# cocowy1/Cost-Volume-Aggregation-in-Stereo-Matching-Revisited

Hardware: AMD Instinct MI355X
Metric: cost-volumes/sec (fwd+bwd) at 544x960 D=192 (higher is better)
Workload: dtype f32

## Files before the change

### cost-volume-aggregation-in-stereo-matching-revisited_amd/csrc/pointwise.hip

```cpp
#include "dca_frag.h"
#include "../../include/dca_hip.h"

__global__ __launch_bounds__(256) void bn_stats_kernel(const float* __restrict__ x, double* __restrict__ part, int N,
                                                       int C, long S, int nchunk, long chunk_len, int vec) {
  const int c = blockIdx.x, ch = blockIdx.y, tid = threadIdx.x;
  const long s0 = ch * chunk_len, s1 = min(S, s0 + chunk_len);
  const float K = x[(long)c * S];
  if (ch == 0 && tid == 0) part[(long)C * nchunk * 2 + c] = (double)K;
  float s = 0.f, ss = 0.f;
  for (int n = 0; n < N; ++n) {
    const float* p = x + ((long)n * C + c) * S;
    if (vec) {
      for (long i = s0 + 4 * tid; i < s1; i += 1024) {
        float4 v = *(const float4*)(p + i);
        v.x -= K; v.y -= K; v.z -= K; v.w -= K;
        s += (v.x + v.y) + (v.z + v.w);
        ss += (v.x * v.x + v.y * v.y) + (v.z * v.z + v.w * v.w);
      }
    } else {
      for (long i = s0 + tid; i < s1; i += 256) {
        const float v = p[i] - K;
        s += v;
        ss += v * v;
      }
    }
  }
  double ds = wave_sum_d((double)s), dss = wave_sum_d((double)ss);
  __shared__ double red[8];
  if ((tid & 63) == 0) { red[(tid >> 6) * 2] = ds; red[(tid >> 6) * 2 + 1] = dss; }
  __syncthreads();
  if (tid == 0) {
    part[((long)c * nchunk + ch) * 2 + 0] = red[0] + red[2] + red[4] + red[6];
    part[((long)c * nchunk + ch) * 2 + 1] = red[1] + red[3] + red[5] + red[7];
  }
}

__device__ __forceinline__ int bn_bound_exp(float gamma, float beta, double count, int c, const unsigned* rp_slots, int rp_n,
                                            const unsigned* rq_slots, int rq_n) {
  unsigned a = 0, b2 = 0;
  const int lane = threadIdx.x & 63;
  if (rp_slots) for (int i = lane; i < rp_n; i += 64) { const unsigned u = rp_slots[(long)c * DCA_AMAX_CSLOTS + i]; a = a > u ? a : u; }
  if (rq_slots) for (int i = lane; i < rq_n; i += 64) { const unsigned u = rq_slots[(long)c * DCA_AMAX_CSLOTS + i]; b2 = b2 > u ? b2 : u; }
#pragma unroll
  for (int o = 32; o > 0; o >>= 1) {
    const unsigned u = (unsigned)__shfl_xor((int)a, o, 64), w = (unsigned)__shfl_xor((int)b2, o, 64);
    a = a > u ? a : u;
    b2 = b2 > w ? b2 : w;
  }
  const float b = (fabsf(gamma) * sqrtf((float)count) + fabsf(beta) + __uint_as_float(a) + __uint_as_float(b2)) * 1.0001f;
  return x2_scale_exp(__float_as_uint(b));
}

__global__ __launch_bounds__(64) void bn_finalize_kernel(const double* __restrict__ part, int nchunk, double count,
                                   const float* __restrict__ gamma, const float* __restrict__ beta,
                                   float* __restrict__ running_mean, float* __restrict__ running_var, float momentum,
                                   float eps, int training, float* __restrict__ stats, int* __restrict__ zexps,
                                   const unsigned* __restrict__ rp_slots, int rp_n, const unsigned* __restrict__ rq_slots,
                                   int rq_n, int C) {
  const int c = blockIdx.x, lane = threadIdx.x;
  float mean, var;
  if (training) {
    double s = 0.0, ss = 0.0;
    for (int i = lane; i < nchunk; i += 64) {
      s += part[((long)c * nchunk + i) * 2 + 0];
      ss += part[((long)c * nchunk + i) * 2 + 1];
    }
    s = wave_sum_d(s);
    ss = wave_sum_d(ss);
    const double ms = s / count;
    double v = ss / count - ms * ms;
    if (v < 0.0) v = 0.0;
    const double m = part[(long)C * nchunk * 2 + c] + ms;
    mean = (float)m;
    var = (float)v;
    if (running_mean && lane == 0) {
      const double unb = count > 1.0 ? v * count / (count - 1.0) : v;
      running_mean[c] = (1.f - momentum) * running_mean[c] + momentum * mean;
      running_var[c] = (1.f - momentum) * running_var[c] + momentum * (float)unb;
    }
  } else {
    mean = running_mean[c];
    var = running_var[c];
  }
  const float g = gamma ? gamma[c] : 1.f, b = beta ? beta[c] : 0.f;
  const int ze = zexps ? bn_bound_exp(g, b, count, c, rp_slots, rp_n, rq_slots, rq_n) : 0;
  if (lane != 0) return;
  const float invstd = 1.0f / sqrtf(var + eps);
  stats[c] = mean;
  stats[C + c] = invstd;
  stats[2 * C + c] = g * invstd;
  stats[3 * C + c] = b - mean * g * invstd;
  if (zexps) zexps[c] = ze;
}

__global__ __launch_bounds__(64) void bn_finalize_centered_kernel(const double* __restrict__ part, int nchunk,
                                   const float* __restrict__ gamma, const float* __restrict__ beta,
                                   float* __restrict__ running_mean, float* __restrict__ running_var, float momentum,
                                   float eps, float* __restrict__ stats, int* __restrict__ zexps,
                                   const unsigned* __restrict__ rp_slots, int rp_n, const unsigned* __restrict__ rq_slots,
                                   int rq_n, int C) {
  const int c = blockIdx.x, lane = threadIdx.x;
  const double* p = part + (long)c * nchunk * 4;
  const double kref = p[0];
  double n = 0.0, s = 0.0, q = 0.0;
  for (int i = lane; i < nchunk; i += 64) {
    const double ki = p[i * 4 + 0], ni = p[i * 4 + 1], si = p[i * 4 + 2], qi = p[i * 4 + 3];
    const double dk = ki - kref;
    n += ni;
    s += si + ni * dk;
    q += qi + 2.0 * dk * si + ni * dk * dk;
  }
  n = wave_sum_d(n);
  s = wave_sum_d(s);
  q = wave_sum_d(q);
  const float g = gamma ? gamma[c] : 1.f, b = beta ? beta[c] : 0.f;
  const int ze = zexps ? bn_bound_exp(g, b, n, c, rp_slots, rp_n, rq_slots, rq_n) : 0;
  if (lane != 0) return;
  const double ms = s / n;
  double v = q / n - ms * ms;
  if (v < 0.0) v = 0.0;
  const float mean = (float)(kref + ms), var = (float)v;
  if (running_mean) {
    const double unb = n > 1.0 ? v * n / (n - 1.0) : v;
    running_mean[c] = (1.f - momentum) * running_mean[c] + momentum * mean;
    running_var[c] = (1.f - momentum) * running_var[c] + momentum * (float)unb;
  }
  const float invstd = 1.0f / sqrtf(var + eps);
  stats[c] = mean;
  stats[C + c] = invstd;
  stats[2 * C + c] = g * invstd;
  stats[3 * C + c] = b - mean * g * invstd;
  if (zexps) zexps[c] = ze;
}


__global__ __launch_bounds__(256) void bn_apply_kernel(const float* __restrict__ y, const float* __restrict__ stats,
                                                       const float* __restrict__ res_pre, const float* __restrict__ res_post,
                                                       float* __restrict__ z, int N, int C, long S, long chunk_len,
                                                       float slope, int vec, unsigned* __restrict__ zmax,
                                                       unsigned* __restrict__ ymax) {
  const int c = blockIdx.y, ch = blockIdx.x, tid = threadIdx.x;
  const long s0 = ch * chunk_len, s1 = min(S, s0 + chunk_len);
  const float mean = stats[c], sc = stats[2 * C + c], sh = stats[3 * C + c];
  float am = 0.f, ym = 0.f;
  for (int n = N - 1; n >= 0; --n) {
    const long base = ((long)n * C + c) * S;
    if (vec) {
      for (long i = s0 + 4 * tid; i < s1; i += 1024) {
        float4 v = *(const float4*)(y + base + i);
        ym = fmaxf(fmaxf(ym, fmaxf(fabsf(v.x - mean), fabsf(v.y - mean))), fmaxf(fabsf(v.z - mean), fabsf(v.w - mean)));
        v.x = v.x * sc + sh; v.y = v.y * sc + sh; v.z = v.z * sc + sh; v.w = v.w * sc + sh;
        if (res_pre) { const float4 r = *(const float4*)(res_pre + base + i); v.x += r.x; v.y += r.y; v.z += r.z; v.w += r.w; }
        v.x = act_apply(v.x, slope); v.y = act_apply(v.y, slope); v.z = act_apply(v.z, slope); v.w = act_apply(v.w, slope);
        if (res_post) { const float4 r = *(const float4*)(res_post + base + i); v.x += r.x; v.y += r.y; v.z += r.z; v.w += r.w; }
        *(float4*)(z + base + i) = v;
        am = fmaxf(fmaxf(am, fmaxf(fabsf(v.x), fabsf(v.y))), fmaxf(fabsf(v.z), fabsf(v.w)));
      }
    } else {
      for (long i = s0 + tid; i < s1; i += 256) {
        const float yv = y[base + i];
        ym = fmaxf(ym, fabsf(yv - mean));
        float v = yv * sc + sh;
        if (res_pre) v += res_pre[base + i];
        v = act_apply(v, slope);
        if (res_post) v += res_post[base + i];
        z[base + i] = v;
        am = fmaxf(am, fabsf(v));
      }
    }
  }
  if (zmax) dca_cmax_put(am, zmax + (long)c * DCA_AMAX_CSLOTS + ch);
  if (ymax) dca_cmax_put(ym, ymax + (long)c * DCA_AMAX_CSLOTS + ch);
}

__device__ __forceinline__ void px2_split(float v, int e, unsigned short& h, unsigned short& l) {
  _Float16 hh, ll;
  x2_split(v, e, hh, ll);
  h = __builtin_bit_cast(unsigned short, hh);
  l = __builtin_bit_cast(unsigned short, ll);
}
typedef unsigned short u16x8 __attribute__((ext_vector_type(8)));

__global__ __launch_bounds__(256) void bn_apply_pack_kernel(const float* __restrict__ y, const float* __restrict__ stats,
                                                            const int* __restrict__ zexps, char* __restrict__ zp, int N,
                                                            int C, long S, long chunk_len, float slope,
                                                            unsigned* __restrict__ ymax, const float* __restrict__ res_pre,
                                                            const float* __restrict__ res_post, float* __restrict__ zf,
                                                            unsigned* __restrict__ zmax) {
  const int cg = blockIdx.y, ch = blockIdx.x, tid = threadIdx.x;
  const long s0 = ch * chunk_len, s1 = min(S, s0 + chunk_len);
  float mean[8], sc[8], sh[8], ym[8], zm[8];
  int ex[8];
#pragma unroll
  for (int j = 0; j < 8; ++j) {
    const int c = cg * 8 + j;
    mean[j] = stats ? stats[c] : 0.f;
    sc[j] = stats ? stats[2 * C + c] : 1.f;
    sh[j] = stats ? stats[3 * C + c] : 0.f;
    ex[j] = dca_coherent_loadi(zexps + c);
    ym[j] = zm[j] = 0.f;
  }
  const long tb = px2_term_bytes(C, S);
  for (int n = N - 1; n >= 0; --n) {
    const float* yb = y + ((long)n * C + cg * 8) * S;
    char* zb = zp + (long)n * 2 * tb + (long)cg * S * 16;
    const long cb = ((long)n * C + cg * 8) * S;
    for (long i = s0 + tid; i < s1; i += 256) {
      float v[8], rp[8], rq[8];
#pragma unroll
      for (int j = 0; j < 8; ++j) {
        v[j] = yb[j * S + i];
        rp[j] = res_pre ? res_pre[cb + j * S + i] : -0.f;
        rq[j] = res_post ? res_post[cb + j * S + i] : -0.f;
      }
      u16x8 hv, lv;
#pragma unroll
      for (int j = 0; j < 8; ++j) {
        ym[j] = fmaxf(ym[j], fabsf(v[j] - mean[j]));
        const float zz = act_apply(v[j] * sc[j] + sh[j] + rp[j], slope) + rq[j];
        if (zf) zf[cb + j * S + i] = zz;
        zm[j] = fmaxf(zm[j], fabsf(zz));
        unsigned short h, l;
        px2_split(zz, ex[j], h, l);
        hv[j] = h; lv[j] = l;
      }
      *(u16x8*)(zb + i * 16) = hv;
      *(u16x8*)(zb + tb + i * 16) = lv;
    }
  }
  if (ymax) {
#pragma unroll
    for (int j = 0; j < 8; ++j) dca_cmax_put(ym[j], ymax + (long)(cg * 8 + j) * DCA_AMAX_CSLOTS + ch);
  }
  if (zmax) {
#pragma unroll
    for (int j = 0; j < 8; ++j) dca_cmax_put(zm[j], zmax + (long)(cg * 8 + j) * DCA_AMAX_CSLOTS + ch);
  }
}

__global__ __launch_bounds__(256) void bn_apply_pack4_kernel(const float* __restrict__ y, const float* __restrict__ stats,
                                                             const int* __restrict__ zexps, char* __restrict__ zp, int N,
                                                             int C, long S, long chunk_len, float slope,
                                                             unsigned* __restrict__ ymax, const float* __restrict__ res_pre,
                                                             const float* __restrict__ res_post, float* __restrict__ zf,
                                                             unsigned* __restrict__ zmax) {
  const int cg = blockIdx.y, ch = blockIdx.x, tid = threadIdx.x;
  const long s0 = ch * chunk_len, s1 = min(S, s0 + chunk_len);
  float mean[8], sc[8], sh[8], ym[8], zm[8];
  int ex[8];
#pragma unroll
  for (int j = 0; j < 8; ++j) {
    const int c = cg * 8 + j;
    mean[j] = stats ? stats[c] : 0.f;
    sc[j] = stats ? stats[2 * C + c] : 1.f;
    sh[j] = stats ? stats[3 * C + c] : 0.f;
    ex[j] = dca_coherent_loadi(zexps + c);
    ym[j] = zm[j] = 0.f;
  }
  const long tb = px2_term_bytes(C, S);
  for (int n = N - 1; n >= 0; --n) {
    const long cb = ((long)n * C + cg * 8) * S;
    char* zb = zp + (long)n * 2 * tb + (long)cg * S * 16;
    for (long i = s0 + 4 * tid; i < s1; i += 1024) {
      u16x8 hv[4], lv[4];
#pragma unroll
      for (int j = 0; j < 8; ++j) {
        const float4 v4 = *(const float4*)(y + cb + j * S + i);
        float4 p4 = make_float4(-0.f, -0.f, -0.f, -0.f), q4 = p4;
        if (res_pre) p4 = *(const float4*)(res_pre + cb + j * S + i);
        if (res_post) q4 = *(const float4*)(res_post + cb + j * S + i);
        const float v[4] = {v4.x, v4.y, v4.z, v4.w}, rp[4] = {p4.x, p4.y, p4.z, p4.w}, rq[4] = {q4.x, q4.y, q4.z, q4.w};
        float zz[4];
#pragma unroll
        for (int e = 0; e < 4; ++e) {
          ym[j] = fmaxf(ym[j], fabsf(v[e] - mean[j]));
          zz[e] = act_apply(v[e] * sc[j] + sh[j] + rp[e], slope) + rq[e];
          zm[j] = fmaxf(zm[j], fabsf(zz[e]));
          unsigned short h, l;
          px2_split(zz[e], ex[j], h, l);
          hv[e][j] = h; lv[e][j] = l;
        }
        if (zf) *(float4*)(zf + cb + j * S + i) = make_float4(zz[0], zz[1], zz[2], zz[3]);
      }
#pragma unroll
      for (int e = 0; e < 4; ++e) {
        *(u16x8*)(zb + (i + e) * 16) = hv[e];
        *(u16x8*)(zb + tb + (i + e) * 16) = lv[e];
      }
    }
  }
  if (ymax) {
#pragma unroll
    for (int j = 0; j < 8; ++j) dca_cmax_put(ym[j], ymax + (long)(cg * 8 + j) * DCA_AMAX_CSLOTS + ch);
  }
  if (zmax) {
#pragma unroll
    for (int j = 0; j < 8; ++j) dca_cmax_put(zm[j], zmax + (long)(cg * 8 + j) * DCA_AMAX_CSLOTS + ch);
  }
}

__global__ __launch_bounds__(256) void cmax_kernel(const float* __restrict__ x, int N, int C, long S, long chunk_len, int vec,
                                                   unsigned* __restrict__ slots) {
  const int c = blockIdx.y, ch = blockIdx.x, tid = threadIdx.x;
  const long s0 = ch * chunk_len, s1 = min(S, s0 + chunk_len);
  float m = 0.f;
  for (int n = 0; n < N; ++n) {
    const float* p = x + ((long)n * C + c) * S;
    if (vec) {
      for (long i = s0 + 4 * tid; i < s1; i += 1024) {
        const float4 v = *(const float4*)(p + i);
        m = fmaxf(fmaxf(m, fmaxf(fabsf(v.x), fabsf(v.y))), fmaxf(fabsf(v.z), fabsf(v.w)));
      }
    } else {
      for (long i = s0 + tid; i < s1; i += 256) m = fmaxf(m, fabsf(p[i]));
    }
  }
  dca_cmax_put(m, slots + (long)c * DCA_AMAX_CSLOTS + ch);
}

__global__ __launch_bounds__(64) void cmax_exps_kernel(const unsigned* __restrict__ slots, int nslots, int* __restrict__ exps) {
  const int c = blockIdx.x, lane = threadIdx.x;
  unsigned v = 0;
  for (int i = lane; i < nslots; i += 64) { const unsigned u = slots[(long)c * DCA_AMAX_CSLOTS + i]; v = v > u ? v : u; }
#pragma unroll
  for (int o = 32; o > 0; o >>= 1) { const unsigned u = (unsigned)__shfl_xor((int)v, o, 64); v = v > u ? v : u; }
  if (lane == 0) exps[c] = x2_scale_exp(v);
}

__global__ __launch_bounds__(256) void bn_bwd_reduce_kernel(const float* __restrict__ dz, const float* __restrict__ y,
                                                            const float* __restrict__ res_pre,
                                                            const float* __restrict__ stats,
                                                            double* __restrict__ part, int N, int C, long S,
                                                            int nchunk, long chunk_len, float slope, int vec,
                                                            unsigned* __restrict__ gmax) {
  const int c = blockIdx.x, ch = blockIdx.y, tid = threadIdx.x;
  const long s0 = ch * chunk_len, s1 = min(S, s0 + chunk_len);
  const float mean = stats[c], invstd = stats[C + c], sc = stats[2 * C + c], sh = stats[3 * C + c];
  float a0 = 0.f, a1 = 0.f, gm = 0.f;
  for (int n = N - 1; n >= 0; --n) {
    const long base = ((long)n * C + c) * S;
    if (vec) {
      for (long i = s0 + 4 * tid; i < s1; i += 1024) {
        const float4 yv = *(const float4*)(y + base + i);
        const float4 dv = *(const float4*)(dz + base + i);
        float4 rv = make_float4(0.f, 0.f, 0.f, 0.f);
        if (res_pre) rv = *(const float4*)(res_pre + base + i);
        const float ys[4] = {yv.x, yv.y, yv.z, yv.w}, ds[4] = {dv.x, dv.y, dv.z, dv.w}, rs[4] = {rv.x, rv.y, rv.z, rv.w};
#pragma unroll
        for (int j = 0; j < 4; ++j) {
          const float u = ys[j] * sc + sh + rs[j];
          const float g = ds[j] * (u > 0.f ? 1.f : slope);
          a0 += g;
          a1 += g * (ys[j] - mean) * invstd;
          gm = fmaxf(gm, fabsf(g));
        }
      }
    } else {
      for (long i = s0 + tid; i < s1; i += 256) {
        const float yv = y[base + i];
        float u = yv * sc + sh;
        if (res_pre) u += res_pre[base + i];
        const float g = dz[base + i] * (u > 0.f ? 1.f : slope);
        a0 += g;
        a1 += g * (yv - mean) * invstd;
        gm = fmaxf(gm, fabsf(g));
      }
    }
  }
  double d0 = wave_sum_d((double)a0), d1 = wave_sum_d((double)a1);
  __shared__ double red[8];
  if ((tid & 63) == 0) { red[(tid >> 6) * 2] = d0; red[(tid >> 6) * 2 + 1] = d1; }
  __syncthreads();
  if (tid == 0) {
    part[((long)c * nchunk + ch) * 2 + 0] = red[0] + red[2] + red[4] + red[6];
    part[((long)c * nchunk + ch) * 2 + 1] = red[1] + red[3] + red[5] + red[7];
  }
  if (gmax) dca_cmax_put(gm, gmax + (long)c * DCA_AMAX_CSLOTS + ch);
}

__global__ __launch_bounds__(64) void bn_bwd_finalize_kernel(const double* __restrict__ part, int nchunk, double count,
                                       float* __restrict__ dgb, int C, const float* __restrict__ stats, int training,
                                       const unsigned* __restrict__ gmax, const unsigned* __restrict__ ymax, int ymax_slots,
                                       int* __restrict__ dyexps) {
  const int c = blockIdx.x, lane = threadIdx.x;
  double s0 = 0.0, s1 = 0.0;
  for (int i = lane; i < nchunk; i += 64) {
    s0 += part[((long)c * nchunk + i) * 2 + 0];
    s1 += part[((long)c * nchunk + i) * 2 + 1];
  }
  s0 = wave_sum_d(s0);
  s1 = wave_sum_d(s1);
  unsigned gmb = 0, ymb = 0;
  if (dyexps) {
    for (int i = lane; i < nchunk; i += 64) { const unsigned u = gmax[(long)c * DCA_AMAX_CSLOTS + i]; gmb = gmb > u ? gmb : u; }
    if (ymax)
      for (int i = lane; i < ymax_slots; i += 64) { const unsigned u = ymax[(long)c * DCA_AMAX_CSLOTS + i]; ymb = ymb > u ? ymb : u; }
#pragma unroll
    for (int o = 32; o > 0; o >>= 1) {
      const unsigned u = (unsigned)__shfl_xor((int)gmb, o, 64), w = (unsigned)__shfl_xor((int)ymb, o, 64);
      gmb = gmb > u ? gmb : u;
      ymb = ymb > w ? ymb : w;
    }
  }
  if (lane != 0) return;
  dgb[c] = (float)s1;
  dgb[C + c] = (float)s0;
  dgb[2 * C + c] = (float)(s0 / count);
  dgb[3 * C + c] = (float)(s1 / count);
  if (dyexps) {
    const float invstd = stats[C + c], sc = fabsf(stats[2 * C + c]);
    const float xh = ymax ? __uint_as_float(ymb) * invstd : sqrtf((float)count);
    float bound = __uint_as_float(gmb);
    if (training) bound += fabsf((float)(s0 / count)) + xh * fabsf((float)(s1 / count));
    dyexps[c] = x2_scale_exp(__float_as_uint(bound * sc * 1.0001f));
  }
}

__global__ __launch_bounds__(256) void bn_bwd_apply_kernel(const float* __restrict__ dz, const float* __restrict__ y,
                                    const float* __restrict__ res_pre, const float* __restrict__ stats,
                                    const float* __restrict__ dgb, float* __restrict__ dy, float* __restrict__ g_out,
                                    int N, int C, long S, long chunk_len, float slope, int training, int vec,
                                    unsigned* __restrict__ dmax) {
  const int c = blockIdx.y, ch = blockIdx.x, tid = threadIdx.x;
  const long s0 = ch * chunk_len, s1 = min(S, s0 + chunk_len);
  const float mean = stats[c], invstd = stats[C + c], sc = stats[2 * C + c], sh = stats[3 * C + c];
  const float k1 = training ? dgb[2 * C + c] : 0.f, k2 = training ? dgb[3 * C + c] * invstd : 0.f;
  float am = 0.f;
  for (int n = 0; n < N; ++n) {
    const long base = ((long)n * C + c) * S;
    if (vec) {
      for (long i = s0 + 4 * tid; i < s1; i += 1024) {
        const float4 yv = *(const float4*)(y + base + i), dv = *(const float4*)(dz + base + i);
        float4 rv = make_float4(0.f, 0.f, 0.f, 0.f);
        if (res_pre) rv = *(const float4*)(res_pre + base + i);
        const float ys[4] = {yv.x, yv.y, yv.z, yv.w}, ds[4] = {dv.x, dv.y, dv.z, dv.w}, rs[4] = {rv.x, rv.y, rv.z, rv.w};
        float o[4], g[4];
#pragma unroll
        for (int j = 0; j < 4; ++j) {
          const float u = ys[j] * sc + sh + rs[j];
          g[j] = ds[j] * (u > 0.f ? 1.f : slope);
          o[j] = (g[j] - k1 - (ys[j] - mean) * k2) * sc;
        }
        *(float4*)(dy + base + i) = make_float4(o[0], o[1], o[2], o[3]);
        if (g_out) *(float4*)(g_out + base + i) = make_float4(g[0], g[1], g[2], g[3]);
        am = fmaxf(fmaxf(am, fmaxf(fabsf(o[0]), fabsf(o[1]))), fmaxf(fabsf(o[2]), fabsf(o[3])));
      }
    } else {
      for (long i = s0 + tid; i < s1; i += 256) {
        const float yv = y[base + i];
        float u = yv * sc + sh;
        if (res_pre) u += res_pre[base + i];
        const float g = dz[base + i] * (u > 0.f ? 1.f : slope);
        float v = g;
        if (training) v -= dgb[2 * C + c] + (yv - mean) * invstd * dgb[3 * C + c];
        dy[base + i] = v * sc;
        if (g_out) g_out[base + i] = g;
        am = fmaxf(am, fabsf(v * sc));
      }
    }
  }
  if (dmax) dca_cmax_put(am, dmax + (long)c * DCA_AMAX_CSLOTS + ch);
}

__global__ __launch_bounds__(256) void bn_bwd_apply_pack_kernel(const float* __restrict__ dz, const float* __restrict__ y,
                                    const float* __restrict__ stats, const float* __restrict__ dgb,
                                    const int* __restrict__ dyexps, char* __restrict__ dyp, int N, int C, long S,
                                    long chunk_len, float slope, int training) {
  const int cg = blockIdx.y, ch = blockIdx.x, tid = threadIdx.x;
  const long s0 = ch * chunk_len, s1 = min(S, s0 + chunk_len);
  float mean[8], sc[8], sh[8], k1[8], k2[8];
  int ex[8];
#pragma unroll
  for (int j = 0; j < 8; ++j) {
    const int c = cg * 8 + j;
    mean[j] = stats[c]; sc[j] = stats[2 * C + c]; sh[j] = stats[3 * C + c];
    k1[j] = training ? dca_coherent_loadf(dgb + 2 * C + c) : 0.f;
    k2[j] = training ? dca_coherent_loadf(dgb + 3 * C + c) * stats[C + c] : 0.f;
    ex[j] = dca_coherent_loadi(dyexps + c);
  }
  const long tb = px2_term_bytes(C, S);
  for (int n = 0; n < N; ++n) {
    const long base = ((long)n * C + cg * 8) * S;
    char* ob = dyp + (long)n * 2 * tb + (long)cg * S * 16;
    for (long i = s0 + tid; i < s1; i += 256) {
      float yv[8], dv[8];
#pragma unroll
      for (int j = 0; j < 8; ++j) { yv[j] = y[base + j * S + i]; dv[j] = dz[base + j * S + i]; }
      u16x8 hv, lv;
#pragma unroll
      for (int j = 0; j < 8; ++j) {
        const float u = yv[j] * sc[j] + sh[j];
        const float g = dv[j] * (u > 0.f ? 1.f : slope);
        const float o = (g - k1[j] - (yv[j] - mean[j]) * k2[j]) * sc[j];
        unsigned short h, l;
        px2_split(o, ex[j], h, l);
        hv[j] = h; lv[j] = l;
      }
      *(u16x8*)(ob + i * 16) = hv;
      *(u16x8*)(ob + tb + i * 16) = lv;
    }
  }
}

__global__ __launch_bounds__(256) void avgpool3d_fwd_kernel(const float* __restrict__ x, float* __restrict__ y, int Di,
                                                            int Hi, int Wi, int Do, int Ho, int Wo) {
  const long row = blockIdx.x;
  const int od = (int)(row % Do);
  const long nc = row / Do;
  const long plane = (long)Di * Hi * Wi;
  const __amdgpu_buffer_rsrc_t xr = dca_rsrc(x + nc * plane, plane * 4);
  const int HW = Ho * Wo, end = min(HW, ((int)blockIdx.y + 1) * 1024);
  for (int i = blockIdx.y * 1024 + threadIdx.x; i < end; i += 256) {
    const int oh = i / Wo, ow = i - oh * Wo;
    float s = 0.f;
#pragma unroll
    for (int kd = 0; kd < 3; ++kd) {
      const int d = 2 * od - 1 + kd;
#pragma unroll
      for (int kh = 0; kh < 3; ++kh) {
        const int h = 2 * oh - 1 + kh;
#pragma unroll
        for (int kw = 0; kw < 3; ++kw) {
          const int w = 2 * ow - 1 + kw;
          const int ok = (int)((unsigned)d < (unsigned)Di) & (int)((unsigned)h < (unsigned)Hi) & (int)((unsigned)w < (unsigned)Wi);
          s += dca_bload1(xr, ((d * Hi + h) * Wi + w) * 4, ok);
        }
      }
    }
    y[row * HW + i] = s * (1.0f / 27.0f);
  }
}

__global__ __launch_bounds__(256) void avgpool3d_bwd_kernel(const float* __restrict__ gy, float* __restrict__ gx,
                                                            const float* __restrict__ res, const float* __restrict__ res2,
                                                            int Di, int Hi, int Wi, int Do, int Ho, int Wo) {
  const long row = blockIdx.x;
  const int d = (int)(row % Di);
  const long nc = row / Di;
  const long plane = (long)Do * Ho * Wo;
  const __amdgpu_buffer_rsrc_t gr = dca_rsrc(gy + nc * plane, plane * 4);
  const int HW = Hi * Wi, end = min(HW, ((int)blockIdx.y + 1) * 1024);
  const int d0 = d >> 1, dn = d & 1;
  for (int i = blockIdx.y * 1024 + threadIdx.x; i < end; i += 256) {
    const int h = i / Wi, w = i - h * Wi;
    const int h0 = h >> 1, hn = h & 1, w0 = w >> 1, wn = w & 1;
    float s = 0.f;
#pragma unroll
    for (int a = 0; a < 2; ++a)
#pragma unroll
      for (int b = 0; b < 2; ++b)
#pragma unroll
        for (int c = 0; c < 2; ++c) {
          const int od = d0 + a, oh = h0 + b, ow = w0 + c;
          const int ok = (a <= dn) & (b <= hn) & (c <= wn) & (int)(od < Do) & (int)(oh < Ho) & (int)(ow < Wo);
          s += dca_bload1(gr, ((od * Ho + oh) * Wo + ow) * 4, ok);
        }
    float o = s * (1.0f / 27.0f) + (res ? res[row * HW + i] : 0.f);
    if (res2) o += res2[row * HW + i];
    gx[row * HW + i] = o;
  }
}

__global__ __launch_bounds__(256) void avgpool3d_fwd_tiled_kernel(const float* __restrict__ x, float* __restrict__ y,
                                                                  int Di, int Hi, int Wi, int Do, int Ho, int Wo) {
  constexpr int TH = 8, TW = 32, FH = 2 * TH + 1, PW = 2 * TW + 2;
  __shared__ __attribute__((aligned(16))) float tile[3 * FH * PW];
  const int tid = threadIdx.x, ow0 = blockIdx.x * TW, oh0 = blockIdx.y * TH;
  const int od = blockIdx.z % Do;
  const long nc = blockIdx.z / Do;
  const long plane = (long)Di * Hi * Wi;
  const __amdgpu_buffer_rsrc_t xr = dca_rsrc(x + nc * plane, plane * 4);
  constexpr int NQ = 3 * FH * 16, KQ = (NQ + 255) / 256;
  float4 rq[KQ];
#pragma unroll
  for (int k = 0; k < KQ; ++k) {
    const int it = tid + 256 * k, q = it & 15, row = it >> 4, a = row / FH, b = row - a * FH;
    const int d = 2 * od - 1 + a, h = 2 * oh0 - 1 + b, w = 2 * ow0 + 4 * q;
    const int ok = (int)(it < NQ) & (int)((unsigned)d < (unsigned)Di) & (int)((unsigned)h < (unsigned)Hi) & (int)(w < Wi);
    rq[k] = dca_bload4(xr, ((d * Hi + h) * Wi + w) * 4, ok);
  }
  float redge = 0.f;
  {
    const int a = tid / FH, b = tid - a * FH;
    const int d = 2 * od - 1 + a, h = 2 * oh0 - 1 + b, w = 2 * ow0 - 1;
    const int ok = (int)(tid < 3 * FH) & (int)((unsigned)d < (unsigned)Di) & (int)((unsigned)h < (unsigned)Hi) &
                   (int)((unsigned)w < (unsigned)Wi);
    redge = dca_bload1(xr, ((d * Hi + h) * Wi + w) * 4, ok);
  }
#pragma unroll
  for (int k = 0; k < KQ; ++k) {
    const int it = tid + 256 * k;
    if (it < NQ) {
      float* p = tile + (it >> 4) * PW + 1 + 4 * (it & 15);
      p[0] = rq[k].x; p[1] = rq[k].y; p[2] = rq[k].z; p[3] = rq[k].w;
    }
  }
  if (tid < 3 * FH) tile[tid * PW] = redge;
  __syncthreads();
  const int hl = tid >> 5, wl = tid & 31, oh = oh0 + hl, ow = ow0 + wl;
  if (oh >= Ho || ow >= Wo) return;
  float s = 0.f;
#pragma unroll
  for (int kd = 0; kd < 3; ++kd)
#pragma unroll
    for (int kh = 0; kh < 3; ++kh) {
      const float* row = tile + (kd * FH + 2 * hl + kh) * PW + 2 * wl;
      const float2 lo = *(const float2*)row;
      s += lo.x;
      s += lo.y;
      s += row[2];
    }
  y[((nc * Do + od) * Ho + oh) * (long)Wo + ow] = s * (1.0f / 27.0f);
}

__global__ __launch_bounds__(256) void avgpool3d_bwd_vec_kernel(const float* __restrict__ gy, float* __restrict__ gx,
                                                                const float* __restrict__ res, const float* __restrict__ res2,
                                                                int Di, int Hi, int Wi, int Do, int Ho, int Wo) {
  const int BD = Di / 2 + 1, BH = Hi / 2 + 1;
  const int bd = (int)(blockIdx.x % BD);
  const long nc = blockIdx.x / BD;
  const long plane = (long)Do * Ho * Wo;
  const __amdgpu_buffer_rsrc_t gr = dca_rsrc(gy + nc * plane, plane * 4);
  const int WQ = Wi >> 2, HQ = BH * WQ, end = min(HQ, ((int)blockIdx.y + 1) * 1024);
  for (int i = blockIdx.y * 1024 + threadIdx.x; i < end; i += 256) {
    const int bh = i / WQ, t = i - bh * WQ, c0 = 2 * t;
    float g[2][2][3];
#pragma unroll
    for (int a = 0; a < 2; ++a)
#pragma unroll
      for (int b = 0; b < 2; ++b)
#pragma unroll
        for (int c = 0; c < 3; ++c) {
          const int od = bd - 1 + a, oh = bh - 1 + b, ow = c0 + c;
          const int ok = (int)((unsigned)od < (unsigned)Do) & (int)((unsigned)oh < (unsigned)Ho) & (int)(ow < Wo);
          g[a][b][c] = dca_bload1(gr, ((od * Ho + oh) * Wo + ow) * 4, ok);
        }
#pragma unroll
    for (int pd = 0; pd < 2; ++pd) {
      const int d = 2 * bd - 1 + pd;
      if ((unsigned)d >= (unsigned)Di) continue;
#pragma unroll
      for (int ph = 0; ph < 2; ++ph) {
        const int h = 2 * bh - 1 + ph;
        if ((unsigned)h >= (unsigned)Hi) continue;
        float o[4];
#pragma unroll
        for (int e = 0; e < 4; ++e) {
          float s = 0.f;
#pragma unroll
          for (int a = pd; a < 2; ++a)
#pragma unroll
            for (int b = ph; b < 2; ++b) {
              s += g[a][b][e >> 1];
              s += (e & 1) ? g[a][b][(e + 1) >> 1] : 0.f;
            }
          o[e] = s * (1.0f / 27.0f);
        }
        const long off = ((nc * Di + d) * Hi + h) * (long)Wi + 4 * t;
        if (res) {
          const float4 r = *(const float4*)(res + off);
          o[0] += r.x; o[1] += r.y; o[2] += r.z; o[3] += r.w;
        }
        if (res2) {
          const float4 r = *(const float4*)(res2 + off);
          o[0] += r.x; o[1] += r.y; o[2] += r.z; o[3] += r.w;
        }
        *(float4*)(gx + off) = make_float4(o[0], o[1], o[2], o[3]);
      }
    }
  }
}

__device__ __forceinline__ void lin_src(int o, float rs, int n, int& i0, int& i1, float& l0, float& l1) {
  float src = rs * ((float)o + 0.5f) - 0.5f;
  if (src < 0.f) src = 0.f;
  i0 = (int)src;
  i1 = i0 + (i0 < n - 1 ? 1 : 0);
  l1 = src - (float)i0;
  l0 = 1.f - l1;
}

__global__ void trilinear_fwd_kernel(const float* __restrict__ x, float* __restrict__ y, long NC, int Di, int Hi,
                                     int Wi, int s) {
  const int Do = Di * s, Ho = Hi * s, Wo = Wi * s;
  const float rs = 1.0f / (float)s;
  const long total = NC * Do * Ho * Wo;
  for (long idx = (long)blockIdx.x * blockDim.x + threadIdx.x; idx < total; idx += (long)gridDim.x * blockDim.x) {
    const int ow = idx % Wo;
    long t = idx / Wo;
    const int oh = t % Ho; t /= Ho;
    const int od = t % Do;
    const long nc = t / Do;
    int d0, d1, h0, h1, w0, w1;
    float ld0, ld1, lh0, lh1, lw0, lw1;
    lin_src(od, rs, Di, d0, d1, ld0, ld1);
    lin_src(oh, rs, Hi, h0, h1, lh0, lh1);
    lin_src(ow, rs, Wi, w0, w1, lw0, lw1);
    const float* p = x + nc * Di * Hi * Wi;
#define XV(d, h, w) p[((long)(d) * Hi + (h)) * Wi + (w)]
    const float v = ld0 * (lh0 * (lw0 * XV(d0, h0, w0) + lw1 * XV(d0, h0, w1)) +
                           lh1 * (lw0 * XV(d0, h1, w0) + lw1 * XV(d0, h1, w1))) +
                    ld1 * (lh0 * (lw0 * XV(d1, h0, w0) + lw1 * XV(d1, h0, w1)) +
                           lh1 * (lw0 * XV(d1, h1, w0) + lw1 * XV(d1, h1, w1)));
#undef XV
    y[idx] = v;
  }
}

__device__ __forceinline__ float lin_w(int o, int i, float rs, int n) {
  int i0, i1;
  float l0, l1;
  lin_src(o, rs, n, i0, i1, l0, l1);
  return (i0 == i ? l0 : 0.f) + (i1 == i ? l1 : 0.f);
}

__global__ void trilinear_bwd_kernel(const float* __restrict__ gy, float* __restrict__ gx, long NC, int Di, int Hi,
                                     int Wi, int s) {
  const int Do = Di * s, Ho = Hi * s, Wo = Wi * s;
  const float rs = 1.0f / (float)s;
  const long total = NC * Di * Hi * Wi;
  const int lo_off = (s + 1) / 2, hi_off = (3 * s) / 2 - 1 + (s & 1);
  for (long idx = (long)blockIdx.x * blockDim.x + threadIdx.x; idx < total; idx += (long)gridDim.x * blockDim.x) {
    const int w = idx % Wi;
    long t = idx / Wi;
    const int h = t % Hi; t /= Hi;
    const int d = t % Di;
    const long nc = t / Di;
    const float* p = gy + nc * Do * Ho * Wo;
    const int od0 = max(0, s * d - lo_off), od1 = min(Do - 1, s * d + hi_off);
    const int oh0 = max(0, s * h - lo_off), oh1 = min(Ho - 1, s * h + hi_off);
    const int ow0 = max(0, s * w - lo_off), ow1 = min(Wo - 1, s * w + hi_off);
    float acc = 0.f;
    for (int od = od0; od <= od1; ++od) {
      const float wd = lin_w(od, d, rs, Di);
      if (wd == 0.f) continue;
      for (int oh = oh0; oh <= oh1; ++oh) {
        const float wh = lin_w(oh, h, rs, Hi);
        if (wh == 0.f) continue;
        const float* row = p + ((long)od * Ho + oh) * Wo;
        float r = 0.f;
        for (int ow = ow0; ow <= ow1; ++ow) r += lin_w(ow, w, rs, Wi) * row[ow];
        acc += wd * wh * r;
      }
    }
    gx[idx] = acc;
  }
}

__global__ __launch_bounds__(256) void trilinear_up2_fwd_kernel(const float* __restrict__ x, float* __restrict__ y,
                                                                int Di, int Hi, int Wi) {
  const int mw = blockIdx.x * 64 + (threadIdx.x & 63), mh = blockIdx.y * 4 + (threadIdx.x >> 6);
  const int md = blockIdx.z % Di;
  const long nc = blockIdx.z / Di;
  if (mw >= Wi || mh >= Hi) return;
  const float* p = x + nc * Di * Hi * Wi;
  const int dm = max(md - 1, 0), dp = min(md + 1, Di - 1), hm = max(mh - 1, 0), hp = min(mh + 1, Hi - 1);
  const int wm = max(mw - 1, 0), wp = min(mw + 1, Wi - 1);
  float r0[3][3], r1[3][3];
  const int ds[3] = {dm, md, dp}, hs[3] = {hm, mh, hp};
#pragma unroll
  for (int a = 0; a < 3; ++a)
#pragma unroll
    for (int b = 0; b < 3; ++b) {
      const float* row = p + ((long)ds[a] * Hi + hs[b]) * Wi;
      const float xm = row[wm], x0 = row[mw], xp = row[wp];
      r0[a][b] = 0.25f * xm + 0.75f * x0;
      r1[a][b] = 0.75f * x0 + 0.25f * xp;
    }
  const int Ho = 2 * Hi, Wo = 2 * Wi;
  float* q = y + nc * (2L * Di) * Ho * Wo;
#pragma unroll
  for (int pd = 0; pd < 2; ++pd)
#pragma unroll
    for (int ph = 0; ph < 2; ++ph) {
      const int a0 = pd ? 1 : 0, a1 = pd ? 2 : 1, b0 = ph ? 1 : 0, b1 = ph ? 2 : 1;
      const float wa0 = pd ? 0.75f : 0.25f, wa1 = pd ? 0.25f : 0.75f, wb0 = ph ? 0.75f : 0.25f, wb1 = ph ? 0.25f : 0.75f;
      float2 o;
      o.x = wa0 * (wb0 * r0[a0][b0] + wb1 * r0[a0][b1]) + wa1 * (wb0 * r0[a1][b0] + wb1 * r0[a1][b1]);
      o.y = wa0 * (wb0 * r1[a0][b0] + wb1 * r1[a0][b1]) + wa1 * (wb0 * r1[a1][b0] + wb1 * r1[a1][b1]);
      *(float2*)(q + ((long)(2 * md + pd) * Ho + 2 * mh + ph) * Wo + 2 * mw) = o;
    }
}

__device__ __forceinline__ void up2_bwd_w(int i, int n, float w[4]) {
  w[0] = (i > 0) ? 0.25f : 0.f;
  w[1] = (i > 0) ? 0.75f : 1.0f;
  w[2] = (i < n - 1) ? 0.75f : 1.0f;
  w[3] = (i < n - 1) ? 0.25f : 0.f;
}

__global__ __launch_bounds__(256) void trilinear_up2_bwd_kernel(const float* __restrict__ gy, float* __restrict__ gx,
                                                                int Di, int Hi, int Wi) {
  const int w = blockIdx.x * 256 + threadIdx.x, h = blockIdx.y;
  const int d = blockIdx.z % Di;
  const long nc = blockIdx.z / Di;
  const int Ho = 2 * Hi, Wo = 2 * Wi;
  const long plane = (2L * Di) * Ho * Wo;
  const __amdgpu_buffer_rsrc_t gr = dca_rsrc(gy + nc * plane, plane * 4);
  const int wok = (int)(w < Wi);
  float wd[4], wh[4], ww[4];
  up2_bwd_w(d, Di, wd); up2_bwd_w(h, Hi, wh); up2_bwd_w(w, Wi, ww);
  float acc = 0.f;
#pragma unroll
  for (int a = 0; a < 4; ++a) {
    const int od = 2 * d - 1 + a;
#pragma unroll
    for (int b = 0; b < 4; ++b) {
      const int oh = 2 * h - 1 + b;
      const int ok = wok & (int)(wd[a] != 0.f) & (int)(wh[b] != 0.f);
      const int off = ((od * Ho + oh) * Wo + 2 * w) * 4;
      const float2 mid = dca_bload2(gr, off, ok);
      const float lo = dca_bload1(gr, off - 4, ok & (int)(ww[0] != 0.f));
      const float hi = dca_bload1(gr, off + 8, ok & (int)(ww[3] != 0.f));
      float r = ww[1] * mid.x + ww[2] * mid.y;
      r += ww[0] * lo;
      r += ww[3] * hi;
      acc += wd[a] * wh[b] * r;
    }
  }
  if (wok) gx[((nc * Di + d) * Hi + h) * Wi + w] = acc;
}

__global__ __launch_bounds__(256) void trilinear_up2_bwd_tiled_kernel(const float* __restrict__ gy, float* __restrict__ gx,
                                                                      int Di, int Hi, int Wi) {
  constexpr int TH = 8, TW = 32, FH = 2 * TH + 2, FW = 2 * TW + 2, PW = FW + 2;
  __shared__ __attribute__((aligned(16))) float tile[4 * FH * PW];
  const int tid = threadIdx.x, w0 = blockIdx.x * TW, h0 = blockIdx.y * TH;
  const int d = blockIdx.z % Di;
  const long nc = blockIdx.z / Di;
  const int Do = 2 * Di, Ho = 2 * Hi, Wo = 2 * Wi;
  const long plane = (long)Do * Ho * Wo;
  const __amdgpu_buffer_rsrc_t gr = dca_rsrc(gy + nc * plane, plane * 4);
  constexpr int NQ = 4 * FH * 16, KQ = (NQ + 255) / 256;
  float4 rq[KQ];
#pragma unroll
  for (int k = 0; k < KQ; ++k) {
    const int it = tid + 256 * k, q = it & 15, row = it >> 4, a = row / FH, b = row - a * FH;
    const int od = 2 * d - 1 + a, oh = 2 * h0 - 1 + b, ow = 2 * w0 + 4 * q;
    const int ok = (int)(it < NQ) & (int)((unsigned)od < (unsigned)Do) & (int)((unsigned)oh < (unsigned)Ho) &
                   (int)(ow < Wo);
    rq[k] = dca_bload4(gr, ((od * Ho + oh) * Wo + ow) * 4, ok);
  }
  float redge = 0.f;
  {
    const int side = tid & 1, row = tid >> 1, a = row / FH, b = row - a * FH;
    const int od = 2 * d - 1 + a, oh = 2 * h0 - 1 + b, ow = side ? 2 * w0 + 2 * TW : 2 * w0 - 1;
    const int ok = (int)(tid < 4 * FH * 2) & (int)((unsigned)od < (unsigned)Do) & (int)((unsigned)oh < (unsigned)Ho) &
                   (int)((unsigned)ow < (unsigned)Wo);
    redge = dca_bload1(gr, ((od * Ho + oh) * Wo + ow) * 4, ok);
  }
#pragma unroll
  for (int k = 0; k < KQ; ++k) {
    const int it = tid + 256 * k;
    if (it < NQ) {
      float* p = tile + (it >> 4) * PW + 1 + 4 * (it & 15);
      p[0] = rq[k].x; p[1] = rq[k].y; p[2] = rq[k].z; p[3] = rq[k].w;
    }
  }
  if (tid < 4 * FH * 2) tile[(tid >> 1) * PW + ((tid & 1) ? FW - 1 : 0)] = redge;
  __syncthreads();
  const int hl = tid >> 5, wl = tid & 31, h = h0 + hl, w = w0 + wl;
  if (h >= Hi || w >= Wi) return;
  float wd[4], wh[4], ww[4];
  up2_bwd_w(d, Di, wd); up2_bwd_w(h, Hi, wh); up2_bwd_w(w, Wi, ww);
  float acc = 0.f;
#pragma unroll
  for (int a = 0; a < 4; ++a)
#pragma unroll
    for (int b = 0; b < 4; ++b) {
      const float* row = tile + (a * FH + 2 * hl + b) * PW + 2 * wl;
      const float2 lo = *(const float2*)row, hi = *(const float2*)(row + 2);
      float r = ww[1] * lo.y + ww[2] * hi.x;
      r += ww[0] * lo.x;
      r += ww[3] * hi.y;
      acc += wd[a] * wh[b] * r;
    }
  gx[((nc * Di + d) * Hi + h) * Wi + w] = acc;
}

static int ew_grid(long total) {
  long g = (total + 255) / 256;
  return (int)(g < 8192 ? (g > 0 ? g : 1) : 8192);
}

static void chunking(long S, int C, int* nchunk, long* chunk_len) {
  long want = (2048 + C - 1) / C;
  if (want > 256) want = 256;
  long len = (S + want - 1) / want;
  len = ((len + 1023) / 1024) * 1024;
  *chunk_len = len;
  *nchunk = (int)((S + len - 1) / len);
}

extern "C" int dca_bn_num_chunks(int C, long S) {
  int n; long l;
  chunking(S, C, &n, &l);
  return n;
}
extern "C" int dca_bn_pack_chunks(int C, long S) {
  int n; long l;
  chunking(S, (C + 7) / 8, &n, &l);
  return n;
}

extern "C" int dca_bn_stats(const float* x, double* part, int N, int C, long S, hipStream_t stream) {
  DCA_REQUIRE(x && part && N > 0 && C > 0 && S > 0 && C <= 65535);
  int nchunk; long len;
  chunking(S, C, &nchunk, &len);
  const int vec = (S % 4 == 0) && (((uintptr_t)x & 15) == 0);
  hipLaunchKernelGGL(bn_stats_kernel, dim3(C, nchunk), dim3(256), 0, stream, x, part, N, C, S, nchunk, len, vec);
  return dca_launch_status();
}

extern "C" int dca_bn_finalize(const double* part, int nchunk, double count, const float* gamma, const float* beta,
                               float* running_mean, float* running_var, float momentum, float eps, int training,
                               float* stats, int* zexps, const unsigned* rpre_slots, int rpre_n,
                               const unsigned* rpost_slots, int rpost_n, int C, hipStream_t stream) {
  DCA_REQUIRE(stats && C > 0 && (training ? (part != nullptr && nchunk > 0) : (running_mean && running_var)));
  DCA_REQUIRE(zexps == nullptr || training);
  DCA_REQUIRE((rpre_slots == nullptr || (rpre_n > 0 && rpre_n <= DCA_AMAX_CSLOTS)) &&
              (rpost_slots == nullptr || (rpost_n > 0 && rpost_n <= DCA_AMAX_CSLOTS)));
  hipLaunchKernelGGL(bn_finalize_kernel, dim3(C), dim3(64), 0, stream, part, nchunk, count, gamma, beta,
                     running_mean, running_var, momentum, eps, training, stats, zexps, rpre_slots, rpre_n, rpost_slots,
                     rpost_n, C);
  return dca_launch_status();
}

extern "C" int dca_bn_finalize_centered(const double* part, int nchunk, const float* gamma, const float* beta,
                                        float* running_mean, float* running_var, float momentum, float eps, float* stats,
                                        int* zexps, const unsigned* rpre_slots, int rpre_n, const unsigned* rpost_slots,
                                        int rpost_n, int C, hipStream_t stream) {
  DCA_REQUIRE(part && nchunk > 0 && stats && C > 0 && ((running_mean == nullptr) == (running_var == nullptr)));
  DCA_REQUIRE((rpre_slots == nullptr || (rpre_n > 0 && rpre_n <= DCA_AMAX_CSLOTS)) &&
              (rpost_slots == nullptr || (rpost_n > 0 && rpost_n <= DCA_AMAX_CSLOTS)));
  hipLaunchKernelGGL(bn_finalize_centered_kernel, dim3(C), dim3(64), 0, stream, part, nchunk, gamma, beta, running_mean,
                     running_var, momentum, eps, stats, zexps, rpre_slots, rpre_n, rpost_slots, rpost_n, C);
  return dca_launch_status();
}

extern "C" int dca_bn_apply(const float* y, const float* stats, const float* res_pre, const float* res_post, float* z,
                            int N, int C, long S, float slope, unsigned* zmax, unsigned* ymax, hipStream_t stream) {
  DCA_REQUIRE(y && stats && z && N > 0 && C > 0 && S > 0 && C <= 65535);
  int nchunk; long len;
  chunking(S, C, &nchunk, &len);
  const uintptr_t al = (uintptr_t)y | (uintptr_t)z | (uintptr_t)res_pre | (uintptr_t)res_post;
  const int vec = (S % 4 == 0) && ((al & 15) == 0);
  hipLaunchKernelGGL(bn_apply_kernel, dim3(nchunk, C), dim3(256), 0, stream, y, stats, res_pre, res_post, z, N, C, S, len,
                     slope, vec, zmax, ymax);
  return dca_launch_status();
}

extern "C" int dca_bn_apply_pack(const float* y, const float* stats, const int* zexps, void* zp, int N, int C, long S,
                                 float slope, unsigned* ymax, const float* res_pre, const float* res_post, float* zf,
                                 unsigned* zmax, hipStream_t stream) {
  DCA_REQUIRE(y && zexps && zp && N > 0 && C > 0 && C % 8 == 0 && S > 0 && C / 8 <= 65535 && ((((uintptr_t)zp) & 15) == 0));
  DCA_REQUIRE(stats != nullptr || (ymax == nullptr && slope == 1.f));
  int nchunk; long len;
  chunking(S, C / 8, &nchunk, &len);
  const uintptr_t al = (uintptr_t)y | (uintptr_t)res_pre | (uintptr_t)res_post | (uintptr_t)zf;
  const bool four = (res_pre || res_post) && S % 4 == 0 && (al & 15) == 0;
  auto kern = four ? bn_apply_pack4_kernel : bn_apply_pack_kernel;
  hipLaunchKernelGGL(kern, dim3(nchunk, C / 8), dim3(256), 0, stream, y, stats, zexps, (char*)zp, N, C, S, len, slope, ymax,
                     res_pre, res_post, zf, zmax);
  return dca_launch_status();
}

extern "C" int dca_cmax_f32(const float* x, int N, int C, long S, unsigned* slots, hipStream_t stream) {
  DCA_REQUIRE(x && slots && N > 0 && C > 0 && S > 0 && C <= 65535);
  int nchunk; long len;
  chunking(S, C, &nchunk, &len);
  const int vec = (S % 4 == 0) && ((((uintptr_t)x) & 15) == 0);
  hipLaunchKernelGGL(cmax_kernel, dim3(nchunk, C), dim3(256), 0, stream, x, N, C, S, len, vec, slots);
  return dca_launch_status();
}

extern "C" int dca_cmax_exps(const unsigned* slots, int nslots, int C, int* exps, hipStream_t stream) {
  DCA_REQUIRE(slots && exps && C > 0 && nslots > 0 && nslots <= DCA_AMAX_CSLOTS);
  hipLaunchKernelGGL(cmax_exps_kernel, dim3(C), dim3(64), 0, stream, slots, nslots, exps);
  return dca_launch_status();
}

extern "C" int dca_bn_backward(const float* dz, const float* y, const float* res_pre, const float* stats,
                               double* part, float* dgb, float* dy, float* g_out, int N, int C, long S, float slope,
                               int training, unsigned* dmax, hipStream_t stream) {
  DCA_REQUIRE(dz && y && stats && part && dgb && dy && N > 0 && C > 0 && S > 0 && C <= 65535);
  int nchunk; long len;
  chunking(S, C, &nchunk, &len);
  const uintptr_t al = (uintptr_t)dz | (uintptr_t)y | (uintptr_t)res_pre | (uintptr_t)dy | (uintptr_t)g_out;
  const int vec = (S % 4 == 0) && ((al & 15) == 0);
  hipLaunchKernelGGL(bn_bwd_reduce_kernel, dim3(C, nchunk), dim3(256), 0, stream, dz, y, res_pre, stats, part, N, C, S,
                     nchunk, len, slope, vec, (unsigned*)nullptr);
  hipLaunchKernelGGL(bn_bwd_finalize_kernel, dim3(C), dim3(64), 0, stream, part, nchunk, (double)N * (double)S, dgb, C,
                     stats, training, (const unsigned*)nullptr, (const unsigned*)nullptr, 0, (int*)nullptr);
  hipLaunchKernelGGL(bn_bwd_apply_kernel, dim3(nchunk, C), dim3(256), 0, stream, dz, y, res_pre, stats, dgb, dy, g_out, N, C,
                     S, len, slope, training, vec, dmax);
  return dca_launch_status();
}

extern "C" int dca_bn_backward_reduce(const float* dz, const float* y, const float* stats, double* part, float* dgb, int N,
                                      int C, long S, float slope, int training, hipStream_t stream) {
  DCA_REQUIRE(dz && y && stats && part && dgb && N > 0 && C > 0 && S > 0 && C <= 65535);
  int nchunk; long len;
  chunking(S, C, &nchunk, &len);
  const int vec = (S % 4 == 0) && ((((uintptr_t)dz | (uintptr_t)y) & 15) == 0);
  hipLaunchKernelGGL(bn_bwd_reduce_kernel, dim3(C, nchunk), dim3(256), 0, stream, dz, y, (const float*)nullptr, stats, part,
                     N, C, S, nchunk, len, slope, vec, (unsigned*)nullptr);
  hipLaunchKernelGGL(bn_bwd_finalize_kernel, dim3(C), dim3(64), 0, stream, part, nchunk, (double)N * (double)S, dgb, C,
                     stats, training, (const unsigned*)nullptr, (const unsigned*)nullptr, 0, (int*)nullptr);
  return dca_launch_status();
}

extern "C" int dca_bn_backward_pack(const float* dz, const float* y, const float* stats, double* part, float* dgb, void* dyp,
                                    int* dyexps, unsigned* gmax, const unsigned* ymax, int ymax_slots, int N, int C, long S,
                                    float slope, int training, hipStream_t stream) {
  DCA_REQUIRE(dz && y && stats && part && dgb && dyp && dyexps && gmax && N > 0 && C > 0 && C % 8 == 0 && S > 0 && C <= 65535);
  DCA_REQUIRE((ymax == nullptr || (ymax_slots > 0 && ymax_slots <= DCA_AMAX_CSLOTS)) && ((((uintptr_t)dyp) & 15) == 0));
  int nchunk; long len;
  chunking(S, C, &nchunk, &len);
  const uintptr_t al = (uintptr_t)dz | (uintptr_t)y;
  const int vec = (S % 4 == 0) && ((al & 15) == 0);
  hipLaunchKernelGGL(bn_bwd_reduce_kernel, dim3(C, nchunk), dim3(256), 0, stream, dz, y, (const float*)nullptr, stats, part,
                     N, C, S, nchunk, len, slope, vec, gmax);
  hipLaunchKernelGGL(bn_bwd_finalize_kernel, dim3(C), dim3(64), 0, stream, part, nchunk, (double)N * (double)S, dgb, C,
                     stats, training, (const unsigned*)gmax, ymax, ymax_slots, dyexps);
  int pchunk; long plen;
  chunking(S, C / 8, &pchunk, &plen);
  hipLaunchKernelGGL(bn_bwd_apply_pack_kernel, dim3(pchunk, C / 8), dim3(256), 0, stream, dz, y, stats, dgb, dyexps,
                     (char*)dyp, N, C, S, plen, slope, training);
  return dca_launch_status();
}

extern "C" int dca_avgpool3d_fwd(const float* x, float* y, long NC, int Di, int Hi, int Wi, hipStream_t stream) {
  DCA_REQUIRE(x && y && NC > 0 && Di > 0 && Hi > 0 && Wi > 0);
  const int Do = (Di + 1) / 2, Ho = (Hi + 1) / 2, Wo = (Wi + 1) / 2;
  DCA_REQUIRE((long)Di * Hi * Wi * 4 < 0x7ffffff0L && NC * Do < 0x7fffffffL);
  if (Wi % 4 == 0 && (((uintptr_t)x) & 15) == 0 && NC * Do <= 65535 && cdiv(Ho, 8) <= 65535) {
    hipLaunchKernelGGL(avgpool3d_fwd_tiled_kernel, dim3(cdiv(Wo, 32), cdiv(Ho, 8), (unsigned)(NC * Do)), dim3(256), 0, stream,
                       x, y, Di, Hi, Wi, Do, Ho, Wo);
    return dca_launch_status();
  }
  hipLaunchKernelGGL(avgpool3d_fwd_kernel, dim3((unsigned)(NC * Do), cdiv((long)Ho * Wo, 1024)), dim3(256), 0, stream, x,
                     y, Di, Hi, Wi, Do, Ho, Wo);
  return dca_launch_status();
}

extern "C" int dca_avgpool3d_bwd(const float* gy, float* gx, const float* res, const float* res2, long NC, int Di, int Hi,
                                 int Wi, hipStream_t stream) {
  DCA_REQUIRE(gy && gx && NC > 0 && Di > 0 && Hi > 0 && Wi > 0 && (res || !res2));
  const int Do = (Di + 1) / 2, Ho = (Hi + 1) / 2, Wo = (Wi + 1) / 2;
  DCA_REQUIRE((long)Di * Hi * Wi * 4 < 0x7ffffff0L && NC * Di < 0x7fffffffL);
  if (Wi % 4 == 0 && ((((uintptr_t)gx) | ((uintptr_t)res) | ((uintptr_t)res2)) & 15) == 0) {
    hipLaunchKernelGGL(avgpool3d_bwd_vec_kernel, dim3((unsigned)(NC * (Di / 2 + 1)), cdiv((long)(Hi / 2 + 1) * (Wi / 4), 1024)),
                       dim3(256), 0, stream, gy, gx, res, res2, Di, Hi, Wi, Do, Ho, Wo);
    return dca_launch_status();
  }
  hipLaunchKernelGGL(avgpool3d_bwd_kernel, dim3((unsigned)(NC * Di), cdiv((long)Hi * Wi, 1024)), dim3(256), 0, stream, gy,
                     gx, res, res2, Di, Hi, Wi, Do, Ho, Wo);
  return dca_launch_status();
}

extern "C" int dca_trilinear_fwd(const float* x, float* y, long NC, int Di, int Hi, int Wi, int scale,
                                 hipStream_t stream) {
  DCA_REQUIRE(x && y && NC > 0 && Di > 0 && Hi > 0 && Wi > 0 && scale >= 1);
  if (scale == 2 && Hi <= 65535 && NC * Di <= 65535 && (((uintptr_t)y & 7) == 0)) {
    hipLaunchKernelGGL(trilinear_up2_fwd_kernel, dim3(cdiv(Wi, 64), cdiv(Hi, 4), (unsigned)(NC * Di)), dim3(256), 0, stream,
                       x, y, Di, Hi, Wi);
    return dca_launch_status();
  }
  const long total = NC * Di * Hi * Wi * scale * scale * scale;
  hipLaunchKernelGGL(trilinear_fwd_kernel, dim3(ew_grid(total)), dim3(256), 0, stream, x, y, NC, Di, Hi, Wi, scale);
  return dca_launch_status();
}

extern "C" int dca_trilinear_bwd(const float* gy, float* gx, long NC, int Di, int Hi, int Wi, int scale,
                                 hipStream_t stream) {
  DCA_REQUIRE(gy && gx && NC > 0 && Di > 0 && Hi > 0 && Wi > 0 && scale >= 1);
  if (scale == 2 && cdiv(Hi, 8) <= 65535 && NC * Di <= 65535 && 32L * Di * Hi * Wi < 0x7ffffff0L && Wi % 2 == 0 &&
      (((uintptr_t)gy & 15) == 0)) {
    hipLaunchKernelGGL(trilinear_up2_bwd_tiled_kernel, dim3(cdiv(Wi, 32), cdiv(Hi, 8), (unsigned)(NC * Di)), dim3(256), 0,
                       stream, gy, gx, Di, Hi, Wi);
    return dca_launch_status();
  }
  if (scale == 2 && Hi <= 65535 && NC * Di <= 65535 && 32L * Di * Hi * Wi < 0x7ffffff0L && (((uintptr_t)gy & 7) == 0)) {
    hipLaunchKernelGGL(trilinear_up2_bwd_kernel, dim3(cdiv(Wi, 256), Hi, (unsigned)(NC * Di)), dim3(256), 0, stream, gy, gx,
                       Di, Hi, Wi);
    return dca_launch_status();
  }
  hipLaunchKernelGGL(trilinear_bwd_kernel, dim3(ew_grid(NC * Di * Hi * Wi)), dim3(256), 0, stream, gy, gx, NC, Di, Hi,
                     Wi, scale);
  return dca_launch_status();
}
```

### cost-volume-aggregation-in-stereo-matching-revisited_amd/models/augment/cva.py

```python
import torch
import torch.nn as nn

from .._bootstrap import ensure as _ensure
from ..submodule import ConvBn3d, ConvBnReLU3d, conv3d_plain, convbn_3d
from .semantic_level import SemanticLevelContext

ops = _ensure().ops


class _DeconvBn3d(nn.Sequential):

    def __init__(self, cin, cout):
        super().__init__(nn.ConvTranspose3d(cin, cout, 3, padding=1, output_padding=1, stride=2, bias=False),
                         nn.BatchNorm3d(cout))

    def forward(self, x, slope=1.0, res_pre=None, res_post=None, pack_out=False):
        return ops.convbn3d(x, self[0], self[1], slope, res_pre, res_post, pack_out=pack_out)


class Multi_Aggregation(nn.Module):

    def __init__(self, in_channels):
        super().__init__()
        self.conv1 = ConvBnReLU3d(in_channels, in_channels * 2, 3, 2, 1)
        self.conv2 = ConvBnReLU3d(in_channels * 2, in_channels * 2, 3, 1, 1)
        self.conv3 = _DeconvBn3d(in_channels * 2, in_channels)
        self.redir = convbn_3d(in_channels, in_channels, kernel_size=1, stride=1, pad=0)

    def forward(self, x, res_post=None):
        c1, skip = ops.convbn3d_pair(x, self.conv1[0][0], self.conv1[0][1], 0.0, self.redir[0], self.redir[1], 1.0,
                                     pack_a=True)
        c2 = self.conv2(c1)
        return self.conv3(c2, slope=0.0, res_pre=skip, res_post=res_post, pack_out="both")


class _Downsample(nn.Sequential):

    def __init__(self):
        super().__init__(nn.AvgPool3d((3, 3, 3), stride=2, padding=1), ConvBn3d(32, 32, 3, 1, 1),
                         nn.ReLU(inplace=True))

    def forward(self, x):
        return self[1](ops.avg_pool3d_k3s2p1(x), slope=0.0)


class _Classify(nn.Sequential):

    def __init__(self, c):
        super().__init__(ConvBn3d(c, c, 3, 1, 1), nn.ReLU(inplace=True),
                         nn.Conv3d(c, 1, kernel_size=3, padding=1, stride=1, bias=False))

    def forward(self, x, alias=False):
        if alias:
            h, xa = self[0](x, slope=0.0, alias=True)
            return conv3d_plain(h, self[2]), xa
        h = self[0](x, slope=0.0)
        if h.dtype != torch.float32:
            return ops.conv3d_c1_lp(h, self[2].weight)
        return conv3d_plain(h, self[2])


class cva(nn.Module):

    def __init__(self, max_disp, in_channel, downsample=True):
        super().__init__()
        self.max_disp = max_disp
        self.channel = in_channel
        if downsample:
            self.downsample = _Downsample()
        self.slc_net = SemanticLevelContext(feats_channels=self.channel, transform_channels=self.channel,
                                            concat_input=True)
        self.classify = _Classify(self.channel)
        self.fuse = nn.Sequential(ConvBn3d(64, 32, 1, 1, 0))
        self.cost_agg = Multi_Aggregation(self.channel)

    def _forward_lp(self, x, res_post):
        lp = x.dtype
        aff = lambda bn: (lambda st, C: (st[2 * C:3 * C], st[3 * C:]))(ops.bn_eval_affine(bn), bn.num_features)
        cost_down = self.downsample[1](ops.avg_pool3d_lp(x), slope=0.0)
        prob_volume = self.classify(cost_down).squeeze(1)
        aug = ops.trilinear_up2_lp(self.slc_net(cost_down, prob_volume), lp)
        sc, sh = aff(self.fuse[0][1])
        fused = ops.conv1x1_lp(aug, self.fuse[0][0].weight, lp, x2=x, scale=sc, shift=sh, slope=1.0)
        agg = self.cost_agg
        sc, sh = aff(agg.conv1[0][1])
        c1 = ops.conv3d_s2_lp(fused, agg.conv1[0][0].weight, sc, sh, 0.0)
        c2 = agg.conv2(c1)
        sc, sh = aff(agg.redir[1])
        skip = ops.conv1x1_lp(fused, agg.redir[0].weight, lp, scale=sc, shift=sh, slope=1.0)
        sc, sh = aff(agg.conv3[1])
        out = ops.deconv3d_lp(c2, agg.conv3[0].weight, lp, sc, sh, 0.0, res_pre=skip, res_post=res_post)
        return prob_volume.unsqueeze(1), out

    def forward(self, cost_volume, downsample=True, res_post=None):
        if cost_volume.dtype != torch.float32:
            if not downsample:
                raise NotImplementedError("reduced-precision path: only the down-sampling form used by GwcNet")
            return self._forward_lp(cost_volume, res_post)
        if downsample:
            if res_post is cost_volume:
                pooled, cost_volume, res_post = ops.avg_pool3d_fork(cost_volume, third=True)
            else:
                pooled, cost_volume = ops.avg_pool3d_fork(cost_volume)
            cost_down = self.downsample[1](pooled, slope=0.0)
            prob_volume = self.classify(cost_down).squeeze(1)
            aug_down = self.slc_net(cost_down, prob_volume)
            aug = ops.trilinear_upsample(aug_down, 2)
        else:
            prob_volume = self.classify(cost_volume).squeeze(1)
            aug = self.slc_net(cost_volume, prob_volume)
        aug = self.fuse[0](aug, x2=cost_volume)
        aug = self.cost_agg(aug, res_post=res_post)
        return prob_volume.unsqueeze(1), aug
```

### cost-volume-aggregation-in-stereo-matching-revisited_amd/ops.py

```python
from __future__ import annotations

import ctypes
import math
import os
import threading
from typing import Optional

import torch

from . import _lib
from . import geometry as _geometry

_C = _lib.CONSTANTS
_vp = ctypes.c_void_p


def _L():
    return _lib.load()


def _ptr(t: Optional[torch.Tensor]):
    return _vp(t.data_ptr()) if t is not None else None


_raw_stream = getattr(torch._C, "_cuda_getCurrentRawStream", None)
_raw_device = getattr(torch._C, "_cuda_getDevice", None)


def _stream():
    if _raw_stream is not None and _raw_device is not None:
        return _vp(_raw_stream(_raw_device()))
    return _vp(torch.cuda.current_stream().cuda_stream)


def _chk(rc: int, name: str):
    if rc != 0:
        raise RuntimeError(f"{name} failed with hipError_t {rc}")


def _req(t: torch.Tensor, name: str, packed_ok: bool = False) -> torch.Tensor:
    if getattr(t, "_dca_px2", None) is not None and not packed_ok:
        raise RuntimeError(f"{name}: got a tensor in the packed px2 operand format (only the f16x2 3x3x3 stride-1 convolution "
                           "reads it; ask the producer for an fp32 result)")
    if not isinstance(t, torch.Tensor) or not t.is_cuda:
        raise RuntimeError(
            f"{name}: the DCANet hot path runs only as HIP kernels on a ROCm device (got "
            f"{'a ' + str(t.device) + ' tensor' if isinstance(t, torch.Tensor) else type(t)}); there is no CPU fallback")
    if t.dtype != torch.float32:
        raise RuntimeError(f"{name}: expected float32, got {t.dtype}")
    t = t.contiguous()
    if t.data_ptr() % 16:
        t = t.clone(memory_format=torch.contiguous_format)
    return t


def _opt(t, name):
    return None if t is None else _req(t, name)


class _GwcVolume(torch.autograd.Function):
    @staticmethod
    def forward(ctx, ref, tgt, maxdisp, num_groups):
        ref, tgt = _req(ref, "build_gwc_volume"), _req(tgt, "build_gwc_volume")
        B, C, H, W = ref.shape
        vol = torch.empty((B, num_groups, maxdisp, H, W), device=ref.device, dtype=torch.float32)
        with torch.cuda.device_of(ref):
            _chk(_L().dca_gwc_volume_fwd(_ptr(ref), _ptr(tgt), _ptr(vol), B, C, H, W, maxdisp, num_groups, _stream()),
                 "dca_gwc_volume_fwd")
        ctx.save_for_backward(ref, tgt)
        ctx.meta = (maxdisp, num_groups)
        return vol

    @staticmethod
    def backward(ctx, gvol):
        ref, tgt = ctx.saved_tensors
        maxdisp, G = ctx.meta
        gvol = _req(gvol, "build_gwc_volume.backward")
        B, C, H, W = ref.shape
        gref, gtgt = torch.empty_like(ref), torch.empty_like(tgt)
        with torch.cuda.device_of(ref):
            _chk(_L().dca_gwc_volume_bwd(_ptr(gvol), _ptr(ref), _ptr(tgt), _ptr(gref), _ptr(gtgt), B, C, H, W,
                                         maxdisp, G, _stream()), "dca_gwc_volume_bwd")
        return gref, gtgt, None, None


class _ConcatVolume(torch.autograd.Function):
    @staticmethod
    def forward(ctx, ref, tgt, maxdisp):
        ref, tgt = _req(ref, "build_concat_volume"), _req(tgt, "build_concat_volume")
        B, C, H, W = ref.shape
        vol = torch.empty((B, 2 * C, maxdisp, H, W), device=ref.device, dtype=torch.float32)
        with torch.cuda.device_of(ref):
            _chk(_L().dca_concat_volume_fwd(_ptr(ref), _ptr(tgt), _ptr(vol), B, C, H, W, maxdisp, _stream()),
                 "dca_concat_volume_fwd")
        ctx.meta = (B, C, H, W, maxdisp)
        return vol

    @staticmethod
    def backward(ctx, gvol):
        B, C, H, W, maxdisp = ctx.meta
        gvol = _req(gvol, "build_concat_volume.backward")
        gref = torch.empty((B, C, H, W), device=gvol.device, dtype=torch.float32)
        gtgt = torch.empty_like(gref)
        with torch.cuda.device_of(gvol):
            _chk(_L().dca_concat_volume_bwd(_ptr(gvol), _ptr(gref), _ptr(gtgt), B, C, H, W, maxdisp, _stream()),
                 "dca_concat_volume_bwd")
        return gref, gtgt, None


def gwc_volume(ref, tgt, maxdisp, num_groups):
    return _GwcVolume.apply(ref, tgt, int(maxdisp), int(num_groups))


class _CostVolume(torch.autograd.Function):

    @staticmethod
    def forward(ctx, maxdisp, num_groups, out_dtype, nseg, has_concat, *tensors):
        refs = [_req(t, "cost_volume.ref") for t in tensors[:nseg]]
        tgts = [_req(t, "cost_volume.tgt") for t in tensors[nseg:2 * nseg]]
        cref = _req(tensors[2 * nseg], "cost_volume.cref") if has_concat else None
        ctgt = _req(tensors[2 * nseg + 1], "cost_volume.ctgt") if has_concat else None
        B, _, H, W = refs[0].shape
        segC = [t.shape[1] for t in refs]
        Cc = cref.shape[1] if has_concat else 0
        for r_, t_ in zip(refs, tgts):
            assert r_.shape == t_.shape and r_.shape[0] == B and tuple(r_.shape[2:]) == (H, W)
        vol = torch.empty((B, num_groups + 2 * Cc, maxdisp, H, W), device=refs[0].device, dtype=out_dtype)
        rp = (ctypes.c_void_p * nseg)(*[t.data_ptr() for t in refs])
        tp = (ctypes.c_void_p * nseg)(*[t.data_ptr() for t in tgts])
        sc = (ctypes.c_int * nseg)(*segC)
        code = 0 if out_dtype == torch.float32 else LP_DTYPES[out_dtype]
        vmax = _cslots(num_groups, vol.device) if (CONV_X2 and AMAX_EMIT and code == 0 and Cc == 0 and B * H <= CSLOTS) else None
        with torch.cuda.device_of(vol):
            _chk(_L().dca_cost_volume_fwd(rp, tp, sc, nseg, _ptr(cref), _ptr(ctgt), Cc, _ptr(vol), B, H, W, maxdisp,
                                          num_groups, code, _ptr(vmax), _stream()), "dca_cost_volume_fwd")
        ctx.save_for_backward(*refs, *tgts)
        ctx.meta = (maxdisp, num_groups, nseg, segC, Cc, (B, H, W))
        return _tag_cmax(vol, vmax, B * H)

    @staticmethod
    def backward(ctx, gvol):
        maxdisp, G, nseg, segC, Cc, (B, H, W) = ctx.meta
        refs, tgts = ctx.saved_tensors[:nseg], ctx.saved_tensors[nseg:]
        gvol = _req(gvol, "cost_volume.backward")
        ref = refs[0] if nseg == 1 else torch.cat(refs, 1)
        tgt = tgts[0] if nseg == 1 else torch.cat(tgts, 1)
        gg = gvol if Cc == 0 else gvol[:, :G].contiguous()
        gref, gtgt = torch.empty_like(ref), torch.empty_like(tgt)
        lib = _L()
        with torch.cuda.device_of(gvol):
            _chk(lib.dca_gwc_volume_bwd(_ptr(gg), _ptr(ref), _ptr(tgt), _ptr(gref), _ptr(gtgt), B, ref.shape[1], H, W,
                                        maxdisp, G, _stream()), "dca_gwc_volume_bwd")
            grads = list(gref.split(segC, 1)) + list(gtgt.split(segC, 1))
            if Cc:
                gc = gvol[:, G:].contiguous()
                gcr = torch.empty((B, Cc, H, W), device=gvol.device, dtype=torch.float32)
                gct = torch.empty_like(gcr)
                _chk(lib.dca_concat_volume_bwd(_ptr(gc), _ptr(gcr), _ptr(gct), B, Cc, H, W, maxdisp, _stream()),
                     "dca_concat_volume_bwd")
                grads += [gcr, gct]
        return (None, None, None, None, None) + tuple(grads)


def cost_volume(ref, tgt, maxdisp, num_groups, cref=None, ctgt=None, out_dtype=torch.float32):
    refs = tuple(ref) if isinstance(ref, (tuple, list)) else (ref,)
    tgts = tuple(tgt) if isinstance(tgt, (tuple, list)) else (tgt,)
    W = refs[0].shape[-1]
    C = sum(t.shape[1] for t in refs)
    cpg = C // num_groups if num_groups else 0
    ok = (W % 4 == 0 and (maxdisp % 4 == 0 or out_dtype != torch.float32) and len(refs) <= 3 and cpg in (1, 2, 4, 8, 16)
          and C % num_groups == 0 and all(t.shape[1] % cpg == 0 for t in refs))
    if not ok:
        if out_dtype != torch.float32:
            raise RuntimeError("cost_volume: the reduced-precision volume needs W % 4 == 0")
        r1 = refs[0] if len(refs) == 1 else torch.cat(refs, 1)
        t1 = tgts[0] if len(tgts) == 1 else torch.cat(tgts, 1)
        vol = gwc_volume(r1, t1, maxdisp, num_groups)
        return vol if cref is None else torch.cat((vol, concat_volume(cref, ctgt, maxdisp)), 1)
    extra = () if cref is None else (cref, ctgt)
    return _CostVolume.apply(int(maxdisp), int(num_groups), out_dtype, len(refs), cref is not None, *refs, *tgts, *extra)


def concat_volume(ref, tgt, maxdisp):
    return _ConcatVolume.apply(ref, tgt, int(maxdisp))


class _SoftArgmin(torch.autograd.Function):
    @staticmethod
    def forward(ctx, x, mode):
        x = _req(x, "softargmin")
        B, K = x.shape[0], x.shape[1]
        HW = x[0, 0].numel()
        out = torch.empty_like(x) if mode == 0 else torch.empty((B, 1) + tuple(x.shape[2:]), device=x.device,
                                                                dtype=torch.float32)
        with torch.cuda.device_of(x):
            _chk(_L().dca_softargmin_fwd(_ptr(x), _ptr(out), B, K, HW, mode, _stream()), "dca_softargmin_fwd")
        ctx.mode = mode
        ctx.save_for_backward(out if mode == 0 else x)
        return out

    @staticmethod
    def backward(ctx, g):
        (aux,) = ctx.saved_tensors
        g = _req(g, "softargmin.backward")
        B, K = aux.shape[0], aux.shape[1]
        HW = aux[0, 0].numel()
        gx = torch.empty_like(aux)
        with torch.cuda.device_of(aux):
            _chk(_L().dca_softargmin_bwd(_ptr(aux), _ptr(g), _ptr(gx), B, K, HW, ctx.mode, _stream()),
                 "dca_softargmin_bwd")
        return gx, None


def softmax_dim1(x):
    return _SoftArgmin.apply(x, 0)


def softargmin(x):
    return _SoftArgmin.apply(x, 1)


def regression(x):
    return _SoftArgmin.apply(x, 2)


CONF_DISP, CONF_DUNI, CONF_MASS, CONF_ENT, CONF_STD, CONF_PLANES = (
    _C[f"DCA_CONF_{n}"] for n in ("DISP", "DUNI", "MASS", "ENT", "STD", "PLANES"))


def _req_no_grad(name, *tensors):
    if torch.is_grad_enabled() and any(isinstance(t, torch.Tensor) and t.requires_grad for t in tensors):
        raise RuntimeError(f"{name} is inference only (no backward): call it under torch.no_grad() or detach its inputs")


def softargmin_stats(logits, radius=1):
    _req_no_grad("softargmin_stats", logits)
    x = _req(logits, "softargmin_stats")
    radius = int(radius)
    if x.dim() < 3 or x.numel() == 0 or radius < 0:
        raise RuntimeError(f"softargmin_stats: expected non-empty (B,K,*spatial) logits and radius >= 0, got "
                           f"{tuple(x.shape)} and radius {radius}")
    B, K = x.shape[0], x.shape[1]
    HW = x[0, 0].numel()
    out = torch.empty((B, CONF_PLANES) + tuple(x.shape[2:]), device=x.device, dtype=torch.float32)
    with torch.cuda.device_of(x):
        _chk(_L().dca_softargmin_stats(_ptr(x), _ptr(out), B, K, HW, min(radius, K), _stream()), "dca_softargmin_stats")
    return out


class _UpSoftArgmin(torch.autograd.Function):

    @staticmethod
    def forward(ctx, logits, scale):
        logits = _req(logits, "up_softargmin")
        B, n, hc, wc = logits.shape
        disp = torch.empty((B, 1, scale * hc, scale * wc), device=logits.device, dtype=torch.float32)
        with torch.cuda.device_of(logits):
            _chk(_L().dca_up_softargmin_fwd(_ptr(logits), _ptr(disp), B, n, hc, wc, scale, _stream()),
                 "dca_up_softargmin_fwd")
        ctx.save_for_backward(logits)
        ctx.scale = scale
        return disp

    @staticmethod
    def backward(ctx, g):
        (logits,) = ctx.saved_tensors
        g = _req(g, "up_softargmin.backward")
        B, n, hc, wc = logits.shape
        s = ctx.scale
        g1 = torch.empty((B, n, s * hc, s * wc), device=logits.device, dtype=torch.float32)
        gl = torch.empty_like(logits)
        with torch.cuda.device_of(logits):
            _chk(_L().dca_up_softargmin_bwd(_ptr(logits), _ptr(g), _ptr(g1), _ptr(gl), B, n, hc, wc, s, _stream()),
                 "dca_up_softargmin_bwd")
        return gl, None


def up_softargmin(logits, scale):
    if logits.shape[1] > 64 or logits.shape[1] < 2 or scale not in (2, 4, 8):
        return softargmin(trilinear_upsample(logits.unsqueeze(1), scale).squeeze(1))
    return _UpSoftArgmin.apply(logits, int(scale))


def _round_up(a, m):
    return (a + m - 1) // m * m


_CONV_MODE = os.environ.get("DCA_CONV", "x2")
CONV_X3 = _CONV_MODE != "fp32"
CONV_X2 = _CONV_MODE == "x2"
WGRAD_S2_X2 = os.environ.get("DCA_WGRAD_S2", "x2") != "fp32"
DECONV_X3 = os.environ.get("DCA_DECONV", "x3") != "fp32"
C1_WGRAD_FUSED = os.environ.get("DCA_C1_WGRAD", "fused") != "expand"
CONV_S2_X2 = os.environ.get("DCA_CONV_S2", "x2") != "fp32"
BN_FUSE = os.environ.get("DCA_BN_FUSE", "1") != "0"
C1_BWD_FUSE = os.environ.get("DCA_C1_BWD", "fused") != "split"
_X3_MIN_WORKGROUPS = 1


AMAX_STATS = {"tagged": 0, "computed": 0, "packed": 0}
CSLOTS = _C["DCA_AMAX_CSLOTS"]
AMAX_EMIT = os.environ.get("DCA_AMAX_EMIT", "1") != "0"
PACK = os.environ.get("DCA_PACK", "1") != "0"


def _cslots(C, device):
    if not AMAX_EMIT:
        return None
    return torch.empty((C * CSLOTS,), device=device, dtype=torch.int32)


def _ver(t):
    return None if t.is_inference() else t._version


def _tag_cmax(t, slots, nslots):
    if slots is not None:
        t._dca_cmax = (slots, int(nslots), _ver(t))
    return t


def _tag_px2(t, exps):
    t._dca_px2 = (exps,)
    return t


def _tag_exps(t, exps):
    t._dca_exps = (exps, _ver(t))


def _tag_twin(t, twin):
    t._dca_twin = (twin, _ver(t))


def _tag_ok(t, name):
    tag = getattr(t, name, None)
    if tag is not None and tag[-1] == _ver(t) and tag[0].device == t.device:
        return tag
    return None


def _copy_tags(src, dst):
    cmax, exps, twin = _tag_ok(src, "_dca_cmax"), _tag_ok(src, "_dca_exps"), _tag_ok(src, "_dca_twin")
    if cmax is not None:
        _tag_cmax(dst, cmax[0], cmax[1])
    if exps is not None:
        _tag_exps(dst, exps[0])
    if twin is not None:
        _tag_twin(dst, twin[0])


def _is_packed(t):
    return getattr(t, "_dca_px2", None) is not None


def _twin_of(t):
    tag = _tag_ok(t, "_dca_twin")
    return None if tag is None else tag[0]


def _slots_of(t):
    tag = _tag_ok(t, "_dca_cmax")
    if tag is not None:
        AMAX_STATS["tagged"] += 1
        return tag[0], tag[1]
    AMAX_STATS["computed"] += 1
    N, C = t.shape[0], t.shape[1]
    S = t[0, 0].numel()
    slots = torch.empty((C * CSLOTS,), device=t.device, dtype=torch.int32)
    lib = _L()
    _chk(lib.dca_cmax_f32(_ptr(t), N, C, S, _ptr(slots), _stream()), "dca_cmax_f32")
    nslots = lib.dca_bn_num_chunks(C, S)
    _tag_cmax(t, slots, nslots)
    return slots, nslots


def _exps_cached(t):
    if _is_packed(t):
        return t._dca_px2[0]
    tag = _tag_ok(t, "_dca_exps")
    return None if tag is None else tag[0]


def _exps_of(t):
    ex = _exps_cached(t)
    if ex is not None:
        return ex
    slots, nslots = _slots_of(t)
    C = t.shape[1]
    ex = torch.empty((C,), device=t.device, dtype=torch.int32)
    _chk(_L().dca_cmax_exps(_ptr(slots), nslots, C, _ptr(ex), _stream()), "dca_cmax_exps")
    _tag_exps(t, ex)
    return ex


def pack_x2(x):
    x = _req(x, "pack_x2")
    N, C = x.shape[0], x.shape[1]
    S = x[0, 0].numel()
    ex = _exps_of(x)
    xp = torch.empty_like(x)
    _chk(_L().dca_bn_apply_pack(_ptr(x), None, _ptr(ex), _ptr(xp), N, C, S, 1.0, None, None, None, None, None, _stream()),
         "dca_bn_apply_pack")
    return _tag_px2(xp, ex)


def _x3_eligible(x, x2, ksize, stride, transposed, A, B):
    if not CONV_X3 or ksize != 3 or stride != 1 or transposed or x2 is not None:
        return False
    N, _, D, H, W = x.shape
    tiles = N * ((D + 3) // 4) * ((H + 7) // 8) * ((W + 15) // 16) * ((B + 31) // 32)
    return tiles >= _X3_MIN_WORKGROUPS and max(A, B) * D * H * W * 4 < 0x7ffffff0


def _dx3_eligible(x, x2, ksize, stride, transposed, A, B):
    if not CONV_X3 or not DECONV_X3 or not transposed or ksize != 3 or stride != 2 or x2 is not None or B > 32 or A > 64:
        return False
    N, _, D, H, W = x.shape
    return W % 4 == 0 and x.data_ptr() % 16 == 0 and max(A, 8) * D * H * W * 4 < 0x7ffffff0 and 256 * D * H * W * 4 < 0x7ffffff0


def _s2x2_eligible(x, x2, ksize, stride, transposed, A, B, scale, res_pre, slope):
    if not (CONV_X2 and CONV_X3 and CONV_S2_X2) or ksize != 3 or stride != 2 or transposed or x2 is not None:
        return False
    if res_pre is not None or A > 256 or A <= 4:
        return False
    N, _, D, H, W = x.shape
    Do, Ho, Wo = (D + 1) // 2, (H + 1) // 2, (W + 1) // 2
    tiles = N * ((Do + 1) // 2) * ((Ho + 3) // 4) * ((Wo + 31) // 32) * ((B + 63) // 64)
    return (W % 4 == 0 and x.data_ptr() % 16 == 0 and tiles >= _X3_MIN_WORKGROUPS
            and (A + 3) * D * H * W * 4 < 0x7ffffff0 and (B + 63) * Do * Ho * Wo * 4 < 0x7ffffff0)


def _c1x3_eligible(x, x2, ksize, A, C1, y):
    if not CONV_X3 or ksize != 1:
        return False
    C2 = 0 if x2 is None else x2.shape[1]
    if (C1, C2) not in ((32, 0), (64, 0), (32, 32)) or A != C1 + C2:
        return False
    S = x[0, 0].numel()
    ptrs = [x.data_ptr(), y.data_ptr()] + ([] if x2 is None else [x2.data_ptr()])
    return S % 4 == 0 and all(p % 16 == 0 for p in ptrs) and 64 * S * 4 < 0x7ffffff0


def _conv_family(x, x2, A, B, ksize, stride, transposed, scale=None, res_pre=None, slope=1.0, y=None):
    if _x3_eligible(x, x2, ksize, stride, transposed, A, B):
        return "x2" if CONV_X2 else "x3"
    if _s2x2_eligible(x, x2, ksize, stride, transposed, A, B, scale, res_pre, slope):
        return "s2x2"
    if _dx3_eligible(x, x2, ksize, stride, transposed, A, B):
        return "dx3"
    return "c1x3" if _c1x3_eligible(x, x2, ksize, A, x.shape[1], y) else "mfma"


def _c1_bwd_route(x, x2, weight, res_pre=None):
    if not C1_BWD_FUSE or res_pre is not None or weight.dim() != 5 or weight.shape[2] != 1 or not torch.is_grad_enabled():
        return "split"
    C1, C2 = x.shape[1], (0 if x2 is None else x2.shape[1])
    if weight.shape[0] != 32 or (C1, C2) not in ((32, 0), (32, 32)) or weight.shape[1] != C1 + C2:
        return "split"
    tensors = (x, weight) if x2 is None else (x, x2, weight)
    if not all(t.is_cuda and t.dtype == torch.float32 and t.requires_grad for t in tensors):
        return "split"
    if x2 is not None and x2.shape != x.shape:
        return "split"
    S = x[0, 0].numel()
    return "fused" if (S % 4 == 0 and x.shape[0] * 32 * S * 4 < 0x7ffff000) else "split"


def _c1_bwd_fused(dz, x, x2, weight):
    tag = getattr(dz, "_dca_lazy", None)
    if tag is None:
        raise RuntimeError("conv3d.backward: expected the gradient the BatchNorm behind this 1x1x1 convolution hands on "
                           "(the tag was lost on the way through autograd)")
    y, stats, dgb, slope, training = tag
    if y.shape != dz.shape or y.shape[0] != x.shape[0] or y.shape[2:] != x.shape[2:]:
        raise RuntimeError("conv3d.backward: the BatchNorm's gradient does not belong to this convolution")
    N, C1 = x.shape[0], x.shape[1]
    C2 = 0 if x2 is None else x2.shape[1]
    S = x[0, 0].numel()
    lib = _L()
    part = torch.empty((lib.dca_conv1_bwd_fused_workspace(N, S, int(x2 is not None)),), device=x.device, dtype=torch.float32)
    gx = torch.empty_like(x)
    gx2 = None if x2 is None else torch.empty_like(x2)
    gw = torch.empty_like(weight)
    _chk(lib.dca_conv1_bwd_fused(_ptr(dz), _ptr(y), _ptr(stats), _ptr(dgb), float(slope), int(training), _ptr(x), _ptr(x2),
                                 _ptr(weight), _ptr(part), _ptr(gx), _ptr(gx2), _ptr(gw), C1 + C2, 1, N, C1, C2,
                                 weight.shape[0], S, _stream()), "dca_conv1_bwd_fused")
    return gx, gx2, gw


def _k3s1(weight, stride, transposed, x2, head=False):
    return x2 is None and not transposed and int(stride) == 1 and weight.shape[2] == 3 and (weight.shape[0] == 1) == head


def _x2_pairs(xp, yp, W):
    return W % 4 == 0 or (xp and yp)


def _wgrad_family(x, dy, Cx, Cy, ksize, stride):
    Di, Hi, Wi = x.shape[2:]
    Do, Ho, Wo = dy.shape[2:]
    xp, yp = _is_packed(x), _is_packed(dy)
    split = (CONV_X3 and ksize == 3 and x.data_ptr() % 16 == 0 and dy.data_ptr() % 16 == 0
             and max(Cx, Cy) * Di * Hi * Wi * 4 < 0x7ffffff0)
    if split and CONV_X2 and stride == 1 and _x2_pairs(xp, yp, Wi):
        return "x2"
    if xp or yp:
        raise RuntimeError("weight gradient: a packed px2 operand can only feed the f16x2 3x3x3 stride-1 kernel")
    if split and stride == 1 and Wi % 4 == 0:
        return "x3"
    if (split and CONV_X2 and WGRAD_S2_X2 and stride == 2 and Wi % 4 == 0 and Wo % 4 == 0
            and (Do, Ho, Wo) == ((Di + 1) // 2, (Hi + 1) // 2, (Wi + 1) // 2)):
        return "s2x2"
    return "mfma"


def _slice_width(ksize, stride, transposed, B):
    if ksize == 1 or transposed:
        return 32
    return 32 if (stride == 1 and B <= 32) else 64


def _prep_weight(w_src, A, B, K, src_ab, flip, ksize, stride, transposed, b_off=0, Bn=None):
    Bn = B if Bn is None else Bn
    if ksize == 1:
        Apad = 32 if A <= 32 else 64
        Bpad = 32
    else:
        Apad = _round_up(A, 8)
        Bpad = 32 if (transposed or (stride == 1 and Bn <= 32)) else 64
    def build():
        wt = torch.empty((K, Apad, Bpad), device=w_src.device, dtype=torch.float32)
        _chk(_L().dca_conv3d_prep_weight(_ptr(w_src), _ptr(wt), A, Bn, Apad, Bpad, K, int(src_ab), int(flip), B, b_off,
                                         _stream()), "dca_conv3d_prep_weight")
        return wt
    return _memo(("prep", A, B, K, int(src_ab), int(flip), Apad, Bpad, b_off, Bn), (w_src,), build,
                 (0, A, Bn, Apad, Bpad, K, int(src_ab), int(flip), B, b_off)), Apad


def _x2_weights(prefix, x, w_src, A, B, src_ab, flip, cached_key):
    lib = _L()
    wx = torch.empty((getattr(lib, prefix + "_weight_bytes")(A, B) // 2,), device=x.device, dtype=torch.int16)
    xexps = _exps_cached(x)
    if xexps is not None:
        AMAX_STATS[cached_key] += 1
        slots, nslots = None, 0
    else:
        slots, nslots = _slots_of(x)
        xexps = torch.empty((A,), device=x.device, dtype=torch.int32)
    _chk(getattr(lib, prefix + "_prep_weight")(_ptr(w_src), _ptr(wx), A, B, int(src_ab), int(flip), _ptr(slots), nslots,
                                               _ptr(xexps), _stream()), prefix + "_prep_weight")
    if slots is not None:
        _tag_exps(x, xexps)
    return wx, xexps


def _x3_weights(w_src, A, B, src_ab, flip):
    def build():
        w3 = torch.empty((_L().dca_conv3d_x3_weight_bytes(A, B) // 2,), device=w_src.device, dtype=torch.int16)
        _chk(_L().dca_conv3d_x3_prep_weight(_ptr(w_src), _ptr(w3), A, B, int(src_ab), int(flip), _stream()),
             "dca_conv3d_x3_prep_weight")
        return w3
    return _memo(("x3prep", A, B, int(src_ab), int(flip)), (w_src,), build, (1, A, B, 0, 0, 27, int(src_ab), int(flip), B, 0))


def _out_dims(dims, ksize, stride, transposed):
    if ksize == 1 or stride == 1:
        return tuple(dims)
    if transposed:
        return tuple(2 * d for d in dims)
    return tuple((d + 1) // 2 for d in dims)


def _conv_sliced(x, x2, w_src, A, B, K, src_ab, flip, ksize, stride, transposed, scale=None, shift=None, slope=1.0,
                 res_pre=None, res_post=None, want_stats=False, emit_amax=False):
    N, C1, Di, Hi, Wi = x.shape
    Do, Ho, Wo = _out_dims((Di, Hi, Wi), ksize, stride, transposed)
    y = torch.empty((N, B, Do, Ho, Wo), device=x.device, dtype=torch.float32)
    packed = _is_packed(x)
    family = _conv_family(x, x2, A, B, ksize, stride, transposed, scale, res_pre, slope, y)
    if packed and family != "x2":
        raise RuntimeError("conv3d: a packed px2 operand can only feed the f16x2 3x3x3 stride-1 convolution")
    lib = _L()
    partials = lambda nchunk: torch.empty((B * nchunk * 4,), device=x.device, dtype=torch.float64)
    part = None
    if family == "x2":
        wx, xexps = _x2_weights("dca_conv3d_x2", x, w_src, A, B, src_ab, flip, "packed" if packed else "tagged")
        if want_stats:
            part = partials(lib.dca_conv3d_x2_stats_chunks(N, B, Di, Hi, Wi))
            _chk(lib.dca_conv3d_x2_forward_stats(_ptr(x), int(packed), _ptr(xexps), _ptr(wx), _ptr(y), _ptr(part), N, A, B,
                                                 Di, Hi, Wi, _stream()), "dca_conv3d_x2_forward_stats")
        else:
            ycm = _cslots(B, x.device) if emit_amax else None
            _chk(lib.dca_conv3d_x2_forward(_ptr(x), int(packed), _ptr(xexps), _ptr(wx), _ptr(y), _ptr(scale), _ptr(shift),
                                           _ptr(res_pre), _ptr(res_post), float(slope), _ptr(ycm), N, A, B, Di, Hi, Wi,
                                           _stream()), "dca_conv3d_x2_forward")
            _tag_cmax(y, ycm, lib.dca_conv3d_x2_stats_chunks(N, B, Di, Hi, Wi))
    elif family == "x3":
        wx = _x3_weights(w_src, A, B, src_ab, flip)
        if want_stats:
            part = partials(lib.dca_conv3d_x3_stats_chunks(N, B, Di, Hi, Wi))
            _chk(lib.dca_conv3d_x3_forward_stats(_ptr(x), _ptr(wx), _ptr(y), _ptr(part), N, A, B, Di, Hi, Wi, _stream()),
                 "dca_conv3d_x3_forward_stats")
        else:
            _chk(lib.dca_conv3d_x3_forward(_ptr(x), _ptr(wx), _ptr(y), _ptr(scale), _ptr(shift), _ptr(res_pre),
                                           _ptr(res_post), float(slope), N, A, B, Di, Hi, Wi, _stream()),
                 "dca_conv3d_x3_forward")
    elif family == "s2x2":
        wx, xexps = _x2_weights("dca_conv3d_s2x2", x, w_src, A, B, src_ab, flip, "tagged")
        nsl = lib.dca_conv3d_s2x2_out_slots(N, B, Di, Hi, Wi)
        ycm = _cslots(B, x.device) if (emit_amax and nsl <= CSLOTS) else None
        _chk(lib.dca_conv3d_s2x2_forward(_ptr(x), _ptr(xexps), _ptr(wx), _ptr(y), _ptr(scale), _ptr(shift), float(slope),
                                         _ptr(res_post), _ptr(ycm), N, A, B, Di, Hi, Wi, _stream()), "dca_conv3d_s2x2_forward")
        if ycm is not None:
            _tag_cmax(y, ycm, nsl)
    elif family == "dx3":
        wx = _x3_weights(w_src, A, B, src_ab, flip)
        if want_stats:
            part = partials(lib.dca_deconv3d_x3_stats_chunks(N, Di, Hi, Wi))
            _chk(lib.dca_deconv3d_x3_forward_stats(_ptr(x), _ptr(wx), _ptr(y), _ptr(part), N, A, B, Di, Hi, Wi,
                                                   _stream()), "dca_deconv3d_x3_forward_stats")
        else:
            _chk(lib.dca_deconv3d_x3_forward(_ptr(x), _ptr(wx), _ptr(y), _ptr(scale), _ptr(shift), _ptr(res_pre),
                                             _ptr(res_post), float(slope), N, A, B, Di, Hi, Wi, _stream()),
                 "dca_deconv3d_x3_forward")
    elif family == "c1x3":
        S = Do * Ho * Wo
        C2 = 0 if x2 is None else x2.shape[1]
        if want_stats:
            part = partials(lib.dca_conv1_x3_stats_chunks(N, S))
        for b0 in range(0, B, 32):
            bn = min(32, B - b0)

            def build_c1(b0=b0, bn=bn):
                wf = torch.empty((lib.dca_conv1_x3_weight_bytes(A) // 2,), device=x.device, dtype=torch.int16)
                _chk(lib.dca_conv1_x3_prep_weight(_ptr(w_src), _ptr(wf), A, bn, int(src_ab), B, b0, _stream()),
                     "dca_conv1_x3_prep_weight")
                return wf
            wf = _memo(("c1x3prep", A, B, int(src_ab), b0, bn), (w_src,), build_c1,
                       (2, A, bn, 0, 0, 1, int(src_ab), 0, B, b0))
            if part is not None:
                _chk(lib.dca_conv1_x3_forward_stats(_ptr(x), _ptr(x2), _ptr(wf), _ptr(y), _ptr(part), N, C1, C2, bn, B, b0,
                                                    S, _stream()), "dca_conv1_x3_forward_stats")
            else:
                _chk(lib.dca_conv1_x3_forward(_ptr(x), _ptr(x2), _ptr(wf), _ptr(y), _ptr(scale), _ptr(shift),
                                              _ptr(res_pre), _ptr(res_post), float(slope), N, C1, C2, bn, B, b0, S,
                                              _stream()), "dca_conv1_x3_forward")
    else:
        width = _slice_width(ksize, stride, transposed, B)
        for b0 in range(0, B, width):
            bn = min(width, B - b0)
            wt, Apad = _prep_weight(w_src, A, B, K, src_ab, flip, ksize, stride, transposed, b0, bn)
            _chk(lib.dca_conv3d_forward(_ptr(x), _ptr(x2), _ptr(wt), _ptr(y), _ptr(scale), _ptr(shift), _ptr(res_pre),
                                        _ptr(res_post), float(slope), N, A, C1, bn, Apad, B, b0, Di, Hi, Wi, Do, Ho, Wo,
                                        ksize, stride, int(transposed), _stream()), "dca_conv3d_forward")
    return (y, part) if want_stats else y


def conv3d_prepared(x, wt, A, Apad, B, ksize, stride, transposed):
    N = x.shape[0]
    Di, Hi, Wi = x.shape[2:]
    Do, Ho, Wo = _out_dims((Di, Hi, Wi), ksize, stride, transposed)
    y = torch.empty((N, B, Do, Ho, Wo), device=x.device, dtype=torch.float32)
    _chk(_L().dca_conv3d_forward(_ptr(x), None, _ptr(wt), _ptr(y), None, None, None, None, 1.0, N, A, A, B, Apad, B, 0,
                                 Di, Hi, Wi, Do, Ho, Wo, ksize, stride, int(transposed), _stream()),
         "dca_conv3d_forward")
    return y


def _conv_forward_impl(x, x2, weight, stride, transposed, scale=None, shift=None, slope=1.0, res_pre=None,
                       res_post=None, want_stats=False, emit_amax=False):
    ksize = weight.shape[2]
    K = ksize ** 3
    if transposed:
        Cin, Cout = weight.shape[0], weight.shape[1]
        src_ab = 1
    else:
        Cout, Cin = weight.shape[0], weight.shape[1]
        src_ab = 0
    assert x.shape[1] + (x2.shape[1] if x2 is not None else 0) == Cin, "conv3d: channel mismatch"
    return _conv_sliced(x, x2, weight, Cin, Cout, K, src_ab, 0, ksize, stride, transposed, scale, shift, slope,
                        res_pre, res_post, want_stats, emit_amax)


def _wgrad(x, dy, dw_view_ptr_tensor, dst_offset, Cx, Cy, ksize, stride, s_cy, s_cx):
    N = x.shape[0]
    Di, Hi, Wi = x.shape[2:]
    Do, Ho, Wo = dy.shape[2:]
    dst = _vp(dw_view_ptr_tensor.data_ptr() + 4 * dst_offset)
    lib = _L()
    family = _wgrad_family(x, dy, Cx, Cy, ksize, stride)
    workspace = lambda nws: torch.empty((nws,), device=x.device, dtype=torch.float32)
    if family == "x2":
        xex, yex = _exps_of(x), _exps_of(dy)
        part = workspace(lib.dca_conv3d_wgrad_x2_workspace(N, Cx, Cy, Di, Hi, Wi))
        _chk(lib.dca_conv3d_wgrad_x2(_ptr(x), int(_is_packed(x)), _ptr(xex), _ptr(dy), int(_is_packed(dy)), _ptr(yex),
                                     _ptr(part), dst, N, Cx, Cy, Di, Hi, Wi, s_cy, s_cx, _stream()), "dca_conv3d_wgrad_x2")
    elif family == "x3":
        part = workspace(lib.dca_conv3d_wgrad_x3_workspace(N, Cx, Cy, Di, Hi, Wi))
        _chk(lib.dca_conv3d_wgrad_x3(_ptr(x), _ptr(dy), _ptr(part), dst, N, Cx, Cy, Di, Hi, Wi, s_cy, s_cx, _stream()),
             "dca_conv3d_wgrad_x3")
    elif family == "s2x2":
        xex, yex = _exps_of(x), _exps_of(dy)
        part = workspace(lib.dca_conv3d_wgrad_s2_x2_workspace(N, Cx, Cy, Di, Hi, Wi))
        _chk(lib.dca_conv3d_wgrad_s2_x2(_ptr(x), _ptr(xex), _ptr(dy), _ptr(yex), _ptr(part), dst, N, Cx, Cy, Di, Hi, Wi,
                                        s_cy, s_cx, _stream()), "dca_conv3d_wgrad_s2_x2")
    else:
        part = workspace(lib.dca_conv3d_wgrad_workspace(N, Cx, Cy, Do, Ho, Wo, ksize, stride))
        _chk(lib.dca_conv3d_wgrad(_ptr(x), _ptr(dy), _ptr(part), dst, N, Cx, Cy, Di, Hi, Wi, Do, Ho, Wo, ksize, stride,
                                  s_cy, s_cx, _stream()), "dca_conv3d_wgrad")


class _Conv3dC1(torch.autograd.Function):

    @staticmethod
    def forward(ctx, x, weight):
        x, weight = _req(x, "conv3d"), _req(weight, "conv3d.weight")
        N, C, D, H, W = x.shape
        with torch.cuda.device_of(x):
            T = _conv_sliced(x, None, weight, C, 27, 1, 1, 0, 1, 1, False)
            y = torch.empty((N, 1, D, H, W), device=x.device, dtype=torch.float32)
            _chk(_L().dca_conv3d_c1_gather(_ptr(T), _ptr(y), N, D, H, W, _stream()), "dca_conv3d_c1_gather")
        ctx.save_for_backward(x, weight)
        return y

    @staticmethod
    def backward(ctx, dy):
        x, weight = ctx.saved_tensors
        dy = _req(dy, "conv3d.backward")
        N, C, D, H, W = x.shape
        gx = gw = None
        lib = _L()
        with torch.cuda.device_of(x):
            if ctx.needs_input_grad[0]:
                gx = torch.empty_like(x)
                _chk(lib.dca_conv3d_c1_bwd_data(_ptr(dy), _ptr(weight), _ptr(gx), N, C, D, H, W, _stream()),
                     "dca_conv3d_c1_bwd_data")
            if ctx.needs_input_grad[1]:
                gw = torch.empty_like(weight)
                if (C1_WGRAD_FUSED and W % 4 == 0 and x.data_ptr() % 16 == 0 and dy.data_ptr() % 16 == 0
                        and x.numel() * 4 < 0x7ffffff0):
                    nws = lib.dca_conv3d_wgrad_workspace(N, C, 27, D, H, W, 1, 1)
                    part = torch.empty((nws,), device=x.device, dtype=torch.float32)
                    _chk(lib.dca_conv3d_c1_wgrad(_ptr(x), _ptr(dy), _ptr(part), _ptr(gw), N, C, D, H, W, _stream()),
                         "dca_conv3d_c1_wgrad")
                else:
                    G = torch.empty((N, 27, D, H, W), device=x.device, dtype=torch.float32)
                    _chk(lib.dca_conv3d_c1_expand(_ptr(dy), _ptr(G), N, D, H, W, _stream()), "dca_conv3d_c1_expand")
                    _wgrad(x, G, gw, 0, C, 27, 1, 1, 1, 27)
        return gx, gw


class _Conv3d(torch.autograd.Function):

    @staticmethod
    def forward(ctx, x, x2, weight, stride, transposed, want_stats=False, alias=False, packed_dy=False, lazy_dy=False):
        x, weight = _req(x, "conv3d", packed_ok=True), _req(weight, "conv3d.weight")
        x2 = _opt(x2, "conv3d.x2")
        if _is_packed(x) and alias:
            raise RuntimeError("conv3d: alias output of a packed px2 operand")
        ctx.save_for_backward(x, x2, weight)
        ctx.meta = (stride, transposed)
        ctx.alias = bool(alias)
        ctx.set_materialize_grads(False)
        ctx.x_px2 = getattr(x, "_dca_px2", None)
        ctx.packed_dy = bool(packed_dy)
        ctx.lazy_dy = bool(lazy_dy)
        ctx.x_exps = None
        Cout, Cin = weight.shape[:2]
        twin = PACK and _k3s1(weight, stride, transposed, x2) and _conv_family(x, None, Cin, Cout, 3, 1, False) == "x2"
        xt = _twin_of(x) if twin else None
        ctx.x_twin = xt
        xin = x if xt is None else xt
        with torch.cuda.device_of(x):
            out = _conv_forward_impl(xin, x2, weight, stride, transposed, want_stats=want_stats)
            ctx.x_exps = _exps_cached(xin)
        if want_stats:
            part = out[1] if out[1] is not None else torch.empty((0,), device=x.device, dtype=torch.float64)
            ctx.mark_non_differentiable(part)
            out = (out[0], part)
        if alias:
            xa = x.view_as(x)
            _copy_tags(x, xa)
            out = (out + (xa,)) if want_stats else (out, xa)
        return out

    @staticmethod
    def backward(ctx, dy, *rest):
        x, x2, weight = ctx.saved_tensors
        xw = x
        if ctx.x_twin is not None:
            xw = ctx.x_twin
        elif ctx.x_px2 is not None:
            _tag_px2(x, ctx.x_px2[0])
        elif ctx.x_exps is not None and _exps_cached(x) is None:
            _tag_exps(x, ctx.x_exps)
        stride, transposed = ctx.meta
        g_alias = _opt(rest[-1], "conv3d.backward") if (ctx.alias and rest) else None
        if dy is None:
            return g_alias, None, None, None, None, None, None, None, None
        if ctx.packed_dy and not _is_packed(dy):
            raise RuntimeError("conv3d.backward: expected the packed px2 gradient of the BatchNorm behind this convolution "
                               "(the tag was lost on the way through autograd)")
        dy = _req(dy, "conv3d.backward", packed_ok=True)
        if ctx.x_twin is not None and not _x2_pairs(True, _is_packed(dy), x.shape[-1]):
            xw = x
        ksize = weight.shape[2]
        K = ksize ** 3
        gx = gx2 = gw = None
        need_x, need_x2, need_w = ctx.needs_input_grad[0], ctx.needs_input_grad[1], ctx.needs_input_grad[2]
        with torch.cuda.device_of(x):
            if transposed:
                Cin, Cout = weight.shape[0], weight.shape[1]
                if need_x:
                    gx = _conv_sliced(dy, None, weight, Cout, Cin, K, 0, 0, 3, 2, False)
                if need_w:
                    gw = torch.empty_like(weight)
                    _wgrad(dy, x, gw, 0, Cout, Cin, 3, 2, Cout * K, K)
            elif ksize == 3:
                Cout, Cin = weight.shape[0], weight.shape[1]
                if need_x:
                    if stride == 1:
                        gx = _conv_sliced(dy, None, weight, Cout, Cin, K, 1, 1, 3, 1, False, res_post=g_alias)
                        g_alias = None
                    else:
                        gx = _conv_sliced(dy, None, weight, Cout, Cin, K, 1, 0, 3, 2, True)
                        if gx.shape != x.shape:
                            raise RuntimeError("stride-2 conv backward needs even input dims")
                if need_w:
                    gw = torch.empty_like(weight)
                    _wgrad(xw, dy, gw, 0, Cin, Cout, 3, stride, Cin * K, K)
            else:
                Cout, Cin = weight.shape[0], weight.shape[1]
                w2 = weight.reshape(Cout, Cin)
                C1 = x.shape[1]
                if Cout not in (32, 64):
                    raise RuntimeError("1x1x1 conv backward-data needs 32 or 64 output channels")
                if ctx.lazy_dy:
                    gx, gx2, gw = _c1_bwd_fused(dy, x, x2, weight)
                    need_x = need_x2 = need_w = False
                if need_x:
                    wa = w2[:, :C1].contiguous()
                    gx = _conv_sliced(dy, None, wa, Cout, C1, 1, 1, 0, 1, 1, False)
                if x2 is not None and need_x2:
                    wb = w2[:, C1:].contiguous()
                    gx2 = _conv_sliced(dy, None, wb, Cout, Cin - C1, 1, 1, 0, 1, 1, False)
                if need_w:
                    gw = torch.empty_like(weight)
                    _wgrad(x, dy, gw, 0, C1, Cout, 1, 1, Cin, 1)
                    if x2 is not None:
                        _wgrad(x2, dy, gw, C1, Cin - C1, Cout, 1, 1, Cin, 1)
        if g_alias is not None:
            gx = g_alias if gx is None else gx + g_alias
        return gx, gx2, gw, None, None, None, None, None, None


class _ConvPair(torch.autograd.Function):

    @staticmethod
    def forward(ctx, x, wa, wb, want_stats, lazy_b=False):
        x, wa, wb = _req(x, "conv_pair"), _req(wa, "conv_pair.weight_a"), _req(wb, "conv_pair.weight_b")
        ctx.save_for_backward(x, wa, wb)
        ctx.lazy_b = bool(lazy_b)
        with torch.cuda.device_of(x):
            if want_stats:
                ya, pa = _conv_forward_impl(x, None, wa, 2, False, want_stats=True)
                yb, pb = _conv_forward_impl(x, None, wb, 1, False, want_stats=True)
            else:
                ya, pa = _conv_forward_impl(x, None, wa, 2, False), None
                yb, pb = _conv_forward_impl(x, None, wb, 1, False), None
        none = lambda: torch.empty((0,), device=x.device, dtype=torch.float64)
        pa, pb = (none() if pa is None else pa), (none() if pb is None else pb)
        ctx.mark_non_differentiable(pa, pb)
        return ya, pa, yb, pb

    @staticmethod
    def backward(ctx, dya, _dpa, dyb, _dpb):
        x, wa, wb = ctx.saved_tensors
        dya, dyb = _req(dya, "conv_pair.backward"), _req(dyb, "conv_pair.backward")
        Ca, Cin, Cb = wa.shape[0], wa.shape[1], wb.shape[0]
        if Cb not in (32, 64):
            raise RuntimeError("1x1x1 conv backward-data needs 32 or 64 output channels")
        with torch.cuda.device_of(x):
            if ctx.lazy_b:
                gb, _, gwb = _c1_bwd_fused(dyb, x, None, wb)
            else:
                gb = _conv_sliced(dyb, None, wb.reshape(Cb, Cin).contiguous(), Cb, Cin, 1, 1, 0, 1, 1, False)
                gwb = None
            gx = _conv_sliced(dya, None, wa, Ca, Cin, 27, 1, 0, 3, 2, True, res_post=gb)
            if gx.shape != x.shape:
                raise RuntimeError("stride-2 conv backward needs even input dims")
            gwa = torch.empty_like(wa)
            _wgrad(x, dya, gwa, 0, Cin, Ca, 3, 2, Cin * 27, 27)
            if gwb is None:
                gwb = torch.empty_like(wb)
                _wgrad(x, dyb, gwb, 0, Cin, Cb, 1, 1, Cin, 1)
        return gx, gwa, gwb, None, None


PAIR_FUSE = os.environ.get("DCA_PAIR_FUSE", "1") != "0"


def convbn3d_pair(x, conv_a, bn_a, slope_a, conv_b, bn_b, slope_b, pack_a=False):
    inference = (not bn_a.training and not bn_b.training and not torch.is_grad_enabled())
    ok = (PAIR_FUSE and not inference and _lp_dtype() is None and conv_a.kernel_size[0] == 3 and conv_a.stride[0] == 2
          and conv_b.kernel_size[0] == 1 and conv_b.weight.shape[0] in (32, 64) and x.dtype == torch.float32
          and not isinstance(conv_a, torch.nn.ConvTranspose3d) and all(d % 2 == 0 for d in x.shape[2:]))
    if not ok:
        return convbn3d(x, conv_a, bn_a, slope_a, pack_out=pack_a), convbn3d(x, conv_b, bn_b, slope_b)
    stats = bool(BN_FUSE and bn_a.training and bn_b.training)
    lazy = _c1_bwd_route(x, None, conv_b.weight) == "fused"
    ya, pa, yb, pb = _ConvPair.apply(x, conv_a.weight, conv_b.weight, stats, lazy)
    za = bn_act(ya, bn_a, slope_a, stats_part=pa if pa.numel() else None, pack_out=pack_a)
    zb = bn_act(yb, bn_b, slope_b, stats_part=pb if pb.numel() else None, lazy_dy=lazy)
    return za, zb


def conv3d(x, weight, stride=1, transposed=False, x2=None):
    if _k3s1(weight, stride, transposed, x2, head=True) and weight.shape[1] in (32, 64):
        return _Conv3dC1.apply(x, weight)
    return _Conv3d.apply(x, x2, weight, int(stride), bool(transposed))


def conv3d_fused_inference(x, weight, stride, transposed, scale, shift, slope, res_pre=None, res_post=None, x2=None):
    x, weight = _req(x, "conv3d"), _req(weight, "conv3d.weight")
    with torch.cuda.device_of(x):
        return _conv_forward_impl(x, _opt(x2, "x2"), weight, int(stride), bool(transposed), _opt(scale, "scale"),
                                  _opt(shift, "shift"), slope, _opt(res_pre, "res_pre"), _opt(res_post, "res_post"),
                                  emit_amax=CONV_X2 and AMAX_EMIT)


def bn_stats_vector(y, gamma, beta, running_mean, running_var, training, momentum, eps, part=None, zexps=None,
                    rpre=None, rpost=None):
    rps, rpn = rpre if rpre is not None else (None, 0)
    rqs, rqn = rpost if rpost is not None else (None, 0)
    N, C = y.shape[0], y.shape[1]
    S = y[0, 0].numel()
    stats = torch.empty((4 * C,), device=y.device, dtype=torch.float32)
    lib = _L()
    if training:
        if part is not None:
            _chk(lib.dca_bn_finalize_centered(_ptr(part), part.numel() // (4 * C), _ptr(gamma), _ptr(beta),
                                              _ptr(running_mean), _ptr(running_var), float(momentum), float(eps),
                                              _ptr(stats), _ptr(zexps), _ptr(rps), rpn, _ptr(rqs), rqn, C, _stream()),
                 "dca_bn_finalize_centered")
            return stats
        nchunk = lib.dca_bn_num_chunks(C, S)
        part = torch.empty((C * nchunk * 2 + C,), device=y.device, dtype=torch.float64)
        _chk(lib.dca_bn_stats(_ptr(y), _ptr(part), N, C, S, _stream()), "dca_bn_stats")
        _chk(lib.dca_bn_finalize(_ptr(part), nchunk, float(N * S), _ptr(gamma), _ptr(beta), _ptr(running_mean),
                                 _ptr(running_var), float(momentum), float(eps), 1, _ptr(stats), _ptr(zexps), _ptr(rps), rpn,
                                 _ptr(rqs), rqn, C, _stream()), "dca_bn_finalize")
    else:
        assert zexps is None
        _chk(lib.dca_bn_finalize(None, 0, float(N * S), _ptr(gamma), _ptr(beta), _ptr(running_mean),
                                 _ptr(running_var), float(momentum), float(eps), 0, _ptr(stats), None, None, 0, None, 0, C,
                                 _stream()), "dca_bn_finalize")
    return stats


def bn_eval_affine(bn):
    C = bn.num_features

    def build():
        stats = torch.empty((4 * C,), device=bn.running_mean.device, dtype=torch.float32)
        _chk(_L().dca_bn_finalize(None, 0, 1.0, _ptr(bn.weight), _ptr(bn.bias), _ptr(bn.running_mean),
                                  _ptr(bn.running_var), 0.1, float(bn.eps), 0, _ptr(stats), None, None, 0, None, 0, C, _stream()),
             "dca_bn_finalize")
        return stats
    src = tuple(t for t in (bn.weight, bn.bias, bn.running_mean, bn.running_var) if t is not None)
    return _memo(("bnfold", float(bn.eps)), src, build)


class _BnAct(torch.autograd.Function):

    @staticmethod
    def forward(ctx, y, gamma, beta, running_mean, running_var, training, momentum, eps, slope, res_pre, res_post,
                part=None, zmax=None, pack_z=False, pack_dy=False, lazy_dy=False):
        y = _req(y, "batch_norm")
        res_pre, res_post = _opt(res_pre, "res_pre"), _opt(res_post, "res_post")
        N, C = y.shape[0], y.shape[1]
        S = y[0, 0].numel()
        lib = _L()
        pack_z = int(pack_z) if (training and C % 8 == 0) else 0
        pack_dy = bool(pack_dy and res_pre is None and C % 8 == 0)
        ctx.lazy_dy = bool(lazy_dy and res_pre is None and not pack_dy)
        with torch.cuda.device_of(y):
            zexps = torch.empty((C,), device=y.device, dtype=torch.int32) if pack_z else None
            rpre = _slots_of(res_pre) if (pack_z and res_pre is not None) else None
            rpost = _slots_of(res_post) if (pack_z and res_post is not None) else None
            stats = bn_stats_vector(y, gamma, beta, running_mean, running_var, training, momentum, eps, part, zexps, rpre, rpost)
            ymax = torch.empty((C * CSLOTS,), device=y.device, dtype=torch.int32) if pack_dy else None
            z = torch.empty_like(y)
            if pack_z:
                zp = z if pack_z == 1 else torch.empty_like(y)
                _chk(lib.dca_bn_apply_pack(_ptr(y), _ptr(stats), _ptr(zexps), _ptr(zp), N, C, S, float(slope), _ptr(ymax),
                                           _ptr(res_pre), _ptr(res_post), _ptr(z) if pack_z == 2 else None,
                                           _ptr(zmax) if pack_z == 2 else None, _stream()), "dca_bn_apply_pack")
                ymax_slots = lib.dca_bn_pack_chunks(C, S)
                _tag_px2(zp, zexps)
                if pack_z == 2:
                    _tag_twin(z, zp)
            else:
                _chk(lib.dca_bn_apply(_ptr(y), _ptr(stats), _ptr(res_pre), _ptr(res_post), _ptr(z), N, C, S, float(slope),
                                      _ptr(zmax), _ptr(ymax), _stream()), "dca_bn_apply")
                ymax_slots = lib.dca_bn_num_chunks(C, S)
        ctx.save_for_backward(y, stats, res_pre if slope != 1.0 else None, ymax)
        ctx.meta = (training, slope, res_pre is not None, res_post is not None, pack_dy, ymax_slots)
        return z if pack_z == 1 else _tag_cmax(z, zmax, ymax_slots)

    @staticmethod
    def backward(ctx, dz):
        y, stats, res_pre, ymax = ctx.saved_tensors
        training, slope, has_pre, has_post, pack_dy, ymax_slots = ctx.meta
        dz = _req(dz, "batch_norm.backward")
        N, C = y.shape[0], y.shape[1]
        S = y[0, 0].numel()
        lib = _L()
        with torch.cuda.device_of(y):
            nchunk = lib.dca_bn_num_chunks(C, S)
            part = torch.empty((C * nchunk * 2,), device=y.device, dtype=torch.float64)
            dgb = torch.empty((4 * C,), device=y.device, dtype=torch.float32)
            g_out = None
            if ctx.lazy_dy:
                _chk(lib.dca_bn_backward_reduce(_ptr(dz), _ptr(y), _ptr(stats), _ptr(part), _ptr(dgb), N, C, S, float(slope),
                                                int(training), _stream()), "dca_bn_backward_reduce")
                dy = dz.view_as(dz)
                dy._dca_lazy = (y, stats, dgb, slope, training)
            elif pack_dy:
                dyexps = torch.empty((C,), device=y.device, dtype=torch.int32)
                gmax = torch.empty((C * CSLOTS,), device=y.device, dtype=torch.int32)
                dy = torch.empty_like(y)
                _chk(lib.dca_bn_backward_pack(_ptr(dz), _ptr(y), _ptr(stats), _ptr(part), _ptr(dgb), _ptr(dy), _ptr(dyexps),
                                              _ptr(gmax), _ptr(ymax), ymax_slots if ymax is not None else 0, N, C, S,
                                              float(slope), int(training), _stream()), "dca_bn_backward_pack")
                _tag_px2(dy, dyexps)
            else:
                dy = torch.empty_like(y)
                want_g = has_pre and slope != 1.0 and ctx.needs_input_grad[9]
                g_out = torch.empty_like(y) if want_g else None
                dm = _cslots(C, y.device) if CONV_X2 else None
                _chk(lib.dca_bn_backward(_ptr(dz), _ptr(y), _ptr(res_pre), _ptr(stats), _ptr(part), _ptr(dgb), _ptr(dy),
                                         _ptr(g_out), N, C, S, float(slope), int(training), _ptr(dm), _stream()),
                     "dca_bn_backward")
                _tag_cmax(dy, dm, nchunk)
        g_pre = None
        if has_pre and ctx.needs_input_grad[9]:
            g_pre = g_out if g_out is not None else dz
        g_post = dz if (has_post and ctx.needs_input_grad[10]) else None
        return dy, dgb[:C], dgb[C:2 * C], None, None, None, None, None, None, g_pre, g_post, None, None, None, None, None


_tls = threading.local()


class frozen_weights:

    def __enter__(self):
        self.prev = getattr(_tls, "frozen", None)
        _tls.frozen = {}
        return self

    def __exit__(self, *exc):
        _tls.frozen = self.prev
        return False


_PLAN_RECORDER = None
_PLAN_ACTIVE = None


class PrepackPlan:

    def __init__(self):
        self.entries = {}
        self.table = None
        self.n = 0

    def recording(self):
        plan = self

        class _Rec:
            def __enter__(self_inner):
                global _PLAN_RECORDER
                self_inner.prev, _PLAN_RECORDER = _PLAN_RECORDER, plan

            def __exit__(self_inner, *exc):
                global _PLAN_RECORDER
                _PLAN_RECORDER = self_inner.prev
                return False
        return _Rec()

    def finalize(self):
        import struct
        rows = []
        for out, desc, tensors in self.entries.values():
            kind, A, Bn, Apad, Bpad, K, src_ab, flip, Btotal, b_off = desc
            nch = (A + 15) // 16
            rows.append(struct.pack("<QQ12iq", tensors[0].data_ptr(), out.data_ptr(), kind, A, Bn, Apad, Bpad, K, src_ab,
                                    flip, Btotal, b_off, nch, 0, out.numel()))
        self.n = len(rows)
        if self.n:
            dev = next(iter(self.entries.values()))[0].device
            self.table = torch.frombuffer(bytearray(b"".join(rows)), dtype=torch.uint8).to(dev)
        return self

    def refresh(self):
        if self.n:
            _chk(_L().dca_conv3d_prep_many(_ptr(self.table), self.n, _stream()), "dca_conv3d_prep_many")

    def active(self):
        plan = self

        class _Act:
            def __enter__(self_inner):
                global _PLAN_ACTIVE
                self_inner.prev = _PLAN_ACTIVE
                _PLAN_ACTIVE = {k: out for k, (out, _, _t) in plan.entries.items()}

            def __exit__(self_inner, *exc):
                global _PLAN_ACTIVE
                _PLAN_ACTIVE = self_inner.prev
                return False
        return _Act()


def _memo(key, tensors, build, desc=None):
    rec = _PLAN_RECORDER
    if rec is not None:
        out = build()
        t = tensors[0] if tensors else None
        if desc is not None and t is not None and t.is_leaf and t._base is None:
            rec.entries[(key,) + tuple((id(x), x.data_ptr()) for x in tensors)] = (out, desc, tensors)
        return out
    act = _PLAN_ACTIVE
    if act is not None and desc is not None:
        hit = act.get((key,) + tuple((id(x), x.data_ptr()) for x in tensors))
        if hit is not None:
            return hit
    cache = getattr(_tls, "frozen", None)
    if cache is None or (tensors and tensors[0].is_cuda and torch.cuda.is_current_stream_capturing()):
        return build()
    k = (key,) + tuple((id(t), t.data_ptr()) for t in tensors)
    hit = cache.get(k)
    if hit is None:
        hit = cache[k] = (build(), tensors)
    return hit[0]


class batched_bn_counters:

    def __enter__(self):
        self.prev = getattr(_tls, "pending", None)
        _tls.pending = []
        return self

    def __exit__(self, *exc):
        pending, _tls.pending = _tls.pending, self.prev
        if pending:
            torch._foreach_add_(pending, 1)
        return False


def bn_act(y, bn, slope=1.0, res_pre=None, res_post=None, stats_part=None, pack_out=False, pack_dy=False, lazy_dy=False):
    momentum = 0.1 if bn.momentum is None else bn.momentum
    training = bn.training or bn.running_mean is None
    if _lp_dtype() is not None:
        raise RuntimeError("ops.reduced_precision is inference only: call the model in eval mode under torch.no_grad()")
    C = y.shape[1]
    pack_z = 0
    if pack_out and PACK and CONV_X2 and training and C % 8 == 0 and torch.is_grad_enabled():
        pack_z = 2 if pack_out == "both" else 1
    pack_dy = bool(pack_dy and PACK and CONV_X2 and res_pre is None and C % 8 == 0)
    zm = _cslots(C, y.device) if (CONV_X2 and pack_z != 1) else None
    z = _BnAct.apply(y, bn.weight, bn.bias, bn.running_mean, bn.running_var, training, momentum, bn.eps, float(slope),
                     res_pre, res_post, stats_part if training else None, zm, pack_z, pack_dy,
                     bool(lazy_dy and res_pre is None))
    if bn.training and bn.num_batches_tracked is not None:
        pending = getattr(_tls, "pending", None)
        if pending is not None:
            pending.append(bn.num_batches_tracked)
        else:
            bn.num_batches_tracked.add_(1)
    return z


class reduced_precision:

    def __init__(self, dtype):
        if dtype not in LP_DTYPES:
            raise ValueError("reduced_precision: torch.bfloat16 or torch.float16")
        self.dtype = dtype

    def __enter__(self):
        self.prev = getattr(_tls, "lp", None)
        _tls.lp = self.dtype
        return self

    def __exit__(self, *exc):
        _tls.lp = self.prev
        return False


def _lp_dtype():
    return getattr(_tls, "lp", None)


def _pack_dy_ok(x, x2, conv, transposed, stride, res_pre):
    if not (PACK and res_pre is None and _k3s1(conv.weight, stride, transposed, x2)):
        return False
    Cout, Cin = conv.weight.shape[0], conv.weight.shape[1]
    if Cout % 8 or _conv_family(x, None, Cin, Cout, 3, 1, False) != "x2":
        return False
    return _x2_pairs(_is_packed(x), True, x.shape[-1]) and (_is_packed(x) or x.data_ptr() % 16 == 0)


def convbn3d(x, conv, bn, slope=1.0, res_pre=None, res_post=None, x2=None, alias=False, pack_out=False):
    transposed = isinstance(conv, torch.nn.ConvTranspose3d)
    stride = conv.stride[0]
    if alias:
        fuse = (PAIR_FUSE and torch.is_grad_enabled() and x.requires_grad and _k3s1(conv.weight, stride, transposed, x2)
                and _lp_dtype() is None and x.dtype == torch.float32)
        if not fuse:
            return convbn3d(x, conv, bn, slope, res_pre, res_post, x2), x
        stats = bool(BN_FUSE and bn.training)
        pdy = _pack_dy_ok(x, None, conv, False, 1, res_pre)
        out = _Conv3d.apply(x, None, conv.weight, 1, False, stats, True, pdy)
        y, part, xa = (out[0], out[1], out[2]) if stats else (out[0], None, out[1])
        z = bn_act(y, bn, slope, res_pre, res_post, part if (part is not None and part.numel()) else None,
                   pack_out=pack_out, pack_dy=pdy)
        return z, xa
    if not bn.training and not torch.is_grad_enabled():
        lp = _lp_dtype()
        if lp is not None and not transposed and stride == 1 and conv.kernel_size[0] == 3 and x2 is None:
            with torch.cuda.device_of(x):
                stats = bn_eval_affine(bn)
            C = bn.num_features
            return conv3d_lp(x, conv.weight, lp, stats[2 * C:3 * C], stats[3 * C:], slope, res_pre, res_post,
                             out_dtype=x.dtype)
        xx = _req(x, "convbn3d")
        with torch.cuda.device_of(xx):
            stats = bn_eval_affine(bn)
        C = bn.num_features
        return conv3d_fused_inference(xx, conv.weight, stride, transposed, stats[2 * C:3 * C], stats[3 * C:], slope,
                                      res_pre, res_post, x2)
    if BN_FUSE and bn.training and conv.weight.shape[0 if not transposed else 1] > 1 and _lp_dtype() is None:
        pdy = _pack_dy_ok(x, x2, conv, transposed, stride, res_pre)
        lazy = not transposed and _c1_bwd_route(x, x2, conv.weight, res_pre) == "fused"
        y, part = _Conv3d.apply(x, x2, conv.weight, int(stride), bool(transposed), True, False, pdy, lazy)
        return bn_act(y, bn, slope, res_pre, res_post, part if part.numel() else None, pack_out=pack_out, pack_dy=pdy,
                      lazy_dy=lazy)
    if not transposed and _lp_dtype() is None and _c1_bwd_route(x, x2, conv.weight, res_pre) == "fused":
        y = _Conv3d.apply(x, x2, conv.weight, int(stride), False, False, False, False, True)
        return bn_act(y, bn, slope, res_pre, res_post, lazy_dy=True)
    if _is_packed(x) and _pack_dy_ok(x, x2, conv, transposed, stride, res_pre):
        y = _Conv3d.apply(x, x2, conv.weight, int(stride), bool(transposed), False, False, True)
        return bn_act(y, bn, slope, res_pre, res_post, pack_dy=True)
    y = conv3d(x, conv.weight, stride, transposed, x2)
    return bn_act(y, bn, slope, res_pre, res_post)


class _AvgPool3d(torch.autograd.Function):
    @staticmethod
    def forward(ctx, x):
        x = _req(x, "avg_pool3d")
        N, C, D, H, W = x.shape
        y = torch.empty((N, C, (D + 1) // 2, (H + 1) // 2, (W + 1) // 2), device=x.device, dtype=torch.float32)
        with torch.cuda.device_of(x):
            _chk(_L().dca_avgpool3d_fwd(_ptr(x), _ptr(y), N * C, D, H, W, _stream()), "dca_avgpool3d_fwd")
        ctx.shape = tuple(x.shape)
        return y

    @staticmethod
    def backward(ctx, gy):
        gy = _req(gy, "avg_pool3d.backward")
        N, C, D, H, W = ctx.shape
        gx = torch.empty(ctx.shape, device=gy.device, dtype=torch.float32)
        with torch.cuda.device_of(gy):
            _chk(_L().dca_avgpool3d_bwd(_ptr(gy), _ptr(gx), None, None, N * C, D, H, W, _stream()), "dca_avgpool3d_bwd")
        return gx


class _PoolFork(torch.autograd.Function):

    @staticmethod
    def forward(ctx, x, third):
        x = _req(x, "avg_pool3d")
        N, C, D, H, W = x.shape
        y = torch.empty((N, C, (D + 1) // 2, (H + 1) // 2, (W + 1) // 2), device=x.device, dtype=torch.float32)
        with torch.cuda.device_of(x):
            _chk(_L().dca_avgpool3d_fwd(_ptr(x), _ptr(y), N * C, D, H, W, _stream()), "dca_avgpool3d_fwd")
        ctx.shape = tuple(x.shape)
        ctx.set_materialize_grads(False)
        if third:
            return y, x.view_as(x), x.view_as(x)
        return y, x.view_as(x)

    @staticmethod
    def backward(ctx, gy, gx2, gx3=None):
        extra = [g for g in (gx2, gx3) if g is not None]
        if gy is None:
            return (extra[0] + extra[1] if len(extra) == 2 else (extra[0] if extra else None)), None
        gy = _req(gy, "avg_pool3d.backward")
        res = _opt(extra[0], "avg_pool3d.backward") if extra else None
        res2 = _opt(extra[1], "avg_pool3d.backward") if len(extra) == 2 else None
        N, C, D, H, W = ctx.shape
        gx = torch.empty(ctx.shape, device=gy.device, dtype=torch.float32)
        with torch.cuda.device_of(gy):
            _chk(_L().dca_avgpool3d_bwd(_ptr(gy), _ptr(gx), _ptr(res), _ptr(res2), N * C, D, H, W, _stream()),
                 "dca_avgpool3d_bwd")
        return gx, None


def avg_pool3d_fork(x, third=False):
    if PAIR_FUSE and torch.is_grad_enabled() and x.requires_grad and x.dtype == torch.float32:
        outs = _PoolFork.apply(x, bool(third))
        for o in outs[1:]:
            _copy_tags(x, o)
        return outs
    return (avg_pool3d_k3s2p1(x), x, x) if third else (avg_pool3d_k3s2p1(x), x)


class _Trilinear(torch.autograd.Function):
    @staticmethod
    def forward(ctx, x, scale):
        x = _req(x, "interpolate")
        N, C, D, H, W = x.shape
        y = torch.empty((N, C, D * scale, H * scale, W * scale), device=x.device, dtype=torch.float32)
        with torch.cuda.device_of(x):
            _chk(_L().dca_trilinear_fwd(_ptr(x), _ptr(y), N * C, D, H, W, scale, _stream()), "dca_trilinear_fwd")
        ctx.meta = (tuple(x.shape), scale)
        return y

    @staticmethod
    def backward(ctx, gy):
        shape, scale = ctx.meta
        gy = _req(gy, "interpolate.backward")
        N, C, D, H, W = shape
        gx = torch.empty(shape, device=gy.device, dtype=torch.float32)
        with torch.cuda.device_of(gy):
            _chk(_L().dca_trilinear_bwd(_ptr(gy), _ptr(gx), N * C, D, H, W, scale, _stream()), "dca_trilinear_bwd")
        return gx, None


def avg_pool3d_k3s2p1(x):
    return _AvgPool3d.apply(x)


def trilinear_upsample(x, scale):
    return _Trilinear.apply(x, int(scale))


class _ContextInject(torch.autograd.Function):
    @staticmethod
    def forward(ctx, x, preds):
        x, preds = _req(x, "context_inject"), _req(preds, "context_inject.preds")
        B, C, n = x.shape[:3]
        HW = x.shape[3] * x.shape[4]
        key = torch.empty_like(x)
        kstar = torch.empty((B, HW), device=x.device, dtype=torch.int32)
        e = torch.empty((B, HW), device=x.device, dtype=torch.float32)
        pm = torch.empty_like(e)
        denom = torch.empty((B, n), device=x.device, dtype=torch.float32)
        part = torch.empty((B * ((HW + 255) // 256) * n,), device=x.device, dtype=torch.float32)
        with torch.cuda.device_of(x):
            _chk(_L().dca_context_inject_fwd(_ptr(x), _ptr(preds), _ptr(key), _ptr(kstar), _ptr(e), _ptr(pm),
                                             _ptr(denom), _ptr(part), B, C, n, HW, _stream()), "dca_context_inject_fwd")
        ctx.save_for_backward(x, preds, kstar, e, pm, denom)
        ctx.mark_non_differentiable(kstar)
        return key, kstar

    @staticmethod
    def backward(ctx, dkey, _unused):
        x, preds, kstar, e, pm, denom = ctx.saved_tensors
        dkey = _req(dkey, "context_inject.backward")
        B, C, n = x.shape[:3]
        HW = x.shape[3] * x.shape[4]
        dx, dpreds = torch.empty_like(x), torch.empty_like(preds)
        dw = torch.empty_like(e)
        T = torch.empty_like(denom)
        part = torch.empty((B * ((HW + 255) // 256) * n,), device=x.device, dtype=torch.float32)
        with torch.cuda.device_of(x):
            _chk(_L().dca_context_inject_bwd(_ptr(dkey), _ptr(x), _ptr(preds), _ptr(kstar), _ptr(e), _ptr(pm),
                                             _ptr(denom), _ptr(dx), _ptr(dpreds), _ptr(dw), _ptr(T), _ptr(part), B, C,
                                             n, HW, _stream()), "dca_context_inject_bwd")
        return dx, dpreds


class _DispAttention(torch.autograd.Function):
    @staticmethod
    def forward(ctx, q, k, v):
        q, k, v = _req(q, "attention.q"), _req(k, "attention.k"), _req(v, "attention.v")
        B, C, n = q.shape[:3]
        HW = q.shape[3] * q.shape[4]
        out = torch.empty_like(q)
        with torch.cuda.device_of(q):
            _chk(_L().dca_disp_attention_fwd(_ptr(q), _ptr(k), _ptr(v), _ptr(out), B, C, n, HW, _stream()),
                 "dca_disp_attention_fwd")
        ctx.save_for_backward(q, k, v)
        return out

    @staticmethod
    def backward(ctx, dout):
        q, k, v = ctx.saved_tensors
        dout = _req(dout, "attention.backward")
        B, C, n = q.shape[:3]
        HW = q.shape[3] * q.shape[4]
        dq, dk, dv = torch.empty_like(q), torch.empty_like(k), torch.empty_like(v)
        with torch.cuda.device_of(q):
            _chk(_L().dca_disp_attention_bwd(_ptr(q), _ptr(k), _ptr(v), _ptr(dout), _ptr(dq), _ptr(dk), _ptr(dv), B,
                                             C, n, HW, _stream()), "dca_disp_attention_bwd")
        return dq, dk, dv


def context_inject(x, preds):
    return _ContextInject.apply(x, preds)


def disparity_attention(q, k, v):
    if q.dim() != 5 or q.shape[1] % 8 or q.shape[2] > 64:
        raise RuntimeError(f"disparity_attention: needs (B, C % 8 == 0, n <= 64, H, W) tensors, got {tuple(q.shape)} "
                           "(n = maxdisp/8 with the down-sampling cva, maxdisp/4 without)")
    return _DispAttention.apply(q, k, v)


class _ConvexUp4(torch.autograd.Function):
    @staticmethod
    def forward(ctx, mask_logits, disp):
        mask_logits, disp = _req(mask_logits, "convex_upsample4.mask"), _req(disp, "convex_upsample4.disp")
        B, C, h, w = mask_logits.shape
        if C != 144 or tuple(disp.shape) != (B, 1, h, w):
            raise RuntimeError(f"convex_upsample4: expected mask (B,144,h,w) and disp (B,1,h,w), got "
                               f"{tuple(mask_logits.shape)} and {tuple(disp.shape)}")
        up = torch.empty((B, 1, 4 * h, 4 * w), device=disp.device, dtype=torch.float32)
        with torch.cuda.device_of(disp):
            _chk(_L().dca_convex_up4_fwd(_ptr(mask_logits), _ptr(disp), _ptr(up), B, h, w, _stream()),
                 "dca_convex_up4_fwd")
        ctx.save_for_backward(mask_logits, disp)
        return up

    @staticmethod
    def backward(ctx, gup):
        mask_logits, disp = ctx.saved_tensors
        gup = _req(gup, "convex_upsample4.backward")
        B, _, h, w = mask_logits.shape
        gl, gd = torch.empty_like(mask_logits), torch.empty_like(disp)
        wk = torch.empty((B, 9, h, w), device=disp.device, dtype=torch.float32)
        with torch.cuda.device_of(disp):
            _chk(_L().dca_convex_up4_bwd(_ptr(mask_logits), _ptr(disp), _ptr(gup), _ptr(gl), _ptr(gd), _ptr(wk), B, h, w,
                                         _stream()), "dca_convex_up4_bwd")
        return gl, gd


def convex_upsample4(mask_logits, disp):
    return _ConvexUp4.apply(mask_logits, disp)


CONF_MAX_PLANES = _C["DCA_CONF_MAX_PLANES"]


def convex_upsample4_planes(mask_logits, planes, scales):
    _req_no_grad("convex_upsample4_planes", mask_logits, planes)
    mask_logits, planes = _req(mask_logits, "convex_upsample4_planes.mask"), _req(planes, "convex_upsample4_planes.planes")
    scales = [float(v) for v in scales]
    if mask_logits.dim() != 4 or planes.dim() != 4:
        raise RuntimeError(f"convex_upsample4_planes: expected mask (B,144,h,w) and planes (B,P,h,w), got "
                           f"{tuple(mask_logits.shape)} and {tuple(planes.shape)}")
    B, C, h, w = mask_logits.shape
    P = planes.shape[1]
    if C != 144 or tuple(planes.shape) != (B, P, h, w) or not 1 <= P <= CONF_MAX_PLANES or len(scales) != P \
            or planes.numel() == 0:
        raise RuntimeError(f"convex_upsample4_planes: expected mask (B,144,h,w), planes (B,P,h,w) with 1 <= P <= "
                           f"{CONF_MAX_PLANES} and P scales, got {tuple(mask_logits.shape)}, {tuple(planes.shape)} and "
                           f"{len(scales)} scales")
    up = torch.empty((B, P, 4 * h, 4 * w), device=planes.device, dtype=torch.float32)
    sc = (ctypes.c_float * P)(*scales)
    with torch.cuda.device_of(planes):
        _chk(_L().dca_convex_up4_planes(_ptr(mask_logits), _ptr(planes), ctypes.cast(sc, _vp), _ptr(up), B, P, h, w,
                                        _stream()), "dca_convex_up4_planes")
    return up


class _FocalLevels(torch.autograd.Function):

    @staticmethod
    def forward(ctx, gt, coef, weights, *ests):
        ests = [_req(e, "focal_loss.est") for e in ests]
        gt = _req(gt, "focal_loss.gt")
        B, K = ests[0].shape[0], ests[0].shape[1]
        HW = ests[0][0, 0].numel()
        n = len(ests)
        if n > 8 or K > 256 or K < 2 or any(e.shape != ests[0].shape for e in ests) or gt.numel() != B * HW:
            raise RuntimeError("focal_loss: at most 8 equally shaped (B,K<=256,H,W) estimates per call and a ground truth "
                               "pooled to (B,1,H,W)")
        lib = _L()
        work = torch.empty((lib.dca_focal_loss_workspace(n, B, HW),), device=gt.device, dtype=torch.float64)
        out = torch.empty((n + 1,), device=gt.device, dtype=torch.float32)
        eptr = (ctypes.c_void_p * n)(*[e.data_ptr() for e in ests])
        wts = (ctypes.c_float * n)(*[float(w) for w in weights])
        with torch.cuda.device_of(gt):
            _chk(lib.dca_focal_loss_fwd(eptr, wts, n, _ptr(gt), _ptr(work), _ptr(out), B, K, HW, float(coef), _stream()),
                 "dca_focal_loss_fwd")
        ctx.save_for_backward(gt, work, *ests)
        ctx.meta = (float(coef), [float(w) for w in weights])
        return out[n]

    @staticmethod
    def backward(ctx, gloss):
        gt, work, *ests = ctx.saved_tensors
        coef, weights = ctx.meta
        n = len(ests)
        B, K = ests[0].shape[0], ests[0].shape[1]
        HW = ests[0][0, 0].numel()
        gloss = _req(gloss.reshape(1), "focal_loss.backward")
        gests = [torch.empty_like(e) for e in ests]
        eptr = (ctypes.c_void_p * n)(*[e.data_ptr() for e in ests])
        gptr = (ctypes.c_void_p * n)(*[g.data_ptr() for g in gests])
        wts = (ctypes.c_float * n)(*weights)
        with torch.cuda.device_of(gt):
            _chk(_L().dca_focal_loss_bwd(eptr, gptr, wts, n, _ptr(gt), _ptr(work), _ptr(gloss), B, K, HW, coef, _stream()),
                 "dca_focal_loss_bwd")
        return (None, None, None) + tuple(gests)
# ... 901 lines not shown
```

### include/dca_hip.h

```cpp
#ifndef DCA_HIP_H
#define DCA_HIP_H

#include <hip/hip_runtime_api.h>

#ifdef __cplusplus
extern "C" {
#endif

#define DCA_ABI_VERSION 20
int dca_abi_version(void);

#define DCA_BF16 1
#define DCA_FP16 2

int dca_gwc_volume_fwd(const float* ref, const float* tgt, float* vol, int B, int C, int H, int W, int maxdisp,
                       int num_groups, hipStream_t stream);
int dca_gwc_volume_bwd(const float* gvol, const float* ref, const float* tgt, float* gref, float* gtgt, int B, int C,
                       int H, int W, int maxdisp, int num_groups, hipStream_t stream);
int dca_concat_volume_fwd(const float* ref, const float* tgt, float* vol, int B, int C, int H, int W, int maxdisp,
                          hipStream_t stream);
int dca_concat_volume_bwd(const float* gvol, float* gref, float* gtgt, int B, int C, int H, int W, int maxdisp,
                          hipStream_t stream);

int dca_cost_volume_fwd(const float* const* refs, const float* const* tgts, const int* seg_channels, int nseg,
                        const float* cref, const float* ctgt, int Cc, void* vol, int B, int H, int W, int maxdisp,
                        int num_groups, int dtype, unsigned* vmax, hipStream_t stream);

int dca_softargmin_fwd(const float* x, float* out, int B, int K, long HW, int mode, hipStream_t stream);
int dca_softargmin_bwd(const float* aux, const float* g, float* gx, int B, int K, long HW, int mode,
                       hipStream_t stream);

int dca_up_softargmin_fwd(const float* logits, float* disp, int B, int n, int hc, int wc, int scale, hipStream_t stream);
int dca_up_softargmin_bwd(const float* logits, const float* gdisp, float* g1, float* glogits, int B, int n, int hc,
                          int wc, int scale, hipStream_t stream);

int dca_conv3d_prep_weight(const float* w, float* wt, int A, int B, int Apad, int Bpad, int K, int src_ab, int flip,
                           int Btotal, int b_off, hipStream_t stream);
int dca_conv3d_forward(const float* x, const float* x2, const float* wt, float* y, const float* scale,
                       const float* shift, const float* res_pre, const float* res_post, float slope, int N, int Cin,
                       int C1, int Cout, int CinPad, int CoutTotal, int co_off, int Di, int Hi, int Wi, int Do, int Ho,
                       int Wo, int ksize, int stride, int transposed, hipStream_t stream);
long dca_conv3d_wgrad_workspace(int N, int Cx, int Cy, int Do, int Ho, int Wo, int ksize, int stride);
int dca_conv3d_wgrad(const float* x, const float* dy, float* part, float* dw, int N, int Cx, int Cy, int Di, int Hi,
                     int Wi, int Do, int Ho, int Wo, int ksize, int stride, long s_cy, long s_cx, hipStream_t stream);

long dca_conv1_bwd_fused_workspace(int N, long S, int two);
int dca_conv1_bwd_fused(const float* dz, const float* y, const float* stats, const float* dgb, float slope, int training,
                        const float* x, const float* x2, const float* w, float* part, float* dx, float* dx2, float* dw,
                        long s_cy, long s_cx, int N, int C1, int C2, int Cout, long S, hipStream_t stream);

long dca_conv1_x3_weight_bytes(int A);
int dca_conv1_x3_prep_weight(const float* w, void* wfrag, int A, int Bn, int src_ab, int Btotal, int b_off,
                             hipStream_t stream);
int dca_conv1_x3_forward(const float* x, const float* x2, const void* wfrag, float* y, const float* scale,
                         const float* shift, const float* res_pre, const float* res_post, float slope, int N, int C1,
                         int C2, int Cout, int CoutTotal, int co_off, long S, hipStream_t stream);

int dca_conv3d_prep_many(const void* table, int n, hipStream_t stream);

int dca_tile_walk(long tiles, int grid, int wg, int* walk);

long dca_conv3d_x3_weight_bytes(int Cin, int Cout);
int dca_conv3d_x3_prep_weight(const float* w, void* wx, int A, int B, int src_ab, int flip, hipStream_t stream);
int dca_conv3d_x3_forward(const float* x, const void* wx, float* y, const float* scale, const float* shift,
                          const float* res_pre, const float* res_post, float slope, int N, int Cin, int Cout, int D,
                          int H, int W, hipStream_t stream);

int dca_deconv3d_x3_forward(const float* x, const void* wx, float* y, const float* scale, const float* shift,
                            const float* res_pre, const float* res_post, float slope, int N, int Cin, int Cout, int Di,
                            int Hi, int Wi, hipStream_t stream);

long dca_conv3d_x3_stats_chunks(int N, int Cout, int D, int H, int W);
int dca_conv3d_x3_forward_stats(const float* x, const void* wx, float* y, double* stat_part, int N, int Cin, int Cout,
                                int D, int H, int W, hipStream_t stream);
long dca_conv1_x3_stats_chunks(int N, long S);
int dca_conv1_x3_forward_stats(const float* x, const float* x2, const void* wfrag, float* y, double* stat_part, int N,
                               int C1, int C2, int Cout, int CoutTotal, int co_off, long S, hipStream_t stream);
long dca_deconv3d_x3_stats_chunks(int N, int Di, int Hi, int Wi);
int dca_deconv3d_x3_forward_stats(const float* x, const void* wx, float* y, double* stat_part, int N, int Cin, int Cout,
                                  int Di, int Hi, int Wi, hipStream_t stream);
int dca_bn_finalize_centered(const double* part, int nchunk, const float* gamma, const float* beta, float* running_mean,
                             float* running_var, float momentum, float eps, float* stats, int* zexps,
                             const unsigned* rpre_slots, int rpre_n, const unsigned* rpost_slots, int rpost_n, int C,
                             hipStream_t stream);

long dca_conv3d_wgrad_x3_workspace(int N, int Cx, int Cy, int D, int H, int W);
int dca_conv3d_wgrad_x3(const float* x, const float* dy, float* part, float* dw, int N, int Cx, int Cy, int D, int H,
                        int W, long s_cy, long s_cx, hipStream_t stream);

#define DCA_AMAX_CSLOTS 1024
int dca_cmax_f32(const float* x, int N, int C, long S, unsigned* slots, hipStream_t stream);
int dca_cmax_exps(const unsigned* slots, int nslots, int C, int* exps, hipStream_t stream);
long dca_conv3d_x2_weight_bytes(int Cin, int Cout);
int dca_conv3d_x2_prep_weight(const float* w, void* wx, int A, int B, int src_ab, int flip, const unsigned* x_slots,
                              int nslots, int* xexps, hipStream_t stream);
int dca_conv3d_x2_forward(const void* x, int packed, const int* xexps, const void* wx, float* y, const float* scale,
                          const float* shift, const float* res_pre, const float* res_post, float slope, unsigned* y_cmax,
                          int N, int Cin, int Cout, int D, int H, int W, hipStream_t stream);
long dca_conv3d_x2_stats_chunks(int N, int Cout, int D, int H, int W);
int dca_conv3d_x2_forward_stats(const void* x, int packed, const int* xexps, const void* wx, float* y, double* stat_part,
                                int N, int Cin, int Cout, int D, int H, int W, hipStream_t stream);
long dca_conv3d_wgrad_s2_x2_workspace(int N, int Cx, int Cy, int D, int H, int W);
int dca_conv3d_wgrad_s2_x2(const float* f, const int* f_exps, const float* c, const int* c_exps, float* part,
                           float* dw, int N, int Cx, int Cy, int D, int H, int W, long s_cy, long s_cx, hipStream_t stream);
long dca_conv3d_s2x2_weight_bytes(int Cin, int Cout);
int dca_conv3d_s2x2_prep_weight(const float* w, void* wx, int A, int B, int src_ab, int flip, const unsigned* x_slots,
                                int nslots, int* xexps, hipStream_t stream);
long dca_conv3d_s2x2_out_slots(int N, int Cout, int Di, int Hi, int Wi);
int dca_conv3d_s2x2_forward(const float* x, const int* xexps, const void* wx, float* y, const float* scale, const float* shift,
                            float slope, const float* res_post, unsigned* y_cmax, int N, int Cin, int Cout, int Di, int Hi, int Wi,
                            hipStream_t stream);
long dca_conv3d_wgrad_x2_workspace(int N, int Cx, int Cy, int D, int H, int W);
int dca_conv3d_wgrad_x2(const void* x, int x_packed, const int* xexps, const void* dy, int dy_packed, const int* yexps,
                        float* part, float* dw, int N, int Cx, int Cy, int D, int H, int W, long s_cy, long s_cx,
                        hipStream_t stream);

int dca_conv3d_c1_gather(const float* T, float* y, int N, int D, int H, int W, hipStream_t stream);
int dca_conv3d_c1_wgrad(const float* x, const float* dy, float* part, float* dw, int N, int C, int D, int H, int W,
                        hipStream_t stream);
int dca_conv3d_c1_expand(const float* dy, float* G, int N, int D, int H, int W, hipStream_t stream);
int dca_conv3d_c1_bwd_data(const float* dy, const float* w, float* dx, int N, int C, int D, int H, int W,
                           hipStream_t stream);

int dca_bn_num_chunks(int C, long S);
int dca_bn_pack_chunks(int C, long S);
int dca_bn_stats(const float* x, double* part, int N, int C, long S, hipStream_t stream);
int dca_bn_finalize(const double* part, int nchunk, double count, const float* gamma, const float* beta,
                    float* running_mean, float* running_var, float momentum, float eps, int training, float* stats,
                    int* zexps, const unsigned* rpre_slots, int rpre_n, const unsigned* rpost_slots, int rpost_n, int C,
                    hipStream_t stream);
int dca_bn_apply(const float* y, const float* stats, const float* res_pre, const float* res_post, float* z, int N,
                 int C, long S, float slope, unsigned* zmax, unsigned* ymax, hipStream_t stream);
int dca_bn_apply_pack(const float* y, const float* stats, const int* zexps, void* zp, int N, int C, long S, float slope,
                      unsigned* ymax, const float* res_pre, const float* res_post, float* zf, unsigned* zmax,
                      hipStream_t stream);
int dca_bn_backward(const float* dz, const float* y, const float* res_pre, const float* stats, double* part,
                    float* dgb, float* dy, float* g_out, int N, int C, long S, float slope, int training,
                    unsigned* dmax, hipStream_t stream);
int dca_bn_backward_reduce(const float* dz, const float* y, const float* stats, double* part, float* dgb, int N, int C,
                           long S, float slope, int training, hipStream_t stream);
int dca_bn_backward_pack(const float* dz, const float* y, const float* stats, double* part, float* dgb, void* dyp,
                         int* dyexps, unsigned* gmax, const unsigned* ymax, int ymax_slots, int N, int C, long S,
                         float slope, int training, hipStream_t stream);

int dca_avgpool3d_fwd(const float* x, float* y, long NC, int Di, int Hi, int Wi, hipStream_t stream);
int dca_avgpool3d_bwd(const float* gy, float* gx, const float* res, const float* res2, long NC, int Di, int Hi, int Wi,
                     hipStream_t stream);

int dca_trilinear_fwd(const float* x, float* y, long NC, int Di, int Hi, int Wi, int scale, hipStream_t stream);
int dca_trilinear_bwd(const float* gy, float* gx, long NC, int Di, int Hi, int Wi, int scale, hipStream_t stream);

int dca_context_inject_fwd(const float* x, const float* preds, float* key, int* kstar, float* e, float* pm,
                           float* denom, float* part, int B, int C, int n, long HW, hipStream_t stream);
int dca_context_inject_bwd(const float* dkey, const float* x, const float* preds, const int* kstar, const float* e,
                           const float* pm, const float* denom, float* dx, float* dpreds, float* dw, float* T,
                           float* part, int B, int C, int n, long HW, hipStream_t stream);

int dca_disp_attention_fwd(const float* q, const float* k, const float* v, float* out, int B, int C, int n, long HW,
                           hipStream_t stream);
int dca_disp_attention_bwd(const float* q, const float* k, const float* v, const float* dout, float* dq, float* dk,
                           float* dv, int B, int C, int n, long HW, hipStream_t stream);

int dca_convex_up4_fwd(const float* mask_logits, const float* disp, float* up, int B, int h, int w, hipStream_t stream);
int dca_convex_up4_bwd(const float* mask_logits, const float* disp, const float* gup, float* glogits, float* gdisp,
                       float* wk, int B, int h, int w, hipStream_t stream);

long dca_focal_loss_workspace(int nlev, int B, long HW);
int dca_focal_loss_fwd(const float* const* ests, const float* weights, int nlev, const float* gt, double* work,
                       float* out, int B, int K, long HW, float focal_coefficient, hipStream_t stream);
int dca_focal_loss_bwd(const float* const* ests, float* const* gests, const float* weights, int nlev, const float* gt,
                       const double* work, const float* gloss, int B, int K, long HW, float focal_coefficient,
                       hipStream_t stream);

long dca_conv3d_lp_weight_bytes(int Cin, int Cout);
int dca_conv3d_lp_prep_weight(const float* w, void* wx, int A, int B, int src_ab, int flip, int dtype,
                              hipStream_t stream);
int dca_conv3d_lp_forward(const void* x, const void* wx, void* y, const float* scale, const float* shift,
                          const void* res_pre, const void* res_post, float slope, int N, int Cin, int Cout, int D, int H,
                          int W, int dtype, int in_f32, int out_f32, hipStream_t stream);

long dca_conv1_lp_weight_bytes(int C1, int C2);
int dca_conv1_lp_prep_weight(const float* w, void* wfrag, int Cout, int C1, int C2, int dtype, hipStream_t stream);
int dca_conv1_lp_forward(const void* x, const void* x2, const void* wfrag, void* y, const float* scale,
                         const float* shift, const void* res_pre, const void* res_post, float slope, int N, int C1,
                         int C2, int Cout, long S, int dtype, int out_f32, hipStream_t stream);

int dca_conv3d_forward_mixed(const void* x, const float* wt, void* y, const float* scale, const float* shift,
                             const void* res_pre, const void* res_post, float slope, int N, int Cin, int Cout, int CinPad,
                             int Di, int Hi, int Wi, int Do, int Ho, int Wo, int transposed, int dtype,
                             hipStream_t stream);
long dca_conv3d_s2_lp_weight_bytes(int Cin);
int dca_conv3d_s2_lp_prep_weight(const float* w, void* wx, int Cin, int Cout, int dtype, hipStream_t stream);
int dca_conv3d_s2_lp_forward(const void* x, const void* wx, float* y, const float* scale, const float* shift, float slope,
                             int N, int Cin, int Cout, int D, int H, int W, int dtype, hipStream_t stream);
int dca_deconv3d_lp_forward(const float* x, const void* wx, void* y, const float* scale, const float* shift,
                            const void* res_pre, const void* res_post, float slope, int N, int Cin, int Cout, int Di,
                            int Hi, int Wi, int dtype, hipStream_t stream);
int dca_avgpool3d_lp_fwd(const void* x, float* y, long NC, int Di, int Hi, int Wi, int dtype, hipStream_t stream);
int dca_trilinear_up2_lp_fwd(const float* x, void* y, long NC, int Di, int Hi, int Wi, int dtype, hipStream_t stream);

#define DCA_EVAL_REC 8
long dca_disp_metrics_workspace(int B, int H, int W);
int dca_disp_metrics(const float* pred, const float* gt, const unsigned char* mask, double* rec, void* workspace, int B,
                     int H, int W, int top_pad, int right_pad, float maxdisp, hipStream_t stream);
#define DCA_EVAL_MAX_CLASSES 64
int dca_region_confusion(const float* vol0, const float* vol1, const float* vol2, const float* gt, long long* cm,
                         int nvol, int B, int C, int hp, int wp, int H, int W, hipStream_t stream);
#define DCA_EVAL_BATCHES 0
#define DCA_EVAL_SUMS 1
#define DCA_EVAL_IMG_KEPT 11
#define DCA_EVAL_IMG_EPE 12
#define DCA_EVAL_IMG_D1 13
#define DCA_EVAL_IMG_THRES 14
#define DCA_EVAL_IMG_SEEN 17
#define DCA_EVAL_PIXELS 18
#define DCA_EVAL_STATE_HEAD 32
long dca_eval_state_len(int C);
int dca_eval_accumulate(const double* rec, const long long* cm, double* state, int B, int nvol, int C, int H, int W,
                        hipStream_t stream);

int dca_frame_hist(const unsigned char* left, const unsigned char* right, unsigned* hist, int H, int W, int C,
                   hipStream_t stream);
int dca_frame_lut(const unsigned* hist, long n_pixels, float* lut, double* stats, hipStream_t stream);
int dca_frame_apply(const unsigned char* left, const unsigned char* right, const float* lut, float* out_left,
                    float* out_right, int H, int W, int C, int Hc, int Wc, int src_y0, int dst_y0, int rows, int cols,
                    hipStream_t stream);
int dca_disp_export(const float* pred, float* out_f32, unsigned short* out_u16, int Hc, int Wc, int y0, int h, int w,
                    float scale, hipStream_t stream);

int dca_train_luma_sum(const unsigned char* left, const unsigned char* right, const unsigned char* bg, long long* S, int H,
                       int W, int C, hipStream_t stream);
int dca_train_tables(const long long* S, long n_pixels, const unsigned char* bg, float f_left, float f_right,
                     const float* norm, unsigned char* U, float* T, hipStream_t stream);
int dca_train_patch_colour(const unsigned char* right, const unsigned char* U, long long* sums, unsigned char* colour,
                           int H, int W, int C, int y1, int x1, int th, int tw, hipStream_t stream);
int dca_train_crop_norm(const unsigned char* left, const unsigned char* right, const float* T, const float* norm,
                        const unsigned char* colour, float* out_left, float* out_right, int H, int W, int C, int y1, int x1,
                        int th, int tw, int py0, int px0, int ph, int pw, hipStream_t stream);
int dca_train_disp_crop(const void* src, int src_u16, float* gt, unsigned char* mask, int H, int W, int y1, int x1, int th,
                        int tw, int flip_rows, float scale, int inf_to_zero, float maxdisp, hipStream_t stream);

#define DCA_CONF_DISP 0
#define DCA_CONF_DUNI 1
#define DCA_CONF_MASS 2
#define DCA_CONF_ENT 3
#define DCA_CONF_STD 4
#define DCA_CONF_PLANES 5
int dca_softargmin_stats(const float* logits, float* out, int B, int K, long HW, int radius, hipStream_t stream);
#define DCA_CONF_MAX_PLANES 8
int dca_convex_up4_planes(const float* mask_logits, const float* planes, const float* scales, float* up, int B, int P,
                          int h, int w, hipStream_t stream);
#define DCA_CONF_MAX_BINS 1024
#define DCA_CONF_ERR_SCALE 1048576
int dca_conf_histogram(const float* conf, const float* pred, const float* gt, long long* state, int B, long HW, int nbins,
                       float maxdisp, hipStream_t stream);

#define DCA_LR_MAX_W 8192
int dca_mirror_pair(const float* left, const float* right, float* out_left, float* out_right, int N, int H, int W,
                    hipStream_t stream);
int dca_lr_consistency(const float* dl, const float* drm, float* diff, float* valid, float* filled, float* disp_right,
                       int B, int H, int W, int cols, float tau, hipStream_t stream);

#define DCA_PC_TILE 1024
#define DCA_PC_RECORD_BYTES 16
int dca_disp_to_depth(const float* pred, const float* mask, float* out_f32, unsigned short* out_u16, int Hc, int Wc, int y0,
                      int rows, int cols, float fb, float doffs, float min_disp, float max_depth, float mask_min,
                      float scale, hipStream_t stream);
long dca_point_cloud_tiles(int rows, int cols);
int dca_point_cloud(const float* pred, const float* mask, const unsigned char* rgb, int C, int Hsrc, int Wsrc, void* vertices,
                    long cap, unsigned* tile_offsets, long long* count, int Hc, int Wc, int y0, int rows, int cols, int v0,
                    int stride, float f, float fb, float cx, float cy, float doffs, float min_disp, float max_depth,
                    float mask_min, hipStream_t stream);

#define DCA_SELFSUP_MAX_LEVELS 8
#define DCA_SELFSUP_TILE_W 64
#define DCA_SELFSUP_TILE_H 16
#define DCA_SELFSUP_SUMS 4
#define DCA_SELFSUP_OUT 5
int dca_selfsup_loss_fwd(const float* left, const float* right, const float* const* disps, const float* weights, int nlev,
                         const void* valid, int valid_u8, double* work, float* out, int B, int H, int W, float alpha,
                         float lam, float c1, float c2, float photo_scale, hipStream_t stream);
int dca_selfsup_loss_bwd(const float* left, const float* right, const float* const* disps, float* const* gdisps,
                         const float* weights, int nlev, const void* valid, int valid_u8, const float* out,
                         const float* gloss, int B, int H, int W, float alpha, float lam, float c1, float c2,
                         float photo_scale, hipStream_t stream);

#define DCA_RECT_FRAC_BITS 5
#define DCA_RECT_MAX_SRC 16384
int dca_rectify_pair(const unsigned char* left, const unsigned char* right, const int* maps, long map_plane,
                     unsigned char* out_left, unsigned char* out_right, int Hs, int Ws, int Hd, int Wd, int C,
                     hipStream_t stream);

#define DCA_ERRMAP_BINS 10
#define DCA_ERRMAP_RGB_0 0x313695
#define DCA_ERRMAP_RGB_1 0x4575B4
#define DCA_ERRMAP_RGB_2 0x74ADD1
#define DCA_ERRMAP_RGB_3 0xABD9E9
#define DCA_ERRMAP_RGB_4 0xE0F3F8
#define DCA_ERRMAP_RGB_5 0xFEE090
#define DCA_ERRMAP_RGB_6 0xFDAE61
#define DCA_ERRMAP_RGB_7 0xF46D43
#define DCA_ERRMAP_RGB_8 0xD73027
#define DCA_ERRMAP_RGB_9 0xA50026
#define DCA_ERRMAP_LEGEND_ROWS 10
#define DCA_ERRMAP_LEGEND_STEP 20
int dca_disp_error_image(const float* pred, const float* gt, float* out_f32, unsigned char* out_u8, int B, int H, int W,
                         int top_pad, int right_pad, float abs_thres, float rel_thres, int legend, hipStream_t stream);
long dca_disp_range_workspace(int B, int rows, int cols);
int dca_disp_range(const float* disp, const float* mask, float* range, void* workspace, int B, int Hc, int Wc, int y0,
                   int rows, int cols, float mask_min, hipStream_t stream);
#define DCA_CMAP_GRAY 0
#define DCA_CMAP_KITTI 1
#define DCA_KITTI_EDGE_0 0
#define DCA_KITTI_EDGE_1 114
#define DCA_KITTI_EDGE_2 299
#define DCA_KITTI_EDGE_3 413
#define DCA_KITTI_EDGE_4 587
#define DCA_KITTI_EDGE_5 701
#define DCA_KITTI_EDGE_6 886
#define DCA_KITTI_EDGE_7 1000
#define DCA_KITTI_CORNERS 0x76325410
int dca_disp_colorize(const float* disp, const float* mask, const float* range, unsigned char* out_u8, int Hc, int Wc, int y0,
                      int rows, int cols, float max_disp, float mask_min, int cmap, hipStream_t stream);

#define DCA_LIDAR_MAX_RADIUS 8
int dca_lidar_disparity(const float* points, long N, int S, long n, float m00, float m01, float m02, float m03, float m10,
                        float m11, float m12, float m13, float m20, float m21, float m22, float m23, int H, int W, float fb,
                        float doffs, float min_depth, float max_depth, float min_disp, float max_disp, int rx, int ry,
                        double rel, float* disp, float* depth, unsigned short* disp_u16, long long* count, unsigned* zbuf,
                        hipStream_t stream);

#ifdef __cplusplus
}
#endif
#endif
```

Baseline: 43.45.

## Fold skip-branch BatchNorm into the consuming BN apply and backward kernels

Adds a path where the 1x1 skip branch's BatchNorm (affine, slope 1) is not materialised. Its normalisation is applied inline inside the downstream BN apply/pack kernel and BN backward kernels, which now read the raw skip conv output y_r and stats_r. The backward kernel also accumulates the skip BN's gradient partials, so a full-tensor write, read and separate backward pass for the skip activation are avoided. In exchange it adds a separate max-scan kernel over y_r, extra registers per thread, and more routing and API complexity.

Result: faster. 44.10 (median of 6 runs) (+1.5%).

```diff
diff --git a/cost-volume-aggregation-in-stereo-matching-revisited_amd/csrc/pointwise.hip b/cost-volume-aggregation-in-stereo-matching-revisited_amd/csrc/pointwise.hip
--- a/cost-volume-aggregation-in-stereo-matching-revisited_amd/csrc/pointwise.hip
+++ b/cost-volume-aggregation-in-stereo-matching-revisited_amd/csrc/pointwise.hip
@@ -134,6 +134,14 @@
 }
 
 
+__device__ __forceinline__ float bn_affine(float y, float sc, float sh) { return __fmaf_rn(y, sc, sh); }
+__device__ __forceinline__ float bn_skip(float y, float sc, float sh) { return act_apply(bn_affine(y, sc, sh), 1.f); }
+__device__ __forceinline__ void bn_bwd_acc(float g, float y, float mean, float invstd, float& a0, float& a1) {
+#pragma clang fp contract(off)
+  a0 += g;
+  a1 += g * (y - mean) * invstd;
+}
+
 __global__ __launch_bounds__(256) void bn_apply_kernel(const float* __restrict__ y, const float* __restrict__ stats,
                                                        const float* __restrict__ res_pre, const float* __restrict__ res_post,
                                                        float* __restrict__ z, int N, int C, long S, long chunk_len,
@@ -149,7 +157,7 @@
       for (long i = s0 + 4 * tid; i < s1; i += 1024) {
         float4 v = *(const float4*)(y + base + i);
         ym = fmaxf(fmaxf(ym, fmaxf(fabsf(v.x - mean), fabsf(v.y - mean))), fmaxf(fabsf(v.z - mean), fabsf(v.w - mean)));
-        v.x = v.x * sc + sh; v.y = v.y * sc + sh; v.z = v.z * sc + sh; v.w = v.w * sc + sh;
+        v.x = bn_affine(v.x, sc, sh); v.y = bn_affine(v.y, sc, sh); v.z = bn_affine(v.z, sc, sh); v.w = bn_affine(v.w, sc, sh);
         if (res_pre) { const float4 r = *(const float4*)(res_pre + base + i); v.x += r.x; v.y += r.y; v.z += r.z; v.w += r.w; }
         v.x = act_apply(v.x, slope); v.y = act_apply(v.y, slope); v.z = act_apply(v.z, slope); v.w = act_apply(v.w, slope);
         if (res_post) { const float4 r = *(const float4*)(res_post + base + i); v.x += r.x; v.y += r.y; v.z += r.z; v.w += r.w; }
@@ -160,7 +168,7 @@
       for (long i = s0 + tid; i < s1; i += 256) {
         const float yv = y[base + i];
         ym = fmaxf(ym, fabsf(yv - mean));
-        float v = yv * sc + sh;
+        float v = bn_affine(yv, sc, sh);
         if (res_pre) v += res_pre[base + i];
         v = act_apply(v, slope);
         if (res_post) v += res_post[base + i];
@@ -181,15 +189,17 @@
 }
 typedef unsigned short u16x8 __attribute__((ext_vector_type(8)));
 
+template <bool SKIP>
 __global__ __launch_bounds__(256) void bn_apply_pack_kernel(const float* __restrict__ y, const float* __restrict__ stats,
                                                             const int* __restrict__ zexps, char* __restrict__ zp, int N,
                                                             int C, long S, long chunk_len, float slope,
                                                             unsigned* __restrict__ ymax, const float* __restrict__ res_pre,
                                                             const float* __restrict__ res_post, float* __restrict__ zf,
-                                                            unsigned* __restrict__ zmax) {
+                                                            unsigned* __restrict__ zmax, const float* __restrict__ y_r,
+                                                            const float* __restrict__ stats_r) {
   const int cg = blockIdx.y, ch = blockIdx.x, tid = threadIdx.x;
   const long s0 = ch * chunk_len, s1 = min(S, s0 + chunk_len);
-  float mean[8], sc[8], sh[8], ym[8], zm[8];
+  float mean[8], sc[8], sh[8], scr[8], shr[8], ym[8], zm[8];
   int ex[8];
 #pragma unroll
   for (int j = 0; j < 8; ++j) {
@@ -197,6 +207,8 @@
     mean[j] = stats ? stats[c] : 0.f;
     sc[j] = stats ? stats[2 * C + c] : 1.f;
     sh[j] = stats ? stats[3 * C + c] : 0.f;
+    scr[j] = SKIP ? stats_r[2 * C + c] : 0.f;
+    shr[j] = SKIP ? stats_r[3 * C + c] : 0.f;
     ex[j] = dca_coherent_loadi(zexps + c);
     ym[j] = zm[j] = 0.f;
   }
@@ -210,14 +222,15 @@
 #pragma unroll
       for (int j = 0; j < 8; ++j) {
         v[j] = yb[j * S + i];
-        rp[j] = res_pre ? res_pre[cb + j * S + i] : -0.f;
+        rp[j] = (!SKIP && res_pre) ? res_pre[cb + j * S + i] : -0.f;
         rq[j] = res_post ? res_post[cb + j * S + i] : -0.f;
+        if (SKIP) rp[j] = bn_skip(y_r[cb + j * S + i], scr[j], shr[j]);
       }
       u16x8 hv, lv;
 #pragma unroll
       for (int j = 0; j < 8; ++j) {
         ym[j] = fmaxf(ym[j], fabsf(v[j] - mean[j]));
-        const float zz = act_apply(v[j] * sc[j] + sh[j] + rp[j], slope) + rq[j];
+        const float zz = act_apply(bn_affine(v[j], sc[j], sh[j]) + rp[j], slope) + rq[j];
         if (zf) zf[cb + j * S + i] = zz;
         zm[j] = fmaxf(zm[j], fabsf(zz));
         unsigned short h, l;
@@ -238,15 +251,17 @@
   }
 }
 
+template <bool SKIP>
 __global__ __launch_bounds__(256) void bn_apply_pack4_kernel(const float* __restrict__ y, const float* __restrict__ stats,
                                                              const int* __restrict__ zexps, char* __restrict__ zp, int N,
                                                              int C, long S, long chunk_len, float slope,
                                                              unsigned* __restrict__ ymax, const float* __restrict__ res_pre,
                                                              const float* __restrict__ res_post, float* __restrict__ zf,
-                                                             unsigned* __restrict__ zmax) {
+                                                             unsigned* __restrict__ zmax, const float* __restrict__ y_r,
+                                                             const float* __restrict__ stats_r) {
   const int cg = blockIdx.y, ch = blockIdx.x, tid = threadIdx.x;
   const long s0 = ch * chunk_len, s1 = min(S, s0 + chunk_len);
-  float mean[8], sc[8], sh[8], ym[8], zm[8];
+  float mean[8], sc[8], sh[8], scr[8], shr[8], ym[8], zm[8];
   int ex[8];
 #pragma unroll
   for (int j = 0; j < 8; ++j) {
@@ -254,6 +269,8 @@
     mean[j] = stats ? stats[c] : 0.f;
     sc[j] = stats ? stats[2 * C + c] : 1.f;
     sh[j] = stats ? stats[3 * C + c] : 0.f;
+    scr[j] = SKIP ? stats_r[2 * C + c] : 0.f;
+    shr[j] = SKIP ? stats_r[3 * C + c] : 0.f;
     ex[j] = dca_coherent_loadi(zexps + c);
     ym[j] = zm[j] = 0.f;
   }
@@ -267,14 +284,19 @@
       for (int j = 0; j < 8; ++j) {
         const float4 v4 = *(const float4*)(y + cb + j * S + i);
         float4 p4 = make_float4(-0.f, -0.f, -0.f, -0.f), q4 = p4;
-        if (res_pre) p4 = *(const float4*)(res_pre + cb + j * S + i);
+        if (!SKIP && res_pre) p4 = *(const float4*)(res_pre + cb + j * S + i);
         if (res_post) q4 = *(const float4*)(res_post + cb + j * S + i);
+        if (SKIP) {
+          const float4 r4 = *(const float4*)(y_r + cb + j * S + i);
+          p4 = make_float4(bn_skip(r4.x, scr[j], shr[j]), bn_skip(r4.y, scr[j], shr[j]), bn_skip(r4.z, scr[j], shr[j]),
+                           bn_skip(r4.w, scr[j], shr[j]));
+        }
         const float v[4] = {v4.x, v4.y, v4.z, v4.w}, rp[4] = {p4.x, p4.y, p4.z, p4.w}, rq[4] = {q4.x, q4.y, q4.z, q4.w};
         float zz[4];
 #pragma unroll
         for (int e = 0; e < 4; ++e) {
           ym[j] = fmaxf(ym[j], fabsf(v[e] - mean[j]));
-          zz[e] = act_apply(v[e] * sc[j] + sh[j] + rp[e], slope) + rq[e];
+          zz[e] = act_apply(bn_affine(v[e], sc[j], sh[j]) + rp[e], slope) + rq[e];
           zm[j] = fmaxf(zm[j], fabsf(zz[e]));
           unsigned short h, l;
           px2_split(zz[e], ex[j], h, l);
@@ -318,6 +340,28 @@
   dca_cmax_put(m, slots + (long)c * DCA_AMAX_CSLOTS + ch);
 }
 
+__global__ __launch_bounds__(256) void bn_skip_max_kernel(const float* __restrict__ y_r, const float* __restrict__ stats_r,
+                                                          int N, int C, long S, long chunk_len, int vec,
+                                                          unsigned* __restrict__ slots) {
+  const int c = blockIdx.y, ch = blockIdx.x, tid = threadIdx.x;
+  const long s0 = ch * chunk_len, s1 = min(S, s0 + chunk_len);
+  const float sc = stats_r[2 * C + c], sh = stats_r[3 * C + c];
+  float m = 0.f;
+  for (int n = N - 1; n >= 0; --n) {
+    const float* p = y_r + ((long)n * C + c) * S;
+    if (vec) {
+      for (long i = s0 + 4 * tid; i < s1; i += 1024) {
+        const float4 v = *(const float4*)(p + i);
+        m = fmaxf(fmaxf(m, fmaxf(fabsf(bn_skip(v.x, sc, sh)), fabsf(bn_skip(v.y, sc, sh)))),
+                  fmaxf(fabsf(bn_skip(v.z, sc, sh)), fabsf(bn_skip(v.w, sc, sh))));
+      }
+    } else {
+      for (long i = s0 + tid; i < s1; i += 256) m = fmaxf(m, fabsf(bn_skip(p[i], sc, sh)));
+    }
+  }
+  dca_cmax_put(m, slots + (long)c * DCA_AMAX_CSLOTS + ch);
+}
+
 __global__ __launch_bounds__(64) void cmax_exps_kernel(const unsigned* __restrict__ slots, int nslots, int* __restrict__ exps) {
   const int c = blockIdx.x, lane = threadIdx.x;
   unsigned v = 0;
@@ -332,11 +376,15 @@
                                                             const float* __restrict__ stats,
                                                             double* __restrict__ part, int N, int C, long S,
                                                             int nchunk, long chunk_len, float slope, int vec,
-                                                            unsigned* __restrict__ gmax) {
+                                                            unsigned* __restrict__ gmax, const float* __restrict__ y_r,
+                                                            const float* __restrict__ stats_r, double* __restrict__ part_r) {
   const int c = blockIdx.x, ch = blockIdx.y, tid = threadIdx.x;
   const long s0 = ch * chunk_len, s1 = min(S, s0 + chunk_len);
   const float mean = stats[c], invstd = stats[C + c], sc = stats[2 * C + c], sh = stats[3 * C + c];
-  float a0 = 0.f, a1 = 0.f, gm = 0.f;
+  const float mean_r = y_r ? stats_r[c] : 0.f, invstd_r = y_r ? stats_r[C + c] : 0.f;
+  const float sc_r = y_r ? stats_r[2 * C + c] : 0.f, sh_r = y_r ? stats_r[3 * C + c] : 0.f;
+  const float* rsrc = y_r ? y_r : res_pre;
+  float a0 = 0.f, a1 = 0.f, b0 = 0.f, b1 = 0.f, gm = 0.f;
   for (int n = N - 1; n >= 0; --n) {
     const long base = ((long)n * C + c) * S;
     if (vec) {
@@ -344,36 +392,50 @@
         const float4 yv = *(const float4*)(y + base + i);
         const float4 dv = *(const float4*)(dz + base + i);
         float4 rv = make_float4(0.f, 0.f, 0.f, 0.f);
-        if (res_pre) rv = *(const float4*)(res_pre + base + i);
+        if (rsrc) rv = *(const float4*)(rsrc + base + i);
+        const float4 rr = rv;
+        if (y_r) rv = make_float4(bn_skip(rr.x, sc_r, sh_r), bn_skip(rr.y, sc_r, sh_r), bn_skip(rr.z, sc_r, sh_r), bn_skip(rr.w, sc_r, sh_r));
         const float ys[4] = {yv.x, yv.y, yv.z, yv.w}, ds[4] = {dv.x, dv.y, dv.z, dv.w}, rs[4] = {rv.x, rv.y, rv.z, rv.w};
+        const float yr[4] = {rr.x, rr.y, rr.z, rr.w};
 #pragma unroll
         for (int j = 0; j < 4; ++j) {
-          const float u = ys[j] * sc + sh + rs[j];
+          const float u = bn_affine(ys[j], sc, sh) + rs[j];
           const float g = ds[j] * (u > 0.f ? 1.f : slope);
-          a0 += g;
-          a1 += g * (ys[j] - mean) * invstd;
+          bn_bwd_acc(g, ys[j], mean, invstd, a0, a1);
+          if (part_r) bn_bwd_acc(g, yr[j], mean_r, invstd_r, b0, b1);
           gm = fmaxf(gm, fabsf(g));
         }
       }
     } else {
       for (long i = s0 + tid; i < s1; i += 256) {
         const float yv = y[base + i];
-        float u = yv * sc + sh;
-        if (res_pre) u += res_pre[base + i];
+        float u = bn_affine(yv, sc, sh), yrv = 0.f;
+        if (rsrc) {
+          yrv = rsrc[base + i];
+          u += y_r ? bn_skip(yrv, sc_r, sh_r) : yrv;
+        }
         const float g = dz[base + i] * (u > 0.f ? 1.f : slope);
-        a0 += g;
-        a1 += g * (yv - mean) * invstd;
+        bn_bwd_acc(g, yv, mean, invstd, a0, a1);
+        if (part_r) bn_bwd_acc(g, yrv, mean_r, invstd_r, b0, b1);
         gm = fmaxf(gm, fabsf(g));
       }
     }
   }
   double d0 = wave_sum_d((double)a0), d1 = wave_sum_d((double)a1);
-  __shared__ double red[8];
+  __shared__ double red[16];
   if ((tid & 63) == 0) { red[(tid >> 6) * 2] = d0; red[(tid >> 6) * 2 + 1] = d1; }
+  if (part_r) {
+    d0 = wave_sum_d((double)b0), d1 = wave_sum_d((double)b1);
+    if ((tid & 63) == 0) { red[8 + (tid >> 6) * 2] = d0; red[8 + (tid >> 6) * 2 + 1] = d1; }
+  }
   __syncthreads();
   if (tid == 0) {
     part[((long)c * nchunk + ch) * 2 + 0] = red[0] + red[2] + red[4] + red[6];
     part[((long)c * nchunk + ch) * 2 + 1] = red[1] + red[3] + red[5] + red[7];
+    if (part_r) {
+      part_r[((long)c * nchunk + ch) * 2 + 0] = red[8] + red[10] + red[12] + red[14];
+      part_r[((long)c * nchunk + ch) * 2 + 1] = red[9] + red[11] + red[13] + red[15];
+    }
   }
   if (gmax) dca_cmax_put(gm, gmax + (long)c * DCA_AMAX_CSLOTS + ch);
 }
@@ -420,10 +482,13 @@
                                     const float* __restrict__ res_pre, const float* __restrict__ stats,
                                     const float* __restrict__ dgb, float* __restrict__ dy, float* __restrict__ g_out,
                                     int N, int C, long S, long chunk_len, float slope, int training, int vec,
-                                    unsigned* __restrict__ dmax) {
+                                    unsigned* __restrict__ dmax, const float* __restrict__ y_r,
+                                    const float* __restrict__ stats_r) {
   const int c = blockIdx.y, ch = blockIdx.x, tid = threadIdx.x;
   const long s0 = ch * chunk_len, s1 = min(S, s0 + chunk_len);
   const float mean = stats[c], invstd = stats[C + c], sc = stats[2 * C + c], sh = stats[3 * C + c];
+  const float sc_r = y_r ? stats_r[2 * C + c] : 0.f, sh_r = y_r ? stats_r[3 * C + c] : 0.f;
+  const float* rsrc = y_r ? y_r : res_pre;
   const float k1 = training ? dgb[2 * C + c] : 0.f, k2 = training ? dgb[3 * C + c] * invstd : 0.f;
   float am = 0.f;
   for (int n = 0; n < N; ++n) {
@@ -432,12 +497,13 @@
       for (long i = s0 + 4 * tid; i < s1; i += 1024) {
         const float4 yv = *(const float4*)(y + base + i), dv = *(const float4*)(dz + base + i);
         float4 rv = make_float4(0.f, 0.f, 0.f, 0.f);
-        if (res_pre) rv = *(const float4*)(res_pre + base + i);
+        if (rsrc) rv = *(const float4*)(rsrc + base + i);
+        if (y_r) rv = make_float4(bn_skip(rv.x, sc_r, sh_r), bn_skip(rv.y, sc_r, sh_r), bn_skip(rv.z, sc_r, sh_r), bn_skip(rv.w, sc_r, sh_r));
         const float ys[4] = {yv.x, yv.y, yv.z, yv.w}, ds[4] = {dv.x, dv.y, dv.z, dv.w}, rs[4] = {rv.x, rv.y, rv.z, rv.w};
         float o[4], g[4];
 #pragma unroll
         for (int j = 0; j < 4; ++j) {
-          const float u = ys[j] * sc + sh + rs[j];
+          const float u = bn_affine(ys[j], sc, sh) + rs[j];
           g[j] = ds[j] * (u > 0.f ? 1.f : slope);
           o[j] = (g[j] - k1 - (ys[j] - mean) * k2) * sc;
         }
@@ -448,8 +514,11 @@
     } else {
       for (long i = s0 + tid; i < s1; i += 256) {
         const float yv = y[base + i];
-        float u = yv * sc + sh;
-        if (res_pre) u += res_pre[base + i];
+        float u = bn_affine(yv, sc, sh);
+        if (rsrc) {
+          const float r = rsrc[base + i];
+          u += y_r ? bn_skip(r, sc_r, sh_r) : r;
+        }
         const float g = dz[base + i] * (u > 0.f ? 1.f : slope);
         float v = g;
         if (training) v -= dgb[2 * C + c] + (yv - mean) * invstd * dgb[3 * C + c];
@@ -950,19 +1019,34 @@
   return dca_launch_status();
 }
 
+static int bn_apply_pack_launch(const float* y, const float* stats, const int* zexps, void* zp, int N, int C, long S,
+                                float slope, unsigned* ymax, const float* res_pre, const float* y_r, const float* stats_r,
+                                const float* res_post, float* zf, unsigned* zmax, hipStream_t stream) {
+  DCA_REQUIRE(y && zexps && zp && N > 0 && C > 0 && C % 8 == 0 && S > 0 && C / 8 <= 65535 && ((((uintptr_t)zp) & 15) == 0));
+  DCA_REQUIRE(stats != nullptr || (ymax == nullptr && slope == 1.f));
+  DCA_REQUIRE((y_r == nullptr) == (stats_r == nullptr) && (y_r == nullptr || (res_pre == nullptr && stats != nullptr)));
+  int nchunk; long len;
+  chunking(S, C / 8, &nchunk, &len);
+  const uintptr_t al = (uintptr_t)y | (uintptr_t)res_pre | (uintptr_t)y_r | (uintptr_t)res_post | (uintptr_t)zf;
+  const bool four = (res_pre || y_r || res_post) && S % 4 == 0 && (al & 15) == 0;
+  auto kern = y_r ? (four ? bn_apply_pack4_kernel<true> : bn_apply_pack_kernel<true>)
+                  : (four ? bn_apply_pack4_kernel<false> : bn_apply_pack_kernel<false>);
+  hipLaunchKernelGGL(kern, dim3(nchunk, C / 8), dim3(256), 0, stream, y, stats, zexps, (char*)zp, N, C, S, len, slope, ymax,
+                     res_pre, res_post, zf, zmax, y_r, stats_r);
+  return dca_launch_status();
+}
+
 extern "C" int dca_bn_apply_pack(const float* y, const float* stats, const int* zexps, void* zp, int N, int C, long S,
                                  float slope, unsigned* ymax, const float* res_pre, const float* res_post, float* zf,
                                  unsigned* zmax, hipStream_t stream) {
-  DCA_REQUIRE(y && zexps && zp && N > 0 && C > 0 && C % 8 == 0 && S > 0 && C / 8 <= 65535 && ((((uintptr_t)zp) & 15) == 0));
-  DCA_REQUIRE(stats != nullptr || (ymax == nullptr && slope == 1.f));
-  int nchunk; long len;
-  chunking(S, C / 8, &nchunk, &len);
-  const uintptr_t al = (uintptr_t)y | (uintptr_t)res_pre | (uintptr_t)res_post | (uintptr_t)zf;
-  const bool four = (res_pre || res_post) && S % 4 == 0 && (al & 15) == 0;
-  auto kern = four ? bn_apply_pack4_kernel : bn_apply_pack_kernel;
-  hipLaunchKernelGGL(kern, dim3(nchunk, C / 8), dim3(256), 0, stream, y, stats, zexps, (char*)zp, N, C, S, len, slope, ymax,
-                     res_pre, res_post, zf, zmax);
-  return dca_launch_status();
+  return bn_apply_pack_launch(y, stats, zexps, zp, N, C, S, slope, ymax, res_pre, nullptr, nullptr, res_post, zf, zmax, stream);
+}
+
+extern "C" int dca_bn_apply_pack_skip(const float* y, const float* stats, const int* zexps, void* zp, int N, int C, long S,
+                                      float slope, unsigned* ymax, const float* y_r, const float* stats_r,
+                                      const float* res_post, float* zf, unsigned* zmax, hipStream_t stream) {
+  DCA_REQUIRE(y_r && stats_r);
+  return bn_apply_pack_launch(y, stats, zexps, zp, N, C, S, slope, ymax, nullptr, y_r, stats_r, res_post, zf, zmax, stream);
 }
 
 extern "C" int dca_cmax_f32(const float* x, int N, int C, long S, unsigned* slots, hipStream_t stream) {
@@ -971,6 +1055,16 @@
   chunking(S, C, &nchunk, &len);
   const int vec = (S % 4 == 0) && ((((uintptr_t)x) & 15) == 0);
   hipLaunchKernelGGL(cmax_kernel, dim3(nchunk, C), dim3(256), 0, stream, x, N, C, S, len, vec, slots);
+  return dca_launch_status();
+}
+
+extern "C" int dca_bn_skip_max(const float* y_r, const float* stats_r, int N, int C, long S, unsigned* slots,
+                               hipStream_t stream) {
+  DCA_REQUIRE(y_r && stats_r && slots && N > 0 && C > 0 && S > 0 && C <= 65535);
+  int nchunk; long len;
+  chunking(S, C, &nchunk, &len);
+  const int vec = (S % 4 == 0) && ((((uintptr_t)y_r) & 15) == 0);
+  hipLaunchKernelGGL(bn_skip_max_kernel, dim3(nchunk, C), dim3(256), 0, stream, y_r, stats_r, N, C, S, len, vec, slots);
   return dca_launch_status();
 }
 
@@ -989,11 +1083,34 @@
   const uintptr_t al = (uintptr_t)dz | (uintptr_t)y | (uintptr_t)res_pre | (uintptr_t)dy | (uintptr_t)g_out;
   const int vec = (S % 4 == 0) && ((al & 15) == 0);
   hipLaunchKernelGGL(bn_bwd_reduce_kernel, dim3(C, nchunk), dim3(256), 0, stream, dz, y, res_pre, stats, part, N, C, S,
-                     nchunk, len, slope, vec, (unsigned*)nullptr);
+                     nchunk, len, slope, vec, (unsigned*)nullptr, (const float*)nullptr, (const float*)nullptr,
+                     (double*)nullptr);
   hipLaunchKernelGGL(bn_bwd_finalize_kernel, dim3(C), dim3(64), 0, stream, part, nchunk, (double)N * (double)S, dgb, C,
                      stats, training, (const unsigned*)nullptr, (const unsigned*)nullptr, 0, (int*)nullptr);
   hipLaunchKernelGGL(bn_bwd_apply_kernel, dim3(nchunk, C), dim3(256), 0, stream, dz, y, res_pre, stats, dgb, dy, g_out, N, C,
-                     S, len, slope, training, vec, dmax);
+                     S, len, slope, training, vec, dmax, (const float*)nullptr, (const float*)nullptr);
+  return dca_launch_status();
+}
+
+extern "C" int dca_bn_backward_skip(const float* dz, const float* y, const float* y_r, const float* stats,
+                                    const float* stats_r, double* part, double* part_r, float* dgb, float* dgb_r, float* dy,
+                                    float* g_out, int N, int C, long S, float slope, int training, unsigned* dmax,
+                                    hipStream_t stream) {
+  DCA_REQUIRE(dz && y && stats && part && dgb && dy && N > 0 && C > 0 && S > 0 && C <= 65535);
+  DCA_REQUIRE(y_r && stats_r && part_r && dgb_r && g_out && part_r != part && dgb_r != dgb);
+  int nchunk; long len;
+  chunking(S, C, &nchunk, &len);
+  const uintptr_t al = (uintptr_t)dz | (uintptr_t)y | (uintptr_t)y_r | (uintptr_t)dy | (uintptr_t)g_out;
+  const int vec = (S % 4 == 0) && ((al & 15) == 0);
+  const double count = (double)N * (double)S;
+  hipLaunchKernelGGL(bn_bwd_reduce_kernel, dim3(C, nchunk), dim3(256), 0, stream, dz, y, (const float*)nullptr, stats, part,
+                     N, C, S, nchunk, len, slope, vec, (unsigned*)nullptr, y_r, stats_r, part_r);
+  hipLaunchKernelGGL(bn_bwd_finalize_kernel, dim3(C), dim3(64), 0, stream, part, nchunk, count, dgb, C, stats, training,
+                     (const unsigned*)nullptr, (const unsigned*)nullptr, 0, (int*)nullptr);
+  hipLaunchKernelGGL(bn_bwd_finalize_kernel, dim3(C), dim3(64), 0, stream, (const double*)part_r, nchunk, count, dgb_r, C,
+                     stats_r, training, (const unsigned*)nullptr, (const unsigned*)nullptr, 0, (int*)nullptr);
+  hipLaunchKernelGGL(bn_bwd_apply_kernel, dim3(nchunk, C), dim3(256), 0, stream, dz, y, (const float*)nullptr, stats, dgb, dy,
+                     g_out, N, C, S, len, slope, training, vec, dmax, y_r, stats_r);
   return dca_launch_status();
 }
 
@@ -1004,7 +1121,8 @@
   chunking(S, C, &nchunk, &len);
   const int vec = (S % 4 == 0) && ((((uintptr_t)dz | (uintptr_t)y) & 15) == 0);
   hipLaunchKernelGGL(bn_bwd_reduce_kernel, dim3(C, nchunk), dim3(256), 0, stream, dz, y, (const float*)nullptr, stats, part,
-                     N, C, S, nchunk, len, slope, vec, (unsigned*)nullptr);
+                     N, C, S, nchunk, len, slope, vec, (unsigned*)nullptr, (const float*)nullptr, (const float*)nullptr,
+                     (double*)nullptr);
   hipLaunchKernelGGL(bn_bwd_finalize_kernel, dim3(C), dim3(64), 0, stream, part, nchunk, (double)N * (double)S, dgb, C,
                      stats, training, (const unsigned*)nullptr, (const unsigned*)nullptr, 0, (int*)nullptr);
   return dca_launch_status();
@@ -1020,7 +1138,7 @@
   const uintptr_t al = (uintptr_t)dz | (uintptr_t)y;
   const int vec = (S % 4 == 0) && ((al & 15) == 0);
   hipLaunchKernelGGL(bn_bwd_reduce_kernel, dim3(C, nchunk), dim3(256), 0, stream, dz, y, (const float*)nullptr, stats, part,
-                     N, C, S, nchunk, len, slope, vec, gmax);
+                     N, C, S, nchunk, len, slope, vec, gmax, (const float*)nullptr, (const float*)nullptr, (double*)nullptr);
   hipLaunchKernelGGL(bn_bwd_finalize_kernel, dim3(C), dim3(64), 0, stream, part, nchunk, (double)N * (double)S, dgb, C,
                      stats, training, (const unsigned*)gmax, ymax, ymax_slots, dyexps);
   int pchunk; long plen;
diff --git a/cost-volume-aggregation-in-stereo-matching-revisited_amd/models/augment/cva.py b/cost-volume-aggregation-in-stereo-matching-revisited_amd/models/augment/cva.py
--- a/cost-volume-aggregation-in-stereo-matching-revisited_amd/models/augment/cva.py
+++ b/cost-volume-aggregation-in-stereo-matching-revisited_amd/models/augment/cva.py
@@ -29,7 +29,7 @@
 
     def forward(self, x, res_post=None):
         c1, skip = ops.convbn3d_pair(x, self.conv1[0][0], self.conv1[0][1], 0.0, self.redir[0], self.redir[1], 1.0,
-                                     pack_a=True)
+                                     pack_a=True, skip_into=self.conv3[1])
         c2 = self.conv2(c1)
         return self.conv3(c2, slope=0.0, res_pre=skip, res_post=res_post, pack_out="both")
 
diff --git a/cost-volume-aggregation-in-stereo-matching-revisited_amd/ops.py b/cost-volume-aggregation-in-stereo-matching-revisited_amd/ops.py
--- a/cost-volume-aggregation-in-stereo-matching-revisited_amd/ops.py
+++ b/cost-volume-aggregation-in-stereo-matching-revisited_amd/ops.py
@@ -295,6 +295,7 @@
 CONV_S2_X2 = os.environ.get("DCA_CONV_S2", "x2") != "fp32"
 BN_FUSE = os.environ.get("DCA_BN_FUSE", "1") != "0"
 C1_BWD_FUSE = os.environ.get("DCA_C1_BWD", "fused") != "split"
+SKIP_FOLD = os.environ.get("DCA_SKIP_FOLD", "1") != "0"
 _X3_MIN_WORKGROUPS = 1
 
 
@@ -488,6 +489,24 @@
                                  _ptr(weight), _ptr(part), _ptr(gx), _ptr(gx2), _ptr(gw), C1 + C2, 1, N, C1, C2,
                                  weight.shape[0], S, _stream()), "dca_conv1_bwd_fused")
     return gx, gx2, gw
+
+
+class _SkipBn:
+    __slots__ = ("y", "part", "bn", "into")
+
+    def __init__(self, y, part, bn, into):
+        self.y, self.part, self.bn, self.into = y, part, bn, into
+
+
+def _skip_fold_route(x, conv_b, bn_b, slope_b, bn_out):
+    if not (SKIP_FOLD and PACK and CONV_X2 and bn_out is not None and torch.is_grad_enabled() and _lp_dtype() is None):
+        return "apply"
+    C = bn_b.num_features
+    if not (bn_b.training and bn_out.training) or bn_out.num_features != C or C % 8 or float(slope_b) != 1.0:
+        return "apply"
+    if x.dtype != torch.float32 or bn_b.weight is None or bn_b.bias is None:
+        return "apply"
+    return "fold" if _c1_bwd_route(x, None, conv_b.weight) == "fused" else "apply"
 
 
 def _k3s1(weight, stride, transposed, x2, head=False):
@@ -902,7 +921,7 @@
 PAIR_FUSE = os.environ.get("DCA_PAIR_FUSE", "1") != "0"
 
 
-def convbn3d_pair(x, conv_a, bn_a, slope_a, conv_b, bn_b, slope_b, pack_a=False):
+def convbn3d_pair(x, conv_a, bn_a, slope_a, conv_b, bn_b, slope_b, pack_a=False, skip_into=None):
     inference = (not bn_a.training and not bn_b.training and not torch.is_grad_enabled())
     ok = (PAIR_FUSE and not inference and _lp_dtype() is None and conv_a.kernel_size[0] == 3 and conv_a.stride[0] == 2
           and conv_b.kernel_size[0] == 1 and conv_b.weight.shape[0] in (32, 64) and x.dtype == torch.float32
@@ -910,9 +929,12 @@
     if not ok:
         return convbn3d(x, conv_a, bn_a, slope_a, pack_out=pack_a), convbn3d(x, conv_b, bn_b, slope_b)
     stats = bool(BN_FUSE and bn_a.training and bn_b.training)
-    lazy = _c1_bwd_route(x, None, conv_b.weight) == "fused"
+    fold = _skip_fold_route(x, conv_b, bn_b, slope_b, skip_into) == "fold"
+    lazy = fold or _c1_bwd_route(x, None, conv_b.weight) == "fused"
     ya, pa, yb, pb = _ConvPair.apply(x, conv_a.weight, conv_b.weight, stats, lazy)
     za = bn_act(ya, bn_a, slope_a, stats_part=pa if pa.numel() else None, pack_out=pack_a)
+    if fold:
+        return za, _SkipBn(yb, pb if pb.numel() else None, bn_b, skip_into)
     zb = bn_act(yb, bn_b, slope_b, stats_part=pb if pb.numel() else None, lazy_dy=lazy)
     return za, zb
 
@@ -1052,6 +1074,61 @@
         return dy, dgb[:C], dgb[C:2 * C], None, None, None, None, None, None, g_pre, g_post, None, None, None, None, None
 
 
+class _BnSkipAct(torch.autograd.Function):
+
+    @staticmethod
+    def forward(ctx, y, gamma, beta, running_mean, running_var, momentum, eps, part, y_r, gamma_r, beta_r, running_mean_r,
+                running_var_r, momentum_r, eps_r, part_r, slope, res_post, zmax):
+        y, y_r = _req(y, "batch_norm"), _req(y_r, "batch_norm.skip")
+        res_post = _opt(res_post, "res_post")
+        if y_r.shape != y.shape:
+            raise RuntimeError("batch_norm: the skip branch does not have the output's shape")
+        N, C = y.shape[0], y.shape[1]
+        S = y[0, 0].numel()
+        lib = _L()
+        with torch.cuda.device_of(y):
+            stats_r = bn_stats_vector(y_r, gamma_r, beta_r, running_mean_r, running_var_r, True, momentum_r, eps_r, part_r)
+            nchunk = lib.dca_bn_num_chunks(C, S)
+            rslots = torch.empty((C * CSLOTS,), device=y.device, dtype=torch.int32)
+            _chk(lib.dca_bn_skip_max(_ptr(y_r), _ptr(stats_r), N, C, S, _ptr(rslots), _stream()), "dca_bn_skip_max")
+            zexps = torch.empty((C,), device=y.device, dtype=torch.int32)
+            rpost = _slots_of(res_post) if res_post is not None else None
+            stats = bn_stats_vector(y, gamma, beta, running_mean, running_var, True, momentum, eps, part, zexps,
+                                    (rslots, nchunk), rpost)
+            z, zp = torch.empty_like(y), torch.empty_like(y)
+            _chk(lib.dca_bn_apply_pack_skip(_ptr(y), _ptr(stats), _ptr(zexps), _ptr(zp), N, C, S, float(slope), None, _ptr(y_r),
+                                            _ptr(stats_r), _ptr(res_post), _ptr(z), _ptr(zmax), _stream()),
+                 "dca_bn_apply_pack_skip")
+            _tag_px2(zp, zexps)
+            _tag_twin(z, zp)
+        ctx.save_for_backward(y, stats, y_r, stats_r)
+        ctx.meta = (slope, res_post is not None)
+        return _tag_cmax(z, zmax, lib.dca_bn_pack_chunks(C, S))
+
+    @staticmethod
+    def backward(ctx, dz):
+        y, stats, y_r, stats_r = ctx.saved_tensors
+        slope, has_post = ctx.meta
+        dz = _req(dz, "batch_norm.backward")
+        N, C = y.shape[0], y.shape[1]
+        S = y[0, 0].numel()
+        lib = _L()
+        with torch.cuda.device_of(y):
+            nchunk = lib.dca_bn_num_chunks(C, S)
+            part, part_r = (torch.empty((C * nchunk * 2,), device=y.device, dtype=torch.float64) for _ in range(2))
+            dgb, dgb_r = (torch.empty((4 * C,), device=y.device, dtype=torch.float32) for _ in range(2))
+            dy, g = torch.empty_like(y), torch.empty_like(y)
+            dm = _cslots(C, y.device)
+            _chk(lib.dca_bn_backward_skip(_ptr(dz), _ptr(y), _ptr(y_r), _ptr(stats), _ptr(stats_r), _ptr(part), _ptr(part_r),
+                                          _ptr(dgb), _ptr(dgb_r), _ptr(dy), _ptr(g), N, C, S, float(slope), 1, _ptr(dm),
+                                          _stream()), "dca_bn_backward_skip")
+            _tag_cmax(dy, dm, nchunk)
+            g._dca_lazy = (y_r, stats_r, dgb_r, 1.0, True)
+        g_post = dz if (has_post and ctx.needs_input_grad[17]) else None
+        return (dy, dgb[:C], dgb[C:2 * C], None, None, None, None, None, g, dgb_r[:C], dgb_r[C:2 * C], None, None, None, None,
+                None, None, g_post, None)
+
+
 _tls = threading.local()
 
 
@@ -1177,12 +1254,30 @@
     z = _BnAct.apply(y, bn.weight, bn.bias, bn.running_mean, bn.running_var, training, momentum, bn.eps, float(slope),
                      res_pre, res_post, stats_part if training else None, zm, pack_z, pack_dy,
                      bool(lazy_dy and res_pre is None))
+    _bn_count(bn)
+    return z
+
+
+def _bn_count(bn):
     if bn.training and bn.num_batches_tracked is not None:
         pending = getattr(_tls, "pending", None)
         if pending is not None:
             pending.append(bn.num_batches_tracked)
         else:
             bn.num_batches_tracked.add_(1)
+
+
+def bn_skip_act(y, bn, slope, skip, res_post=None, stats_part=None):
+    if skip.into is not bn:
+        raise RuntimeError("bn_skip_act: this skip branch was folded for another BatchNorm (convbn3d_pair, skip_into)")
+    br = skip.bn
+    mom = lambda b: 0.1 if b.momentum is None else b.momentum
+    zm = _cslots(y.shape[1], y.device)
+    z = _BnSkipAct.apply(y, bn.weight, bn.bias, bn.running_mean, bn.running_var, mom(bn), bn.eps, stats_part, skip.y,
+                         br.weight, br.bias, br.running_mean, br.running_var, mom(br), br.eps, skip.part, float(slope),
+                         res_post, zm)
+    _bn_count(br)
+    _bn_count(bn)
     return z
 
 
@@ -1219,6 +1314,14 @@
 def convbn3d(x, conv, bn, slope=1.0, res_pre=None, res_post=None, x2=None, alias=False, pack_out=False):
     transposed = isinstance(conv, torch.nn.ConvTranspose3d)
     stride = conv.stride[0]
+    if isinstance(res_pre, _SkipBn):
+        if pack_out != "both" or alias:
+            raise RuntimeError("convbn3d: a folded skip branch needs pack_out='both' (convbn3d_pair, skip_into)")
+        if BN_FUSE and conv.weight.shape[0 if not transposed else 1] > 1:
+            y, part = _Conv3d.apply(x, x2, conv.weight, int(stride), bool(transposed), True)
+        else:
+            y, part = conv3d(x, conv.weight, stride, transposed, x2), None
+        return bn_skip_act(y, bn, slope, res_pre, res_post, part if (part is not None and part.numel()) else None)
     if alias:
         fuse = (PAIR_FUSE and torch.is_grad_enabled() and x.requires_grad and _k3s1(conv.weight, stride, transposed, x2)
                 and _lp_dtype() is None and x.dtype == torch.float32)
diff --git a/include/dca_hip.h b/include/dca_hip.h
--- a/include/dca_hip.h
+++ b/include/dca_hip.h
@@ -142,6 +142,13 @@
 int dca_bn_backward_pack(const float* dz, const float* y, const float* stats, double* part, float* dgb, void* dyp,
                          int* dyexps, unsigned* gmax, const unsigned* ymax, int ymax_slots, int N, int C, long S,
                          float slope, int training, hipStream_t stream);
+int dca_bn_skip_max(const float* y_r, const float* stats_r, int N, int C, long S, unsigned* slots, hipStream_t stream);
+int dca_bn_apply_pack_skip(const float* y, const float* stats, const int* zexps, void* zp, int N, int C, long S, float slope,
+                           unsigned* ymax, const float* y_r, const float* stats_r, const float* res_post, float* zf,
+                           unsigned* zmax, hipStream_t stream);
+int dca_bn_backward_skip(const float* dz, const float* y, const float* y_r, const float* stats, const float* stats_r,
+                         double* part, double* part_r, float* dgb, float* dgb_r, float* dy, float* g_out, int N, int C,
+                         long S, float slope, int training, unsigned* dmax, hipStream_t stream);
 
 int dca_avgpool3d_fwd(const float* x, float* y, long NC, int Di, int Hi, int Wi, hipStream_t stream);
 int dca_avgpool3d_bwd(const float* gy, float* gx, const float* res, const float* res2, long NC, int Di, int Hi, int Wi,
```
